# Elliotshui/ABRSimulator

Hardware: AMD Instinct MI355X
Metric: env_steps_per_sec (higher is better)
Workload: dtype f64

## Files before the change

abrsimulator_amd/csrc/abr_env.hip:

```cpp
#include <hip/hip_runtime.h>

#include <climits>
#include <cmath>
#include <cstdarg>
#include <cstdio>
#include <cstdlib>
#include <cstring>
#include <new>
#include <type_traits>
#include <vector>

#include "abr_env.h"

#ifdef ABR_SPLIT_STAMPS
#include "abr_diag_stamps.h"
#else
#define ABR_STAMP(n)
#define ABR_STAMP_INIT()
#define ABR_STAMP_FLUSH()
#define ABR_WG_TIME(slot)
#define ABR_WG_WHERE(role)
#define K3_STAMP_DECL
#define K3_STAMP(n)
#define K3_STAMP_FLUSH()
// ... 104 lines not shown
    int32_t pending_speed_rows;
    bool pending_rule_on;
    abrx::SpeedRuleBlock pending_rule;
    bool speeds_dirty;
    const double *pending_br_table;
    bool br_table_dirty;
    bool armed;
    bool sampler_on;
    abrx::EpisodeSampler sampler;
    abrx::EpisodeLedger ledger;
};

static void apply_pending(abr_env *env) {
    if (env->br_table_dirty) { env->p.br_table = env->pending_br_table; env->br_table_dirty = false; }
    if (env->speeds_dirty) {
        env->p.lane_speeds = env->pending_speeds; env->p.speed_rows = env->pending_speed_rows;
        env->p.speed_rule = env->pending_rule;
        if (env->pending_rule_on) { env->p.lane_speeds = env->p.sd_lane; env->p.speed_rows = abrx::kSpeedRowsRule; }
        env->speeds_dirty = false;
    }
}

__device__ inline double chunk_bitrate(const EnvParams &p, int32_t chunk, int32_t rate) {
    return p.br_table ? p.br_table[(int64_t)chunk * p.n_rates + rate] : p.ladder[rate];
}

__host__ __device__ inline uint32_t philox_action(uint64_t seed, uint64_t lane, uint32_t step,
                                                  uint32_t episode, uint32_t n_rates) {
    uint32_t c0 = (uint32_t)lane, c1 = (uint32_t)(lane >> 32), c2 = step, c3 = episode;
    uint32_t k0 = (uint32_t)seed, k1 = (uint32_t)(seed >> 32);
#pragma unroll
    for (int r = 0; r < 10; r++) {
        uint64_t p0 = (uint64_t)0xD2511F53u * c0, p1 = (uint64_t)0xCD9E8D57u * c2;
        uint32_t n0 = (uint32_t)(p1 >> 32) ^ c1 ^ k0, n1 = (uint32_t)p1;
        uint32_t n2 = (uint32_t)(p0 >> 32) ^ c3 ^ k1, n3 = (uint32_t)p0;
        c0 = n0; c1 = n1; c2 = n2; c3 = n3;
        k0 += 0x9E3779B9u; k1 += 0xBB67AE85u;
    }
    return (uint32_t)(((uint64_t)c0 * n_rates) >> 32);
}

struct Lane {
    double buf, dl, target, c, c_next;
    long long sumk;
    int32_t k, k_end, chunk_id, n_su, n_rb, n_play, n_dl, j, tpos, tlen;
    int32_t avail_k, avail_next, cur_action, last_action;
    bool su, be, bf;
    bool done_dl;
    bool running;
    const double *trace;
};

__device__ inline void lane_head(Lane &s) {
    s.n_su += s.su ? 1 : 0;
    s.n_rb += (!s.su && s.be) ? 1 : 0;
    const bool call = s.done_dl && (s.k >= s.avail_k) && !s.bf;
    s.running = !call;
}

__device__ inline void lane_init(Lane &s, const EnvParams &p, int32_t offset0) {
    s.buf = 0.0; s.dl = 0.0; s.target = 0.0; s.sumk = 0;
    s.k = 0; s.chunk_id = 0; s.n_su = 0; s.n_rb = 0; s.n_play = 0; s.n_dl = 0;
    s.cur_action = -1; s.last_action = -1;
    s.su = true; s.be = true; s.bf = false;
    s.done_dl = true;
    s.j = 0;
    s.tpos = offset0 % s.tlen;
    s.avail_k = p.avail_tick[0];
    s.avail_next = s.avail_k;
    lane_head(s);
}

__device__ inline void lane_refresh_interval(Lane &s, const EnvParams &p) {
    int32_t ke = p.interval_tick[s.j + 1];
    while (s.k >= ke) {
        s.j++;
        s.tpos = (s.tpos + 1 == s.tlen) ? 0 : s.tpos + 1;
        ke = p.interval_tick[s.j + 1];
    }
    s.k_end = ke;
    const int32_t tn = (s.tpos + 1 == s.tlen) ? 0 : s.tpos + 1;
    s.c = s.trace[s.tpos] * kDt;
    s.c_next = s.trace[tn] * kDt;
}

__device__ inline double avg_latency_from(double sd, double play_time, long long sumk, int32_t n_play) {
    if (n_play == 0) return 0.0;
    double tri = (double)(((long long)n_play * (n_play - 1)) / 2);
    return (kDt * (double)sumk - sd * tri) / play_time;
}
__device__ inline double lane_avg_latency(const EnvParams &p, long long sumk, int32_t n_play) {
    return avg_latency_from(p.sd, p.GP[n_play], sumk, n_play);
}
__device__ inline double avg_latency_sched(double play_time, long long sumk, double pt_sum, int32_t n_play) {
    if (n_play == 0) return 0.0;
    return (kDt * (double)sumk - pt_sum) / play_time;
}

__device__ inline void lane_load(Lane &s, const EnvParams &p, int64_t i) {
    s.buf = p.buf[i]; s.sumk = p.sumk[i];
    s.k = p.k[i]; s.chunk_id = p.chunk_id[i]; s.n_su = p.n_su[i]; s.n_rb = p.n_rb[i];
    s.n_play = p.n_play[i]; s.j = p.j[i]; s.tpos = p.tpos[i];
    s.last_action = p.last_action[i]; s.cur_action = -1;
    const uint8_t f = p.flags[i];
    s.su = f & kFlagStartUp; s.be = f & kFlagBufEmpty; s.bf = f & kFlagBufFull;
    s.dl = 0.0; s.n_dl = 0; s.target = 0.0; s.done_dl = true; s.running = false;
    const int32_t c = s.chunk_id < p.video_length ? s.chunk_id : p.video_length;
    s.avail_k = p.avail_tick[c];
    s.avail_next = s.avail_k;
}

__device__ inline void lane_store(const Lane &s, const EnvParams &p, int64_t i) {
    p.buf[i] = s.buf; p.sumk[i] = s.sumk;
    p.k[i] = s.k; p.chunk_id[i] = s.chunk_id; p.n_su[i] = s.n_su; p.n_rb[i] = s.n_rb;
    p.n_play[i] = s.n_play; p.j[i] = s.j; p.tpos[i] = s.tpos; p.last_action[i] = s.last_action;
    p.flags[i] = (uint8_t)((s.su ? kFlagStartUp : 0) | (s.be ? kFlagBufEmpty : 0) |
                           (s.bf ? kFlagBufFull : 0) | kFlagArmed);
}

__device__ inline void write_obs(const Lane &s, const EnvParams &p, int64_t i, float *obs,
                                 double last_bw) {
    if (!obs) return;
    const int64_t n = p.n_lanes;
    obs[ABR_OBS_CHUNK_ID * n + i] = (float)s.chunk_id;
    obs[ABR_OBS_LAST_BITRATE * n + i] = (float)s.last_action;
    obs[ABR_OBS_LAST_BANDWIDTH * n + i] = (float)last_bw;
    obs[ABR_OBS_BUFFER_LEVEL * n + i] = (float)s.buf;
    obs[ABR_OBS_GLOBAL_TIME * n + i] = (float)p.G[s.k];
    obs[ABR_OBS_PLAY_TIME * n + i] = (float)p.GP[s.n_play];
    obs[ABR_OBS_REBUFFER_TIME * n + i] = (float)p.G[s.n_rb];
    obs[ABR_OBS_STARTUP_TIME * n + i] = (float)p.G[s.n_su];
}


__device__ inline int32_t rule_action(const EnvParams &p, const abrx::RuleParams &rule, int64_t i, int32_t c, int32_t pv,
                                      double B) {
    const auto br = [&](int32_t m) { return chunk_bitrate(p, c, m); };
    const auto hist = [&](int32_t j) { return p.bw_hist[(int64_t)j * p.n_lanes + i]; };
    return abrx::rule_select_at(rule, br, hist, p.n_rates, p.video_length, c, pv, B);
}

__device__ inline void sampled_episode(const EnvParams &p, const abrx::EpisodeSampler &smp, int64_t i, int32_t e,
                                       int32_t &t, int32_t &off) {
    abrx::episode_assign(smp, (uint64_t)(p.lane_id_base + i), (uint32_t)e, p.n_traces, p.trace_len, t, off);
}

__device__ inline void ledger_record(const EnvParams &p, const abrx::EpisodeLedger &led, int64_t i, double g_rb, double g_su,
                                     double lat, double var_run, int32_t episode_no, int32_t trace_id, int32_t offset0,
                                     int32_t chunks, uint8_t done) {
    abrx::ledger_append(led, p.n_lanes, i, p.wr, p.wv, p.ws, p.wl, g_rb, g_su, lat, var_run, episode_no, trace_id, offset0,
                        chunks, (int32_t)done);
}

template <int MODE, bool SAMPLE = false, bool LEDGER = false>
__global__ __launch_bounds__(64) void env_advance_kernel(
    EnvParams p, const int32_t *__restrict__ actions, const int32_t *__restrict__ trace_id_in,
    const int32_t *__restrict__ offset_in, const uint8_t *__restrict__ lane_mask,
    float *__restrict__ obs_out, float *__restrict__ reward_out, uint8_t *__restrict__ done_out,
    int32_t *__restrict__ actions_out, int32_t n_steps, uint64_t seed, abrx::RuleParams rule,
    abrx::EpisodeSampler smp, abrx::EpisodeLedger led) {
    const int64_t i = (int64_t)blockIdx.x * 64 + threadIdx.x;
    const bool in_range = i < p.n_lanes;
    const int32_t n_total = (MODE >= 2) ? n_steps : 1;
    Lane s;
    bool active = in_range;
    bool touched = in_range;
    bool fresh = (MODE == 0);
    bool need_action = false;
    uint8_t done = 0;
    int32_t n_su_obs = 0, n_rb_obs = 0, episode_no = 0, offset0 = 0, prev_action = -1;
    double last_bw = 0.0, hist_n = 0.0, hist_s = 0.0, var_run = 0.0;
    int32_t step_idx = 0;
    s.running = false; s.done_dl = true;

    if (in_range) {
        if (MODE == 0) {
            if (lane_mask && !lane_mask[i]) { active = false; touched = false; }
            if (active) {
                int32_t t;
                if constexpr (SAMPLE) {
                    sampled_episode(p, smp, i, (p.flags[i] & kFlagArmed) ? p.episode_no[i] + 1 : 0, t, offset0);
                } else {
                    t = trace_id_in[i];
                    offset0 = offset_in ? offset_in[i] : 0;
                }
                if (t < 0 || t >= p.n_traces || offset0 < 0) { done |= ABR_DONE_BADARG; t = 0; offset0 = 0; }
                episode_no = (p.flags[i] & kFlagArmed) ? p.episode_no[i] + 1 : 0;
                p.trace_id[i] = t; p.offset0[i] = offset0;
                s.tlen = p.trace_len[t]; s.trace = p.traces + p.trace_off[t];
                lane_init(s, p, offset0);
                if (done) {
                    write_obs(s, p, i, obs_out, 0.0);
                    active = false; s.running = false;
                }
            }
        } else {
            done = p.done[i];
            const int32_t t = p.trace_id[i];
            offset0 = p.offset0[i];
            s.tlen = p.trace_len[t]; s.trace = p.traces + p.trace_off[t];
            lane_load(s, p, i);
            n_su_obs = p.n_su_obs[i]; n_rb_obs = p.n_rb_obs[i]; episode_no = p.episode_no[i];
            last_bw = p.last_bw[i]; hist_n = p.hist_n[i]; hist_s = p.hist_s[i]; var_run = p.var_run[i];
            if (done) active = false;
            need_action = active;
        }
    }

    const double L = p.chunk_length, sd = p.sd, max_buffer = p.max_buffer, sul = p.start_up_length;
    const int32_t V = p.video_length, max_ticks = p.max_ticks, T = p.t_block;

    while (__any(active)) {
        if (active && !s.running) {
            const bool ended = s.chunk_id >= V;
            const bool timeout = !ended && (s.k >= max_ticks);
            bool emit_obs = !need_action;
            if (!need_action && !fresh) {
                const int64_t o = (int64_t)step_idx * p.n_lanes + i;
                double var = 0.0;
                if (s.done_dl && s.cur_action >= 0) {
                    const double bw = s.dl / p.G[s.n_dl];
                    const int64_t h = (int64_t)(s.chunk_id - 1) * p.n_lanes + i;
                    p.bw_hist[h] = bw;
                    p.action_hist[h] = (uint8_t)s.cur_action;
                    last_bw = bw;
                    hist_s = hist_s + 1.0 / bw;
                    hist_n = hist_n + 1.0;
                    s.last_action = s.cur_action;
                    if (prev_action >= 0)
                        var = fabs(chunk_bitrate(p, s.chunk_id - 1, s.cur_action) -
                                   chunk_bitrate(p, s.chunk_id - 2, prev_action));
                    var_run = var_run + var;
                }
                const double r = p.wr * (p.G[s.n_rb] - p.G[n_rb_obs]) +
                                 p.ws * (p.G[s.n_su] - p.G[n_su_obs]) + p.wv * var;
                if (ended) done |= ABR_DONE_EPISODE;
                if (timeout) done |= ABR_DONE_TIMEOUT;
                if (reward_out) reward_out[o] = (float)r;
                if (done_out) done_out[o] = done;
                n_su_obs = s.n_su; n_rb_obs = s.n_rb;
                s.cur_action = -1;
                if (ended || timeout) {
                    p.ep_qoe_terms[0 * p.n_lanes + i] = p.G[s.n_rb];
                    p.ep_qoe_terms[1 * p.n_lanes + i] = p.G[s.n_su];
                    p.ep_qoe_terms[2 * p.n_lanes + i] = lane_avg_latency(p, s.sumk, s.n_play);
                    p.ep_qoe_terms[3 * p.n_lanes + i] = var_run;
                    if constexpr (LEDGER)
                        ledger_record(p, led, i, p.G[s.n_rb], p.G[s.n_su], lane_avg_latency(p, s.sumk, s.n_play), var_run,
                                      episode_no, p.trace_id[i], offset0, s.chunk_id, done);
                    if (p.auto_reset && ended) {
                        if constexpr (SAMPLE) {
                            int32_t t;
                            sampled_episode(p, smp, i, episode_no + 1, t, offset0);
                            p.trace_id[i] = t; p.offset0[i] = offset0;
                            s.tlen = p.trace_len[t]; s.trace = p.traces + p.trace_off[t];
                        }
                        lane_init(s, p, offset0);
                        episode_no++;
                        n_su_obs = 0; n_rb_obs = 0;
                        last_bw = 0.0; hist_n = 0.0; hist_s = 0.0; var_run = 0.0;
                        done = 0; fresh = true;
                        emit_obs = !s.running;
                    }
                }
            } else if (!need_action && fresh && timeout) {
                done |= ABR_DONE_TIMEOUT;
                if (MODE != 0 && done_out) done_out[(int64_t)step_idx * p.n_lanes + i] = done;
            }
            if (emit_obs) {
                fresh = false;
                float *obs = obs_out ? obs_out + (int64_t)step_idx * ABR_OBS_DIM * p.n_lanes : nullptr;
                write_obs(s, p, i, obs, last_bw);
                step_idx++;
                if (done || step_idx >= n_total) active = false;
                else need_action = true;
            }
            if (active && need_action) {
                int32_t a;
                if (MODE == 1) a = actions[i];
                else if (MODE == 3) a = actions[(int64_t)step_idx * p.n_lanes + i];
                else if (MODE == 4) a = rule_action(p, rule, i, s.chunk_id, s.last_action, s.buf);
                else a = (int32_t)philox_action(seed, (uint64_t)(p.lane_id_base + i),
                                                (uint32_t)s.chunk_id, (uint32_t)episode_no,
                                                (uint32_t)p.n_rates);
                if ((MODE == 2 || MODE == 4) && actions_out) actions_out[(int64_t)step_idx * p.n_lanes + i] = a;
                need_action = false;
                if (a < 0 || a >= p.n_rates) {
                    done |= ABR_DONE_BADACT;
                    if (done_out) done_out[(int64_t)step_idx * p.n_lanes + i] = done;
                    if (reward_out) reward_out[(int64_t)step_idx * p.n_lanes + i] = 0.0f;
                    float *obs = obs_out ? obs_out + (int64_t)step_idx * ABR_OBS_DIM * p.n_lanes : nullptr;
                    write_obs(s, p, i, obs, last_bw);
                    step_idx++;
                    active = false;
                } else {
                    prev_action = s.last_action;
                    s.cur_action = a;
                    s.target = chunk_bitrate(p, s.chunk_id, a) * L;
                    s.dl = 0.0; s.n_dl = 0; s.done_dl = false;
                    s.avail_next = p.avail_tick[s.chunk_id + 1];
                    s.running = true;
                }
            }
        }
        if (!__any(active)) break;
        if (active) lane_refresh_interval(s, p);

        double buf = s.buf, dl = s.dl, c = s.c;
        const double target = s.target, c_next = s.c_next;
        int32_t k = s.k, k_end = s.k_end, chunk_id = s.chunk_id, n_su = s.n_su, n_rb = s.n_rb;
        int32_t n_play = s.n_play, n_dl = s.n_dl, avail_k = s.avail_k;
        const int32_t avail_next = s.avail_next;
        uint32_t sk = 0;
        bool su = s.su, be = s.be, bf = s.bf, done_dl = s.done_dl;
        bool running = active && s.running;
        bool crossed = false;
        for (int32_t t = 0; t < T; t++) {
            if (!__any(running)) break;
            const bool dling = running && !done_dl;
            const double dl2 = dl + c;
            dl = dling ? dl2 : dl;
            n_dl += dling ? 1 : 0;
            const bool hit = dling && (dl2 >= target);
            done_dl = done_dl || hit;
            chunk_id += hit ? 1 : 0;
            avail_k = hit ? avail_next : avail_k;
            const double bufA = hit ? buf + L : buf;
            const bool playing = running && !(be || su);
            sk += playing ? (uint32_t)k : 0u;
            n_play += playing ? 1 : 0;
            const double bufB = playing ? bufA - sd : bufA;
            bf = bufB >= max_buffer;
            be = bufB <= 0.0;
            buf = be ? 0.0 : bufB;
            su = su && !(buf >= sul);
            k += running ? 1 : 0;
            const bool next = running && (chunk_id < V) && (k < max_ticks);
            n_su += (next && su) ? 1 : 0;
            n_rb += (next && !su && be) ? 1 : 0;
            const bool call = done_dl && (k >= avail_k) && !bf;
            running = next && !call;
            const bool cross = (k == k_end);
            c = cross ? c_next : c;
            crossed = crossed || cross;
        }
        if (active) {
            s.buf = buf; s.dl = dl; s.c = c; s.k = k; s.chunk_id = chunk_id; s.n_su = n_su;
            s.n_rb = n_rb; s.n_play = n_play; s.n_dl = n_dl; s.avail_k = avail_k;
            s.su = su; s.be = be; s.bf = bf; s.done_dl = done_dl; s.running = running;
            s.sumk += (long long)sk;
            (void)crossed;
        }
    }

    if (touched) {
        lane_store(s, p, i);
        p.n_su_obs[i] = n_su_obs; p.n_rb_obs[i] = n_rb_obs; p.episode_no[i] = episode_no;
        p.last_bw[i] = last_bw; p.hist_n[i] = hist_n; p.hist_s[i] = hist_s; p.var_run[i] = var_run;
        p.done[i] = done;
        if (MODE != 0) {
            for (int32_t t = step_idx; t < n_total; t++) {
                const int64_t o = (int64_t)t * p.n_lanes + i;
                if (reward_out) reward_out[o] = 0.0f;
                if (done_out) done_out[o] = done;
                if ((MODE == 2 || MODE == 4) && actions_out) actions_out[o] = -1;
                if (obs_out)
                    write_obs(s, p, i, obs_out + (int64_t)t * ABR_OBS_DIM * p.n_lanes, last_bw);
            }
        }
    }
}

using abrx::LaneJ;

__device__ inline abrx::Tables make_tables(const EnvParams &p, bool cascade = true) {
    abrx::Tables t;
    t.G = p.G; t.interval_tick = p.interval_tick; t.avail_tick = p.avail_tick;
    t.L = p.chunk_length; t.sd = p.sd; t.max_buffer = p.max_buffer;
    t.start_up_length = p.start_up_length; t.V = p.video_length; t.max_ticks = p.max_ticks;
    t.per_lane_speed = p.lane_speeds != nullptr;
    t.speed_rows = p.lane_speeds ? p.speed_rows : 0;
    t.speed_stride = p.n_lanes; t.speeds = p.lane_speeds;
    t.drain = p.drain;
    if (p.lane_speeds || !cascade) t.drain.n = 0;
#ifdef ABR_NO_DRAIN_CASCADE
    t.drain.n = 0;
#endif
    return t;
}

__device__ inline void lanej_load(LaneJ &s, const EnvParams &p, int64_t i) {
    s.buf = p.buf[i]; s.sumk = p.sumk[i];
    s.k = p.k[i]; s.chunk_id = p.chunk_id[i]; s.n_su = p.n_su[i]; s.n_rb = p.n_rb[i];
    s.n_play = p.n_play[i]; s.cur.j = p.j[i]; s.cur.tpos = p.tpos[i];
    s.last_action = p.last_action[i];
    const uint8_t f = p.flags[i];
    s.su = f & kFlagStartUp; s.be = f & kFlagBufEmpty; s.bf = f & kFlagBufFull;
    const int32_t c = s.chunk_id < p.video_length ? s.chunk_id : p.video_length;
    s.avail_k = p.avail_tick[c];
    if (p.lane_speeds) { s.sd = p.sd_lane[i]; s.pt = p.pt_lane[i]; } else { s.sd = p.sd; s.pt = 0.0; }
    s.lane = i; s.pl_left = 0; s.play_id = 0; s.pt_sum = 0.0;
    if (p.lane_speeds && p.speed_rows >= 2) { s.pl_left = p.pl_left[i]; s.play_id = p.play_id[i]; s.pt_sum = p.pt_sum[i]; }
}

__device__ inline void lanej_store(const LaneJ &s, const EnvParams &p, int64_t i) {
    p.buf[i] = s.buf; p.sumk[i] = s.sumk;
    p.k[i] = s.k; p.chunk_id[i] = s.chunk_id; p.n_su[i] = s.n_su; p.n_rb[i] = s.n_rb;
    p.n_play[i] = s.n_play; p.j[i] = s.cur.j; p.tpos[i] = s.cur.tpos; p.last_action[i] = s.last_action;
    p.flags[i] = (uint8_t)((s.su ? kFlagStartUp : 0) | (s.be ? kFlagBufEmpty : 0) |
                           (s.bf ? kFlagBufFull : 0) | kFlagArmed);
    if (p.lane_speeds) { p.sd_lane[i] = s.sd; p.pt_lane[i] = s.pt; }
    if (p.lane_speeds && p.speed_rows >= 2) { p.pl_left[i] = s.pl_left; p.play_id[i] = s.play_id; p.pt_sum[i] = s.pt_sum; }
}

#ifndef ABR_NO_NT_STORES
#define ABR_OUT(ref, val) __builtin_nontemporal_store((val), &(ref))
#else
#define ABR_OUT(ref, val) ((ref) = (val))
#endif

__device__ inline void write_obs_j(const LaneJ &s, const EnvParams &p, int64_t i, float *obs,
                                   double last_bw) {
    if (!obs) return;
    const int64_t n = p.n_lanes;
    ABR_OUT(obs[ABR_OBS_CHUNK_ID * n + i], (float)s.chunk_id);
    ABR_OUT(obs[ABR_OBS_LAST_BITRATE * n + i], (float)s.last_action);
    ABR_OUT(obs[ABR_OBS_LAST_BANDWIDTH * n + i], (float)last_bw);
    ABR_OUT(obs[ABR_OBS_BUFFER_LEVEL * n + i], (float)s.buf);
    ABR_OUT(obs[ABR_OBS_GLOBAL_TIME * n + i], (float)p.G[s.k]);
    ABR_OUT(obs[ABR_OBS_PLAY_TIME * n + i], (float)(p.lane_speeds ? s.pt : p.GP[s.n_play]));
    ABR_OUT(obs[ABR_OBS_REBUFFER_TIME * n + i], (float)p.G[s.n_rb]);
    ABR_OUT(obs[ABR_OBS_STARTUP_TIME * n + i], (float)p.G[s.n_su]);
}

__device__ inline void write_obs_vals(const LaneJ &s, const EnvParams &p, int64_t i, float *obs, double last_bw,
                                      double g_k, double g_play, double g_rb, double g_su) {
    if (!obs) return;
    const int64_t n = p.n_lanes;
    ABR_OUT(obs[ABR_OBS_CHUNK_ID * n + i], (float)s.chunk_id);
    ABR_OUT(obs[ABR_OBS_LAST_BITRATE * n + i], (float)s.last_action);
    ABR_OUT(obs[ABR_OBS_LAST_BANDWIDTH * n + i], (float)last_bw);
    ABR_OUT(obs[ABR_OBS_BUFFER_LEVEL * n + i], (float)s.buf);
    ABR_OUT(obs[ABR_OBS_GLOBAL_TIME * n + i], (float)g_k);
    ABR_OUT(obs[ABR_OBS_PLAY_TIME * n + i], (float)g_play);
    ABR_OUT(obs[ABR_OBS_REBUFFER_TIME * n + i], (float)g_rb);
    ABR_OUT(obs[ABR_OBS_STARTUP_TIME * n + i], (float)g_su);
}

#ifndef ABR_JUMP_WAVES
#define ABR_JUMP_WAVES 5
#endif
#define ABR_JUMP_BOUNDS(MODE, SAMPLE) __launch_bounds__(64, ((MODE) == 1 || (MODE) == 4 || (SAMPLE) ? 4 : ABR_JUMP_WAVES))
template <int MODE, bool SAMPLE = false, bool LEDGER = false>
__global__ ABR_JUMP_BOUNDS(MODE, SAMPLE || LEDGER) void env_jump_kernel(
    EnvParams p, const int32_t *__restrict__ actions, const int32_t *__restrict__ trace_id_in,
    const int32_t *__restrict__ offset_in, const uint8_t *__restrict__ lane_mask,
    float *__restrict__ obs_out, float *__restrict__ reward_out, uint8_t *__restrict__ done_out,
    int32_t *__restrict__ actions_out, int32_t n_steps, uint64_t seed, abrx::RuleParams rule,
    abrx::EpisodeSampler smp, abrx::EpisodeLedger led) {
    const int64_t i = (int64_t)blockIdx.x * 64 + threadIdx.x;
    const bool in_range = i < p.n_lanes;
    const int32_t n_total = (MODE >= 2) ? n_steps : 1;
    const abrx::Tables tb = make_tables(p);
    LaneJ s;
    bool active = in_range, touched = in_range;
    uint8_t done = 0;
    int32_t n_su_obs = 0, n_rb_obs = 0, episode_no = 0, offset0 = 0;
    double last_bw = 0.0, hist_n = 0.0, hist_s = 0.0, var_run = 0.0;
    double g_su_obs = 0.0, g_rb_obs = 0.0;

    if (in_range) {
        if (MODE == 0) {
            if (lane_mask && !lane_mask[i]) { active = false; touched = false; }
            if (active) {
                int32_t t;
                if constexpr (SAMPLE) {
                    sampled_episode(p, smp, i, (p.flags[i] & kFlagArmed) ? p.episode_no[i] + 1 : 0, t, offset0);
                } else {
                    t = trace_id_in[i];
                    offset0 = offset_in ? offset_in[i] : 0;
                }
                const bool bad = t < 0 || t >= p.n_traces || offset0 < 0;
                if (bad) { done |= ABR_DONE_BADARG; t = 0; offset0 = 0; }
                episode_no = (p.flags[i] & kFlagArmed) ? p.episode_no[i] + 1 : 0;
                p.trace_id[i] = t; p.offset0[i] = offset0;
                s.cur.tlen = p.trace_len[t]; s.cur.trace = p.traces + p.trace_off[t];
                s.sd = (p.lane_speeds && p.speed_rows != abrx::kSpeedRowsRule) ? p.lane_speeds[i] * kDt : p.sd;
                s.lane = i;
                abrx::lanej_init(s, tb, offset0);
                if (!bad && !abrx::lanej_wait_call(s, tb)) done |= ABR_DONE_TIMEOUT;
                write_obs_j(s, p, i, obs_out, 0.0);
            }
        } else {
            done = p.done[i];
            const int32_t t = p.trace_id[i];
            offset0 = p.offset0[i];
            s.cur.tlen = p.trace_len[t]; s.cur.trace = p.traces + p.trace_off[t];
            lanej_load(s, p, i);
            n_su_obs = p.n_su_obs[i]; n_rb_obs = p.n_rb_obs[i]; episode_no = p.episode_no[i];
            last_bw = p.last_bw[i]; hist_n = p.hist_n[i]; hist_s = p.hist_s[i]; var_run = p.var_run[i];
            g_su_obs = p.G[n_su_obs]; g_rb_obs = p.G[n_rb_obs];
            if (done) active = false;
        }
    }

    if (MODE != 0) {
        for (int32_t step = 0; step < n_total; step++) {
            const int64_t o = (int64_t)step * p.n_lanes + i;
            float *obs = obs_out ? obs_out + (int64_t)step * ABR_OBS_DIM * p.n_lanes : nullptr;
            if (active) {
                const int32_t a_rule = (MODE == 4) ? rule_action(p, rule, i, s.chunk_id, s.last_action, s.buf) : 0;
                const abrx::StepStart st = abrx::lanej_begin_step(s.cur, tb, s.k, s.chunk_id);
                int32_t a;
                if (MODE == 1) a = actions[i];
                else if (MODE == 3) a = actions[o];
                else if (MODE == 4) a = a_rule;
                else a = (int32_t)philox_action(seed, (uint64_t)(p.lane_id_base + i),
                                                (uint32_t)s.chunk_id, (uint32_t)episode_no,
                                                (uint32_t)p.n_rates);
                if ((MODE == 2 || MODE == 4) && actions_out) ABR_OUT(actions_out[o], a);
                if (a < 0 || a >= p.n_rates) {
                    done |= ABR_DONE_BADACT;
                    if (reward_out) ABR_OUT(reward_out[o], 0.0f);
                    if (done_out) ABR_OUT(done_out[o], (uint8_t)done);
                    write_obs_j(s, p, i, obs, last_bw);
                    active = false;
                } else {
                    const int32_t prev_action = s.last_action;
                    const int32_t chunk = s.chunk_id;
                    const abrx::StepResult r = abrx::lanej_download_and_wait(
                        s, tb, st, chunk_bitrate(p, chunk, a) * p.chunk_length , a);
                    const double g_rb = p.G[s.n_rb], g_su = p.G[s.n_su];
                    double o_k = p.G[s.k], o_pl = p.lane_speeds ? s.pt : p.GP[s.n_play], o_rb = g_rb, o_su = g_su;
                    double var = 0.0;
                    if (r.hit) {
                        const int64_t h = (int64_t)chunk * p.n_lanes + i;
                        ABR_OUT(p.bw_hist[h], r.bw);
                        ABR_OUT(p.action_hist[h], (uint8_t)a);
                        last_bw = r.bw;
                        hist_s = hist_s + 1.0 / r.bw;
                        hist_n = hist_n + 1.0;
                        if (prev_action >= 0)
                            var = fabs(chunk_bitrate(p, chunk, a) - chunk_bitrate(p, chunk - 1, prev_action));
                        var_run = var_run + var;
                    }
                    const double rew = p.wr * (g_rb - g_rb_obs) + p.ws * (g_su - g_su_obs) + p.wv * var;
                    if (r.ended) done |= ABR_DONE_EPISODE;
                    if (r.timeout) done |= ABR_DONE_TIMEOUT;
                    if (reward_out) ABR_OUT(reward_out[o], (float)rew);
                    if (done_out) ABR_OUT(done_out[o], (uint8_t)done);
                    n_su_obs = s.n_su; n_rb_obs = s.n_rb;
                    g_su_obs = g_su; g_rb_obs = g_rb;
                    if (r.ended || r.timeout) {
                        p.ep_qoe_terms[0 * p.n_lanes + i] = g_rb;
                        p.ep_qoe_terms[1 * p.n_lanes + i] = g_su;
                        p.ep_qoe_terms[2 * p.n_lanes + i] =
                            !p.lane_speeds ? lane_avg_latency(p, s.sumk, s.n_play)
                            : (p.speed_rows >= 2 ? avg_latency_sched(s.pt, s.sumk, s.pt_sum, s.n_play)
                                                 : avg_latency_from(s.sd, s.pt, s.sumk, s.n_play));
                        p.ep_qoe_terms[3 * p.n_lanes + i] = var_run;
                        if constexpr (LEDGER)
                            ledger_record(p, led, i, g_rb, g_su, p.ep_qoe_terms[2 * p.n_lanes + i], var_run, episode_no,
                                          p.trace_id[i], offset0, s.chunk_id, done);
                        if (p.auto_reset && r.ended) {
                            if constexpr (SAMPLE) {
                                int32_t t;
                                sampled_episode(p, smp, i, episode_no + 1, t, offset0);
                                p.trace_id[i] = t; p.offset0[i] = offset0;
                                s.cur.tlen = p.trace_len[t]; s.cur.trace = p.traces + p.trace_off[t];
                            }
                            abrx::lanej_init(s, tb, offset0);
                            episode_no++;
                            n_su_obs = 0; n_rb_obs = 0; g_su_obs = 0.0; g_rb_obs = 0.0;
                            last_bw = 0.0; hist_n = 0.0; hist_s = 0.0; var_run = 0.0;
                            done = 0;
                            if (!abrx::lanej_wait_call(s, tb)) done |= ABR_DONE_TIMEOUT;
                            o_k = p.G[s.k]; o_pl = p.lane_speeds ? s.pt : p.GP[s.n_play];
                            o_rb = p.G[s.n_rb]; o_su = p.G[s.n_su];
                        }
                    }
                    write_obs_vals(s, p, i, obs, last_bw, o_k, o_pl, o_rb, o_su);
                    if (done) active = false;
                }
            } else if (in_range) {
                if (reward_out) ABR_OUT(reward_out[o], 0.0f);
                if (done_out) ABR_OUT(done_out[o], (uint8_t)done);
                if ((MODE == 2 || MODE == 4) && actions_out) ABR_OUT(actions_out[o], (int32_t)-1);
                write_obs_j(s, p, i, obs, last_bw);
            }
        }
    }

    if (touched) {
        lanej_store(s, p, i);
        p.n_su_obs[i] = n_su_obs; p.n_rb_obs[i] = n_rb_obs; p.episode_no[i] = episode_no;
        p.last_bw[i] = last_bw; p.hist_n[i] = hist_n; p.hist_s[i] = hist_s; p.var_run[i] = var_run;
        p.done[i] = done;
    }
}

#include "abr_env_roles.h"
#ifdef ABR_WITH_RING
#include "abr_env_ring.h"
#include "abr_env_pair.h"
#endif
#ifdef ABR_WITH_ASYNC
#include "abr_env_async.h"
#endif

__global__ void episode_qoe_kernel(EnvParams p, double *__restrict__ qoe_out) {
    const int64_t i = (int64_t)blockIdx.x * blockDim.x + threadIdx.x;
    if (i >= p.n_lanes) return;
    double variance = 0.0;
    if (p.auto_reset) {
        variance = p.ep_qoe_terms[3 * p.n_lanes + i];
    } else {
        for (int c = 0; c < p.video_length - 1; c++) {
            int a0 = p.action_hist[(int64_t)c * p.n_lanes + i], a1 = p.action_hist[(int64_t)(c + 1) * p.n_lanes + i];
            variance += fabs(chunk_bitrate(p, c, a0) - chunk_bitrate(p, c + 1, a1));
        }
    }
    qoe_out[i] = p.wr * p.ep_qoe_terms[0 * p.n_lanes + i] + p.wv * variance +
                 p.ws * p.ep_qoe_terms[1 * p.n_lanes + i] +
                 p.wl * p.ep_qoe_terms[2 * p.n_lanes + i];
}

__global__ void observe_f64_kernel(EnvParams p, double *__restrict__ out) {
    const int64_t i = (int64_t)blockIdx.x * blockDim.x + threadIdx.x;
    if (i >= p.n_lanes) return;
    const int64_t n = p.n_lanes;
    out[ABR_F64_GLOBAL_TIME * n + i] = p.G[p.k[i]];
    out[ABR_F64_REBUFFER_TIME * n + i] = p.G[p.n_rb[i]];
    out[ABR_F64_STARTUP_TIME * n + i] = p.G[p.n_su[i]];
    int32_t P = p.play_ticks_per_chunk;
    const bool sched = p.lane_speeds && p.speed_rows >= 2;
    if (p.lane_speeds) {
        double x = 0.0; int32_t a = 0;
        abrx::chain<abrx::STOP_GE>(x, p.sd_lane[i], p.chunk_length, p.max_ticks + 1, a);
        P = a > 0 ? a : 1;
        out[ABR_F64_PLAY_TIME * n + i] = p.pt_lane[i];
        out[ABR_F64_AVERAGE_LATENCY * n + i] =
            sched ? avg_latency_sched(p.pt_lane[i], p.sumk[i], p.pt_sum[i], p.n_play[i])
                  : avg_latency_from(p.sd_lane[i], p.pt_lane[i], p.sumk[i], p.n_play[i]);
    } else {
        out[ABR_F64_PLAY_TIME * n + i] = p.GP[p.n_play[i]];
        out[ABR_F64_AVERAGE_LATENCY * n + i] = lane_avg_latency(p, p.sumk[i], p.n_play[i]);
    }
    out[ABR_F64_BUFFER_LEVEL * n + i] = p.buf[i];
    if (sched) {
        const int32_t pl = p.pl_left[i];
        double x = 0.0; int32_t a = 0;
        abrx::chain<abrx::STOP_GE>(x, p.sd_lane[i], 1.0e300, pl > 0 ? P - pl : 0, a);
        out[ABR_F64_PLAY_LENGTH * n + i] = x;
    } else if (p.lane_speeds) {
        double x = 0.0; int32_t a = 0;
        abrx::chain<abrx::STOP_GE>(x, p.sd_lane[i], 1.0e300, p.n_play[i] % P, a);
        out[ABR_F64_PLAY_LENGTH * n + i] = x;
    } else {
        out[ABR_F64_PLAY_LENGTH * n + i] = p.GP[p.n_play[i] % P];
    }
    out[ABR_F64_LAST_BANDWIDTH * n + i] = p.last_bw[i];
    out[ABR_F64_CHUNK_ID * n + i] = (double)p.chunk_id[i];
    out[ABR_F64_PLAY_ID * n + i] = sched ? (double)p.play_id[i] : (double)(p.n_play[i] / P);
    out[ABR_F64_LAST_BITRATE * n + i] = (double)p.last_action[i];
    out[ABR_F64_FLAGS * n + i] = (double)p.flags[i];
    out[ABR_F64_HIST_N * n + i] = p.hist_n[i];
    out[ABR_F64_HIST_SUM_INV * n + i] = p.hist_s[i];
    out[ABR_F64_TICK * n + i] = (double)p.k[i];
    out[ABR_F64_DOWNLOAD_TIME * n + i] = 0.0;
}

static size_t align_up(size_t x, size_t a) { return (x + a - 1) / a * a; }
static size_t mpc_scratch_bytes_max(size_t n_lanes) {
    return n_lanes * ((size_t)ABR_MAX_HORIZON * sizeof(double) + 2 * sizeof(int32_t));
}

struct Layout {
    size_t G, GP, interval_tick, avail_tick;
    size_t f64_state, i64_state, i32_state, u8_state, action_hist, bw_hist, ep_terms;
    size_t mpc_action, mpc_scratch;
    size_t tag;
    size_t total;
    int32_t max_ticks, n_intervals;
};

static double min_episode_ticks(const abr_env_config *c) {
    return ((double)c->video_length + 1.0) * ceil(c->chunk_length / kDt);
}
static double default_max_ticks(const abr_env_config *c) {
    double per_chunk = ceil(c->chunk_length / kDt);
    double mt = 32.0 * c->video_length * per_chunk;
    if (mt > 16.0e6) mt = 16.0e6;
    if (mt < 2.0 * min_episode_ticks(c)) mt = 2.0 * min_episode_ticks(c);
    if (mt < 1024) mt = 1024;
    return mt;
}

static int validate_cfg(const abr_env_config *c) {
    if (!c) return fail(ABR_E_INVALID, "config is NULL");
    if (c->n_rates < 1 || c->n_rates > ABR_MAX_RATES)
        return fail(ABR_E_INVALID, "n_rates %d outside 1..%d", c->n_rates, ABR_MAX_RATES);
    if (c->video_length < 1 || c->video_length > 65535)
        return fail(ABR_E_INVALID, "video_length %d outside 1..65535", c->video_length);
    if (!(c->chunk_length > 0) || !(c->interval > 0) || !(c->speed > 0))
        return fail(ABR_E_INVALID, "chunk_length, interval and speed must be > 0");
    if (!(c->max_buffer > 0)) return fail(ABR_E_INVALID, "max_buffer must be > 0");
    if (!(c->start_up_length >= 0)) return fail(ABR_E_INVALID, "start_up_length must be >= 0");
    if (c->chunk_length / kDt > 1.0e6)
        return fail(ABR_E_UNSUPPORTED, "chunk_length %g s is more than 1e6 ticks", c->chunk_length);
    for (int r = 0; r < c->n_rates; r++)
        if (!(c->ladder[r] > 0)) return fail(ABR_E_INVALID, "ladder[%d] must be > 0", r);
    return ABR_OK;
}

static int compute_layout(const abr_env_config *c, int64_t n_lanes, Layout *L) {
    int rc = validate_cfg(c);
    if (rc) return rc;
    if (n_lanes < 1) return fail(ABR_E_INVALID, "n_lanes must be >= 1");
    const double mtd = c->max_ticks > 0 ? (double)c->max_ticks : default_max_ticks(c);
    if (mtd > 256.0e6)
        return fail(ABR_E_UNSUPPORTED, "video_length %d x chunk_length %g s needs a %g-entry tick table",
                    c->video_length, c->chunk_length, mtd);
    if (mtd < min_episode_ticks(c))
        return fail(ABR_E_INVALID, "max_ticks %g is below (video_length + 1) * ceil(chunk_length / dt) = %g: "
                    "every lane would end in ABR_DONE_TIMEOUT", mtd, min_episode_ticks(c));
    const int32_t mt = (int32_t)mtd;
    double n_iv = (double)mt * kDt / c->interval + 4.0;
    if (n_iv > 32.0e6)
        return fail(ABR_E_UNSUPPORTED, "interval %g s needs a %g-entry tick table", c->interval, n_iv);
    L->max_ticks = mt;
    L->n_intervals = (int32_t)n_iv;
    size_t o = 0;
    const size_t A = 256;
    size_t N = (size_t)n_lanes, V = (size_t)c->video_length;
    L->G = o; o = align_up(o + sizeof(double) * ((size_t)mt + 2), A);
    L->GP = o; o = align_up(o + sizeof(double) * ((size_t)mt + 2), A);
    L->interval_tick = o; o = align_up(o + sizeof(int32_t) * ((size_t)L->n_intervals + 8), A);
    L->avail_tick = o; o = align_up(o + sizeof(int32_t) * (V + 2), A);
    L->f64_state = o; o = align_up(o + sizeof(double) * 8 * N, A);
    L->i64_state = o; o = align_up(o + sizeof(long long) * 1 * N, A);
    L->i32_state = o; o = align_up(o + sizeof(int32_t) * 15 * N, A);
    L->u8_state = o; o = align_up(o + 2 * N, A);
    L->action_hist = o; o = align_up(o + V * N, A);
    L->bw_hist = o; o = align_up(o + sizeof(double) * V * N, A);
    L->ep_terms = o; o = align_up(o + sizeof(double) * 4 * N, A);
    L->mpc_action = o; o = align_up(o + sizeof(int32_t) * N, A);
    L->mpc_scratch = o; o = align_up(o + mpc_scratch_bytes_max(N), A);
// ... 203 lines not shown
            return fail(ABR_E_INVALID, "speed rule: buf_thr must be strictly ascending (buf_thr[%d])", q);
    }
    for (int i = 0; i <= nl; i++)
        for (int j = 0; j <= nb; j++)
            if (!(std::isfinite(r->speed[i][j]) && r->speed[i][j] > 0.0))
                return fail(ABR_E_INVALID, "speed rule: speed[%d][%d] must be finite and > 0", i, j);
    return ABR_OK;
}

extern "C" int abr_env_set_speed_rule(abr_env *env, const abr_speed_rule *rule, double *speed_log_dev, int32_t log_rows) {
    if (rule) {
        const int rc = check_speed_rule(rule);
        if (rc != ABR_OK) return rc;
        if (log_rows < 0) return fail(ABR_E_INVALID, "log_rows must be >= 0, got %d", log_rows);
        if (log_rows > 0 && !speed_log_dev) return fail(ABR_E_INVALID, "log_rows > 0 needs speed_log_dev");
    }
    if (!env) return fail(ABR_E_INVALID, "env is NULL");
    int rc;
    if (rule && (rc = require(kSpeedRule, env->impl))) return rc;
    env->pending_speeds = nullptr;
    env->pending_speed_rows = 1;
    env->pending_rule_on = rule != nullptr;
    env->pending_rule = abrx::SpeedRuleBlock{};
    if (rule) {
        std::memcpy(&env->pending_rule.rule, rule, sizeof(abr_speed_rule));
        env->pending_rule.log = log_rows > 0 ? speed_log_dev : nullptr;
        env->pending_rule.log_rows = log_rows > 0 ? log_rows : 0;
    }
    env->speeds_dirty = true;
    if (!env->armed) apply_pending(env);
    return ABR_OK;
}

extern "C" int abr_env_set_bitrate_table(abr_env *env, const double *br_table_dev) {
    if (!env) return fail(ABR_E_INVALID, "env is NULL");
    env->pending_br_table = br_table_dev;
    env->br_table_dirty = true;
    if (!env->armed) apply_pending(env);
    return ABR_OK;
}

extern "C" int abr_env_notify_restore(abr_env *env) {
    if (!env) return fail(ABR_E_INVALID, "env is NULL");
    WorkspaceTag got;
    HIP_TRY(hipDeviceSynchronize());
    HIP_TRY(hipMemcpy(&got, env->tag_dev, sizeof(got), hipMemcpyDeviceToHost));
    const WorkspaceTag &w = env->tag;
    if (got.magic != kTagMagic)
        return fail(ABR_E_WORKSPACE, "the restored workspace carries no layout tag: it was not written by this library at ABI "
                    "version >= 4 (a version-2 / -3 checkpoint cannot be restored: the lane-state layout changed)");
    if (got.abi_version != w.abi_version || got.layout_rev != w.layout_rev)
        return fail(ABR_E_WORKSPACE, "the restored workspace was laid out by ABI version %u (layout %u), this library is %u (%u)",
                    got.abi_version, got.layout_rev, w.abi_version, w.layout_rev);
    if (got.n_lanes != w.n_lanes || got.video_length != w.video_length || got.n_rates != w.n_rates ||
        got.max_ticks != w.max_ticks || got.n_intervals != w.n_intervals || got.total_bytes != w.total_bytes ||
        got.chunk_length != w.chunk_length || got.interval != w.interval || got.speed != w.speed)
        return fail(ABR_E_WORKSPACE, "the restored workspace belongs to another configuration: %lld lanes, %d chunks, %u rates, "
                    "%d ticks, %llu bytes (this handle: %lld, %d, %u, %d, %llu)", (long long)got.n_lanes, got.video_length,
                    got.n_rates, got.max_ticks, (unsigned long long)got.total_bytes, (long long)w.n_lanes, w.video_length,
                    w.n_rates, w.max_ticks, (unsigned long long)w.total_bytes);
    apply_pending(env);
    env->armed = true;
    return ABR_OK;
}

extern "C" int abr_env_set_lane_id_base(abr_env *env, int64_t base) {
    if (!env) return fail(ABR_E_INVALID, "env is NULL");
    env->p.lane_id_base = base;
    return ABR_OK;
}

extern "C" int abr_env_set_episode_sampler(abr_env *env, const abr_episode_sampler *s) {
    if (s) {
        if (s->pool && s->n_pool < 1) return fail(ABR_E_INVALID, "episode sampler: a pool needs n_pool >= 1, got %d", s->n_pool);
        if (s->offset_span < 0) return fail(ABR_E_INVALID, "episode sampler: offset_span must be >= 0, got %d", s->offset_span);
    }
    if (!env) return fail(ABR_E_INVALID, "env is NULL");
    if (!s) { env->sampler_on = false; env->sampler = abrx::EpisodeSampler{}; return ABR_OK; }
    if (s->pool) {
        std::vector<int32_t> pool((size_t)s->n_pool);
        HIP_TRY(hipDeviceSynchronize());
        HIP_TRY(hipMemcpy(pool.data(), s->pool, pool.size() * sizeof(int32_t), hipMemcpyDefault));
        for (size_t q = 0; q < pool.size(); q++)
            if (pool[q] < 0 || pool[q] >= env->p.n_traces)
                return fail(ABR_E_INVALID, "episode sampler: pool[%zu] = %d outside [0, %d)", q, pool[q], env->p.n_traces);
    }
    abrx::EpisodeSampler v{};
    v.seed = s->seed; v.pool = s->pool; v.n_pool = s->pool ? s->n_pool : 0; v.offset_span = s->offset_span;
    env->sampler = v;
    env->sampler_on = true;
    return ABR_OK;
}

extern "C" int abr_env_ledger_bytes(int32_t n_lanes, int32_t rows, size_t *bytes_out) {
    if (!bytes_out) return fail(ABR_E_INVALID, "bytes_out is NULL");
    if (n_lanes < 1) return fail(ABR_E_INVALID, "episode ledger: n_lanes must be >= 1, got %d", n_lanes);
    if (rows < 1) return fail(ABR_E_INVALID, "episode ledger: rows must be >= 1, got %d", rows);
    *bytes_out = abrx::ledger_layout(n_lanes, rows).bytes;
    return ABR_OK;
}

extern "C" int abr_env_set_episode_ledger(abr_env *env, const abr_episode_ledger *l) {
    if (l) {
        if (l->rows < 1) return fail(ABR_E_INVALID, "episode ledger: rows must be >= 1, got %d", l->rows);
        if (!l->base_dev) return fail(ABR_E_INVALID, "episode ledger: base_dev is NULL");
        if ((uintptr_t)l->base_dev % 256) return fail(ABR_E_INVALID, "episode ledger: base_dev must be 256-byte aligned");
    }
    if (!env) return fail(ABR_E_INVALID, "env is NULL");
    abrx::EpisodeLedger v{};
    if (l) { v.base = l->base_dev; v.rows = l->rows; }
    env->ledger = v;
    return ABR_OK;
}

extern "C" int abr_env_get_episode(abr_env *env, int32_t *trace_id_out_dev, int32_t *offset_out_dev,
                                   int32_t *episode_out_dev, void *stream) {
    if (!env) return fail(ABR_E_INVALID, "env is NULL");
    const size_t bytes = (size_t)env->p.n_lanes * sizeof(int32_t);
    hipStream_t st = (hipStream_t)stream;
    if (trace_id_out_dev) HIP_TRY(hipMemcpyAsync(trace_id_out_dev, env->p.trace_id, bytes, hipMemcpyDeviceToDevice, st));
    if (offset_out_dev) HIP_TRY(hipMemcpyAsync(offset_out_dev, env->p.offset0, bytes, hipMemcpyDeviceToDevice, st));
    if (episode_out_dev) HIP_TRY(hipMemcpyAsync(episode_out_dev, env->p.episode_no, bytes, hipMemcpyDeviceToDevice, st));
    return ABR_OK;
}

static inline unsigned grid64(int64_t n) { return (unsigned)((n + 63) / 64); }

constexpr int64_t kSplit3MaxLanes = 65536;
constexpr int64_t kSplitMaxLanes = 131072;
#ifdef ABR_WITH_ASYNC
static inline bool async_eligible(const abr_env *env) {
    return !env->p.lane_speeds && env->p.video_length + 2 <= kAvailLds;
}
#endif
static inline int effective_impl(const abr_env *env, bool fused = false) {
    int impl = env->impl;
    if (impl == 3) {
        if (!fused) return 0;
        if (env->p.n_lanes <= kSplit3MaxLanes) return 5;
        return env->p.n_lanes <= kSplitMaxLanes ? 2 : 0;
    }
#ifdef ABR_WITH_ASYNC
    if (impl == 4) return (fused && async_eligible(env)) ? 4 : 2;
#endif
    (void)fused;
    return impl;
}
template <int MODE>
static inline int launch_impl(const abr_env *env, int32_t n_steps) {
    if (MODE == 0 || MODE == 4) return env->impl == 1 ? 1 : 0;
    return effective_impl(env, n_steps > 1);
}

template <int MODE, bool SAMPLE, bool LEDGER>
static void launch_env_kernels(const abr_env *env, int impl, hipStream_t st, const int32_t *actions, float *obs, float *rew,
                               uint8_t *dn, int32_t *acts, int32_t n_steps, uint64_t seed, const abrx::RuleParams &rule,
                               const int32_t *trace_id, const int32_t *start_offset, const uint8_t *lane_mask) {
    const EnvParams &p = env->p;
    const int64_t N = p.n_lanes;
    const abrx::EpisodeSampler smp = SAMPLE ? env->sampler : abrx::EpisodeSampler{};
    const abrx::EpisodeLedger led = LEDGER ? env->ledger : abrx::EpisodeLedger{};
    if (impl == 0 || impl == 1) {
        auto *k = impl == 1 ? env_advance_kernel<MODE, SAMPLE, LEDGER> : env_jump_kernel<MODE, SAMPLE, LEDGER>;
        hipLaunchKernelGGL(k, dim3(grid64(N)), dim3(64), 0, st, p, actions, trace_id, start_offset, lane_mask, obs, rew, dn,
                           acts, n_steps, seed, rule, smp, led);
    } else if constexpr (MODE >= 1 && MODE <= 3) {
        if (impl == 5) {
            auto *k = env_split3_kernel<MODE, SAMPLE, LEDGER>;
            hipLaunchKernelGGL(k, dim3(grid64(N)), dim3(192), 0, st, p, actions, obs, rew, dn, acts, n_steps, seed, smp, led);
        } else if (impl == 2) {
            auto *k = env_split_kernel<MODE, SAMPLE, LEDGER>;
            hipLaunchKernelGGL(k, dim3(grid64(N)), dim3(128), 0, st, p, actions, obs, rew, dn, acts, n_steps, seed, smp, led);
        }
#ifdef ABR_WITH_RING
        else if constexpr (!SAMPLE && !LEDGER) {
            if (impl == 6)
                hipLaunchKernelGGL(env_ring3_kernel<MODE>, dim3(grid64(N)), dim3(64 * ABR_RING_WAVES), 0, st, p, actions, obs,
                                   rew, dn, acts, n_steps, seed);
            else if (impl == 7)
                hipLaunchKernelGGL(env_pair3_kernel<MODE>, dim3(grid64(N)), dim3(192), 0, st, p, actions, obs, rew, dn, acts,
                                   n_steps, seed);
        }
#endif
    }
}

template <int MODE>
static int launch_env(const abr_env *env, int impl, hipStream_t st, const int32_t *actions, float *obs, float *rew,
                      uint8_t *dn, int32_t *acts, int32_t n_steps, uint64_t seed, const abrx::RuleParams &rule = {},
                      const int32_t *trace_id = nullptr, const int32_t *start_offset = nullptr,
                      const uint8_t *lane_mask = nullptr) {
    const EnvParams &p = env->p;
    const int64_t N = p.n_lanes;
    const bool sample = env->sampler_on && !(MODE == 0 && trace_id);
    if (sample && impl != 0 && impl != 1 && impl != 2 && impl != 5)
        return fail(ABR_E_UNSUPPORTED, "the episode sampler runs on impl 0, 1, 2, 3 and 5, not on the diagnostic impl %d", impl);
    if (env->ledger.base && impl != 0 && impl != 1 && impl != 2 && impl != 5)
        return fail(ABR_E_UNSUPPORTED, "the episode ledger runs on impl 0, 1, 2, 3 and 5, not on the diagnostic impl %d", impl);
    (void)N;
#ifdef ABR_WITH_ASYNC
    if constexpr (MODE == 2 || MODE == 3) {
        if (impl == 4) {
            for (int32_t s0 = 0; s0 < n_steps; s0 += kMaxFuse) {
                const int32_t n = n_steps - s0 < kMaxFuse ? n_steps - s0 : kMaxFuse;
                hipLaunchKernelGGL(env_async_kernel<MODE>, dim3((unsigned)((N + kAW - 1) / kAW)), dim3(3 * kAW), 0, st,
                                   p, actions ? actions + (int64_t)s0 * N : nullptr,
                                   obs ? obs + (int64_t)s0 * ABR_OBS_DIM * N : nullptr,
                                   rew ? rew + (int64_t)s0 * N : nullptr, dn ? dn + (int64_t)s0 * N : nullptr,
                                   acts ? acts + (int64_t)s0 * N : nullptr, n, seed);
            }
            HIP_TRY(hipGetLastError());
            return ABR_OK;
        }
    }
#endif
    const bool ledger = MODE != 0 && env->ledger.base;
    const auto go = [&](auto smp_on, auto led_on) {
        launch_env_kernels<MODE, decltype(smp_on)::value, decltype(led_on)::value>(
            env, impl, st, actions, obs, rew, dn, acts, n_steps, seed, rule, trace_id, start_offset, lane_mask);
    };
    if constexpr (MODE == 0) {
        if (sample) go(std::true_type{}, std::false_type{});
        else go(std::false_type{}, std::false_type{});
    } else {
        if (sample && ledger) go(std::true_type{}, std::true_type{});
        else if (sample) go(std::true_type{}, std::false_type{});
        else if (ledger) go(std::false_type{}, std::true_type{});
        else go(std::false_type{}, std::false_type{});
    }
    HIP_TRY(hipGetLastError());
    return ABR_OK;
}

extern "C" int abr_env_reset(abr_env *env, const int32_t *trace_id_dev,
                             const int32_t *start_offset_dev, const uint8_t *lane_mask_dev,
                             float *obs_out_dev, void *stream) {
    if (!env) return fail(ABR_E_INVALID, "env is NULL");
    if (!trace_id_dev && !env->sampler_on)
        return fail(ABR_E_INVALID, "trace_id_dev is NULL (allowed only while an episode sampler is installed)");
    if (!trace_id_dev && start_offset_dev)
        return fail(ABR_E_INVALID, "a sampled reset (trace_id_dev NULL) takes no start_offset_dev");
    if (env->br_table_dirty && lane_mask_dev)
        return fail(ABR_E_INVALID, "abr_env_set_bitrate_table takes effect at a reset of ALL lanes "
                    "(lane_mask_dev must be NULL for the first reset after it)");
    if (env->speeds_dirty && lane_mask_dev)
        return fail(ABR_E_INVALID, "abr_env_set_lane_speeds takes effect at a reset of ALL lanes "
                    "(lane_mask_dev must be NULL for the first reset after it)");
    apply_pending(env);
    env->armed = true;
    return launch_env<0>(env, launch_impl<0>(env, 0), (hipStream_t)stream, nullptr, obs_out_dev, nullptr, nullptr,
                         nullptr, 0, 0ull, {}, trace_id_dev, start_offset_dev, lane_mask_dev);
}

extern "C" int abr_env_step(abr_env *env, const int32_t *actions_dev, float *obs_out_dev,
                            float *reward_out_dev, uint8_t *done_out_dev, void *stream) {
    if (!env) return fail(ABR_E_INVALID, "env is NULL");
    if (!actions_dev) return fail(ABR_E_INVALID, "actions_dev is NULL");
    return launch_env<1>(env, launch_impl<1>(env, 1), (hipStream_t)stream, actions_dev, obs_out_dev, reward_out_dev,
                         done_out_dev, nullptr, 1, 0ull);
}

extern "C" int abr_env_step_random(abr_env *env, int32_t n_steps, uint64_t seed,
                                   float *obs_out_dev, float *reward_out_dev,
                                   uint8_t *done_out_dev, int32_t *actions_out_dev, void *stream) {
    if (!env) return fail(ABR_E_INVALID, "env is NULL");
    if (n_steps < 1) return fail(ABR_E_INVALID, "n_steps must be >= 1");
    return launch_env<2>(env, launch_impl<2>(env, n_steps), (hipStream_t)stream, nullptr, obs_out_dev, reward_out_dev,
                         done_out_dev, actions_out_dev, n_steps, seed);
}

extern "C" int abr_env_step_script(abr_env *env, int32_t n_steps, const int32_t *actions_dev,
                                   float *obs_out_dev, float *reward_out_dev, uint8_t *done_out_dev,
                                   void *stream) {
    if (!env) return fail(ABR_E_INVALID, "env is NULL");
    if (n_steps < 1) return fail(ABR_E_INVALID, "n_steps must be >= 1");
    if (!actions_dev) return fail(ABR_E_INVALID, "actions_dev is NULL");
    return launch_env<3>(env, launch_impl<3>(env, n_steps), (hipStream_t)stream, actions_dev, obs_out_dev, reward_out_dev,
                         done_out_dev, nullptr, n_steps, 0ull);
}

static int validate_rule(const abr_rule_config *r, abrx::RuleParams *out) {
    if (!r) return fail(ABR_E_INVALID, "rule is NULL");
    if (r->kind != ABR_RULE_BUFFER && r->kind != ABR_RULE_RATE && r->kind != ABR_RULE_BOLA)
        return fail(ABR_E_INVALID, "unknown rule kind %d", r->kind);
    const double v[5] = {r->reservoir, r->cushion, r->safety, r->bola_v, r->bola_gp};
    for (double x : v)
        if (!std::isfinite(x)) return fail(ABR_E_INVALID, "rule parameters must be finite");
    if (r->kind == ABR_RULE_BUFFER && !(r->reservoir >= 0.0 && r->cushion > 0.0))
        return fail(ABR_E_INVALID, "BUFFER needs reservoir >= 0 and cushion > 0 (got %g, %g)", r->reservoir, r->cushion);
    if (r->kind == ABR_RULE_RATE && r->window < 1) return fail(ABR_E_INVALID, "RATE needs window >= 1 (got %d)", r->window);
    if (r->kind == ABR_RULE_RATE && !(r->safety > 0.0)) return fail(ABR_E_INVALID, "RATE needs safety > 0 (got %g)", r->safety);
    if (r->kind == ABR_RULE_BOLA && !(r->bola_v > 0.0)) return fail(ABR_E_INVALID, "BOLA needs bola_v > 0 (got %g)", r->bola_v);
    if (r->kind == ABR_RULE_BOLA && !r->utility_dev) return fail(ABR_E_INVALID, "BOLA needs utility_dev");
    out->kind = r->kind; out->window = r->window;
    out->reservoir = r->reservoir; out->cushion = r->cushion; out->safety = r->safety;
    out->bola_v = r->bola_v; out->bola_gp = r->bola_gp; out->utility = r->utility_dev;
    return ABR_OK;
}

extern "C" int abr_env_step_rule(abr_env *env, const abr_rule_config *rule, int32_t n_steps, float *obs_out_dev,
                                 float *reward_out_dev, uint8_t *done_out_dev, int32_t *actions_out_dev, void *stream) {
    abrx::RuleParams rp;
    int rc = validate_rule(rule, &rp);
    if (rc) return rc;
    if (n_steps < 1) return fail(ABR_E_INVALID, "n_steps must be >= 1");
    if (!env) return fail(ABR_E_INVALID, "env is NULL");
    if ((rc = require(kRuleRollout, env->impl))) return rc;
    return launch_env<4>(env, launch_impl<4>(env, n_steps), (hipStream_t)stream, nullptr, obs_out_dev, reward_out_dev,
                         done_out_dev, actions_out_dev, n_steps, 0ull, rp);
}

__global__ __launch_bounds__(256) void rule_select_kernel(EnvParams p, abrx::RuleParams rule, int32_t *__restrict__ action_out) {
    const int64_t i = (int64_t)blockIdx.x * blockDim.x + threadIdx.x;
    if (i >= p.n_lanes) return;
    action_out[i] = p.done[i] ? -1 : rule_action(p, rule, i, p.chunk_id[i], p.last_action[i], p.buf[i]);
}

extern "C" int abr_env_rule_select(abr_env *env, const abr_rule_config *rule, int32_t *action_out_dev, void *stream) {
    abrx::RuleParams rp;
    int rc = validate_rule(rule, &rp);
    if (rc) return rc;
    if (!env || !action_out_dev) return fail(ABR_E_INVALID, "NULL argument");
    hipLaunchKernelGGL(rule_select_kernel, dim3((unsigned)((env->p.n_lanes + 255) / 256)), dim3(256), 0,
                       (hipStream_t)stream, env->p, rp, action_out_dev);
    HIP_TRY(hipGetLastError());
    return ABR_OK;
}

extern "C" int abr_env_get_effective_impl(abr_env *env, int32_t fused, int32_t *impl_out) {
    if (!env || !impl_out) return fail(ABR_E_INVALID, "NULL argument");
    *impl_out = effective_impl(env, fused != 0);
    return ABR_OK;
}

extern "C" int abr_env_episode_qoe(abr_env *env, double *qoe_out_dev, void *stream) {
    if (!env || !qoe_out_dev) return fail(ABR_E_INVALID, "NULL argument");
    hipLaunchKernelGGL(episode_qoe_kernel, dim3((unsigned)((env->p.n_lanes + 255) / 256)),
                       dim3(256), 0, (hipStream_t)stream, env->p, qoe_out_dev);
    HIP_TRY(hipGetLastError());
    return ABR_OK;
}

extern "C" int abr_env_observe_f64(abr_env *env, double *out_dev, void *stream) {
    if (!env || !out_dev) return fail(ABR_E_INVALID, "NULL argument");
    hipLaunchKernelGGL(observe_f64_kernel, dim3((unsigned)((env->p.n_lanes + 255) / 256)),
                       dim3(256), 0, (hipStream_t)stream, env->p, out_dev);
    HIP_TRY(hipGetLastError());
    return ABR_OK;
}

#ifdef ABR_SPLIT_STAMPS
extern "C" int abr_debug_read_stamps(unsigned long long *out32, int reset) {
    (void)hipDeviceSynchronize();
    (void)hipMemcpyFromSymbol(out32, HIP_SYMBOL(g_st_acc), 32 * sizeof(unsigned long long));
    if (reset) { unsigned long long z[32] = {0}; (void)hipMemcpyToSymbol(HIP_SYMBOL(g_st_acc), z, sizeof(z)); }
    return 0;
}
#endif

#ifdef ABR_SPLIT_STAMPS
extern "C" int abr_debug_read_stamps_xcd(unsigned long long *out8x32, int reset) {
    (void)hipDeviceSynchronize();
    (void)hipMemcpyFromSymbol(out8x32, HIP_SYMBOL(g_st_acc_xcd), 8 * 32 * sizeof(unsigned long long));
    if (reset) { static unsigned long long z[8 * 32]; (void)hipMemcpyToSymbol(HIP_SYMBOL(g_st_acc_xcd), z, sizeof(z)); }
    return 0;
}
extern "C" int abr_debug_read_wg_times(unsigned long long *out, int n_wg) {
    (void)hipDeviceSynchronize();
    (void)hipMemcpyFromSymbol(out, HIP_SYMBOL(g_wg_t), (size_t)n_wg * 10 * sizeof(unsigned long long));
    return 0;
}
#endif
// ... 2097 lines not shown
```

abrsimulator_amd/csrc/abr_env_roles.h:

```cpp
#ifndef ABR_ENV_ROLES_H
#define ABR_ENV_ROLES_H


#ifndef ABR_SPLIT3_CASCADE
#define ABR_SPLIT3_CASCADE 0
#endif
#ifndef ABR_PRIO_D
#define ABR_PRIO_D 2
#endif
#ifndef ABR_PRIO_P
#define ABR_PRIO_P 1
#endif
#ifndef ABR_PRIO_S
#define ABR_PRIO_S 0
#endif

struct SplitMail {
    double dl[2][64];
    int32_t n_dl[2][64], k_start[2][64], step[2][64], action[2][64], avail_next[2][64], flags[2][64];
    int32_t fb_step[2][64], fb_k[2][64], fb_chunk[2][64], fb_episode[2][64], fb_alive[2][64];
    double fb_buf[2][64];
    int32_t fb_pf[2][64];
    int32_t any_alive[2];
};
struct ActRing {
    uint8_t act[64][64];
    int32_t act_hi;
};
constexpr int kRecValid = 1, kRecHit = 2, kRecBadAct = 4;

struct SplitMail2 {
    double dl[2][64], buf[2][64], lat[2][64], pt[2][64];
    int32_t meta[2][64], step[2][64], n_dl[2][64], k[2][64], nplay_o[2][64], nrb_o[2][64], nsu_o[2][64],
        nrb_r[2][64], nsu_r[2][64];
};
constexpr int kS3Valid = 0x10000, kS3Hit = 0x100, kS3Bad = 0x200, kS3Ended = 0x400, kS3Timeout = 0x800,
              kS3Reset = 0x1000, kS3Timeout2 = 0x2000;

__device__ __forceinline__ int32_t lds_ld(const int32_t *w) {
    return __hip_atomic_load(w, __ATOMIC_RELAXED, __HIP_MEMORY_SCOPE_WORKGROUP);
}
__device__ __forceinline__ void lds_st(int32_t *w, int32_t v) {
    __hip_atomic_store(w, v, __ATOMIC_RELAXED, __HIP_MEMORY_SCOPE_WORKGROUP);
}
#define ABR_LDS_ORDER() asm volatile("" ::: "memory")
__device__ __forceinline__ void lds_writes_done() {
    ABR_LDS_ORDER();
    __builtin_amdgcn_s_waitcnt(0xc07f);
    ABR_LDS_ORDER();
}

__device__ __forceinline__ const EnvParams &fresh_params() {
    auto kp = __builtin_amdgcn_kernarg_segment_ptr();
    asm volatile("" : "+s"(kp));
    return *(const EnvParams *)kp;
}

__device__ __forceinline__ void selfcheck_answer(const EnvParams &p) {
    if (threadIdx.x == 0 && blockIdx.x == 0) {
        const EnvParams &f = fresh_params();
        *p.selfcheck_out = (f.sentinel == p.sentinel && f.selfcheck_out == p.selfcheck_out && f.n_lanes == p.n_lanes &&
                            f.traces == p.traces && f.G == p.G) ? 1u : 2u;
    }
}

struct RolePark3 { uint32_t p[24][64], s[32][64]; };
struct RolePark2 { uint32_t p[40][64]; };

struct ParkWords {
    uint32_t w[40];
    int n;
};
__device__ __forceinline__ void pw_i32(ParkWords &k, int32_t x) { k.w[k.n++] = (uint32_t)x; }
__device__ __forceinline__ void pw_i64(ParkWords &k, long long x) {
    k.w[k.n++] = (uint32_t)x; k.w[k.n++] = (uint32_t)((unsigned long long)x >> 32);
}
__device__ __forceinline__ void pw_f64(ParkWords &k, double x) { pw_i64(k, __double_as_longlong(x)); }
__device__ __forceinline__ int32_t pr_i32(const ParkWords &k, int &at) { return (int32_t)k.w[at++]; }
__device__ __forceinline__ long long pr_i64(const ParkWords &k, int &at) {
    const unsigned long long lo = k.w[at], hi = k.w[at + 1];
    at += 2;
    return (long long)(lo | (hi << 32));
}
__device__ __forceinline__ double pr_f64(const ParkWords &k, int &at) { return __longlong_as_double(pr_i64(k, at)); }
template <int Q>
__device__ __forceinline__ void park_store(uint32_t (*area)[64], const ParkWords &k) {
    const int l = threadIdx.x & 63;
#pragma unroll
    for (int q = 0; q < 4 * Q; q++) area[q][l] = k.w[q];
}
template <int Q>
__device__ __forceinline__ void park_load(uint32_t (*area)[64], ParkWords &k) {
    const int l = threadIdx.x & 63;
#pragma unroll
    for (int q = 0; q < 4 * Q; q++) k.w[q] = area[q][l];
    k.n = 0;
}

__device__ inline void lanej_store_player(const LaneJ &s, const EnvParams &p, int64_t i) {
    p.buf[i] = s.buf; p.sumk[i] = s.sumk;
    p.k[i] = s.k; p.chunk_id[i] = s.chunk_id; p.n_su[i] = s.n_su; p.n_rb[i] = s.n_rb;
    p.n_play[i] = s.n_play; p.last_action[i] = s.last_action;
    p.flags[i] = (uint8_t)((s.su ? kFlagStartUp : 0) | (s.be ? kFlagBufEmpty : 0) |
                           (s.bf ? kFlagBufFull : 0) | kFlagArmed);
    if (p.lane_speeds) { p.sd_lane[i] = s.sd; p.pt_lane[i] = s.pt; }
    if (p.lane_speeds && p.speed_rows >= 2) { p.pl_left[i] = s.pl_left; p.play_id[i] = s.play_id; p.pt_sum[i] = s.pt_sum; }
}

struct DVars {
    abrx::Cursor cur;
    int32_t snap_j, snap_tpos;
    int32_t d_step, d_k, d_chunk, d_ep, offset0, issued_step, issued_k;
    int32_t issued_ndl, issued_avail;
    bool d_alive, was_alive;
    const double *snap_trace;
    int32_t snap_tlen;
};
__device__ __forceinline__ void role_d_begin(DVars &v, const EnvParams &p) {
    const int l = threadIdx.x & 63;
    const int64_t i = (int64_t)blockIdx.x * 64 + l;
    v.cur.j = 0; v.cur.tpos = 0; v.cur.tlen = 1; v.cur.trace = p.traces;
    v.snap_j = 0; v.snap_tpos = 0; v.d_step = 0; v.d_k = 0; v.d_chunk = 0; v.d_ep = 0; v.offset0 = 0;
    v.issued_step = -1; v.issued_k = -1; v.issued_ndl = 0; v.issued_avail = 0; v.d_alive = false; v.was_alive = false;
    if (i < p.n_lanes) {
        const int32_t t = p.trace_id[i];
        v.offset0 = p.offset0[i];
        v.cur.tlen = p.trace_len[t]; v.cur.trace = p.traces + p.trace_off[t];
        v.cur.j = p.j[i]; v.cur.tpos = p.tpos[i];
        v.d_k = p.k[i]; v.d_chunk = p.chunk_id[i]; v.d_ep = p.episode_no[i];
        v.d_alive = v.was_alive = !p.done[i];
    }
    ABR_STAMP_INIT();
}

template <int MODE, bool ACT_RING, bool SAMPLE = false>
__device__ __forceinline__ void role_d_pre(DVars &v, const EnvParams &p, SplitMail &m, ActRing *ring,
                                           const int32_t *__restrict__ actions, int32_t *__restrict__ actions_out,
                                           int32_t n_total, uint64_t seed, int32_t t,
                                           const abrx::EpisodeSampler &smp = abrx::EpisodeSampler{}) {
    const int l = threadIdx.x & 63;
    const int64_t i = (int64_t)blockIdx.x * 64 + l;
    const int32_t V = p.video_length;
    const int cb = t & 1;
    const abrx::Tables tb = make_tables(p);
    int32_t flags = 0;
    ABR_STAMP(0);
    if (v.d_alive && v.d_step < n_total) {
        v.snap_j = v.cur.j; v.snap_tpos = v.cur.tpos;
        if constexpr (SAMPLE) { v.snap_trace = v.cur.trace; v.snap_tlen = v.cur.tlen; }
        const abrx::StepStart st = abrx::lanej_begin_step(v.cur, tb, v.d_k, v.d_chunk);
        ABR_STAMP(1);
        int32_t a = -1;
        bool drawn = false;
        if (MODE == 1) a = actions[i];
        else if (MODE == 3) a = actions[(int64_t)v.d_step * p.n_lanes + i];
        else if (ACT_RING && t > 0) {
            const int32_t hi = lds_ld(&ring->act_hi);
            ABR_LDS_ORDER();
            drawn = v.d_step < hi && v.d_step >= hi - 64;
            if (drawn) a = ring->act[v.d_step & 63][l];
        }
        if (MODE == 2 && !drawn)
            a = (int32_t)philox_action(seed, (uint64_t)(p.lane_id_base + i), (uint32_t)v.d_chunk,
                                       (uint32_t)v.d_ep, (uint32_t)p.n_rates);
        if (MODE == 2 && actions_out) actions_out[(int64_t)v.d_step * p.n_lanes + i] = a;
        flags = kRecValid;
        abrx::Download d; d.dl = 0.0; d.n_dl = 0; d.hit = false;
        ABR_STAMP(2);
        if (a < 0 || a >= p.n_rates) flags |= kRecBadAct;
        else d = abrx::lanej_download(v.cur, tb, st, v.d_k,
                                      chunk_bitrate(p, v.d_chunk, a) * p.chunk_length );
        ABR_STAMP(3);
        if (d.hit) flags |= kRecHit;
        m.dl[cb][l] = d.dl; m.n_dl[cb][l] = d.n_dl; m.k_start[cb][l] = v.d_k;
        m.step[cb][l] = v.d_step; m.action[cb][l] = a; m.avail_next[cb][l] = st.avail_next;
        v.issued_step = v.d_step; v.issued_k = v.d_k;
        v.issued_ndl = d.hit ? d.n_dl : 0; v.issued_avail = st.avail_next;
        if (!d.hit) v.d_alive = false;
        else {
            v.d_step++;
            v.d_chunk++;
            v.d_k = max(v.d_k + d.n_dl, st.avail_next);
            if (v.d_chunk >= V) {
                if (p.auto_reset) {
                    v.d_chunk = 0; v.d_ep++; v.d_k = tb.avail_tick[0];
                    if constexpr (SAMPLE) {
                        int32_t tr;
                        sampled_episode(p, smp, i, v.d_ep, tr, v.offset0);
                        v.cur.tlen = p.trace_len[tr]; v.cur.trace = p.traces + p.trace_off[tr];
                    }
                    abrx::cursor_init(v.cur, v.offset0);
                } else v.d_alive = false;
            }
            if (v.d_k >= tb.max_ticks) v.d_alive = false;
        }
    }
    m.flags[cb][l] = flags;
    ABR_STAMP(4);
}

template <bool SAMPLE = false>
__device__ __forceinline__ void role_d_validate(DVars &v, SplitMail &m, const abrx::Tables &tb, int32_t t) {
    const int l = threadIdx.x & 63;
    const int cb = t & 1;
    int32_t f_alive = m.fb_alive[cb][l], f_step = m.fb_step[cb][l], f_k = m.fb_k[cb][l], f_pf = m.fb_pf[cb][l];
    double f_buf = m.fb_buf[cb][l];
    asm volatile("" : "+v"(f_alive), "+v"(f_step), "+v"(f_k), "+v"(f_pf), "+v"(f_buf));
    if (!f_alive) v.d_alive = false;
    else if (v.issued_step != f_step || v.issued_k != f_k) {
        v.d_alive = true;
        v.d_step = f_step; v.d_k = f_k;
        v.d_chunk = m.fb_chunk[cb][l]; v.d_ep = m.fb_episode[cb][l];
        if (v.issued_step == v.d_step) {
            v.cur.j = v.snap_j; v.cur.tpos = v.snap_tpos;
            if constexpr (SAMPLE) { v.cur.trace = v.snap_trace; v.cur.tlen = v.snap_tlen; }
        }
        v.issued_step = -1;
    } else if (v.d_alive && v.issued_ndl > 0 && v.d_chunk > 0) {
        const int32_t pf = f_pf;
        const double buf = f_buf;
        if (abrx::lanej_gate_possible(buf, pf & 1, pf & 2, v.issued_ndl, tb)) {
            int32_t kn;
            if (abrx::lanej_predict_next_call(buf, v.issued_k, v.issued_ndl, v.issued_avail, tb, kn)) {
                v.d_k = kn;
                if (kn >= tb.max_ticks) v.d_alive = false;
            }
        }
    }
}

__device__ __forceinline__ void role_d_end(const DVars &v, const EnvParams &p) {
    const int64_t i = (int64_t)blockIdx.x * 64 + (threadIdx.x & 63);
    ABR_STAMP_FLUSH();
    if (i < p.n_lanes && v.was_alive) { p.j[i] = v.cur.j; p.tpos[i] = v.cur.tpos; }
}

struct PVars {
    LaneJ s;
    int32_t episode_no, b_step;
    bool b_alive, was_done;
};
__device__ __forceinline__ void p_words(ParkWords &k, const PVars &v) {
    const LaneJ &s = v.s;
    pw_f64(k, s.buf); pw_f64(k, s.sd); pw_f64(k, s.pt); pw_f64(k, s.pt_sum); pw_i64(k, s.sumk);
    pw_i32(k, s.k); pw_i32(k, s.chunk_id); pw_i32(k, s.n_su); pw_i32(k, s.n_rb); pw_i32(k, s.n_play);
    pw_i32(k, s.avail_k); pw_i32(k, s.last_action); pw_i32(k, s.pl_left); pw_i32(k, s.play_id);
    pw_i32(k, (s.su ? 1 : 0) | (s.be ? 2 : 0) | (s.bf ? 4 : 0) | (v.b_alive ? 8 : 0) | (v.was_done ? 16 : 0));
    pw_i32(k, v.episode_no); pw_i32(k, v.b_step);
    pw_i32(k, 0); pw_i32(k, 0);
}
__device__ __forceinline__ void p_unwords(const ParkWords &k, int &at, PVars &v, const EnvParams &p) {
    LaneJ &s = v.s;
    s.buf = pr_f64(k, at); s.sd = pr_f64(k, at); s.pt = pr_f64(k, at); s.pt_sum = pr_f64(k, at); s.sumk = pr_i64(k, at);
    s.k = pr_i32(k, at); s.chunk_id = pr_i32(k, at); s.n_su = pr_i32(k, at); s.n_rb = pr_i32(k, at);
    s.n_play = pr_i32(k, at); s.avail_k = pr_i32(k, at); s.last_action = pr_i32(k, at); s.pl_left = pr_i32(k, at);
    s.play_id = pr_i32(k, at);
    const int32_t fl = pr_i32(k, at);
    s.su = fl & 1; s.be = fl & 2; s.bf = fl & 4; v.b_alive = fl & 8; v.was_done = fl & 16;
    v.episode_no = pr_i32(k, at); v.b_step = pr_i32(k, at);
    at += 2;
    s.cur.j = 0; s.cur.tpos = 0; s.cur.tlen = 1; s.cur.trace = p.traces;
    s.lane = (int64_t)blockIdx.x * 64 + (threadIdx.x & 63);
}
__device__ __forceinline__ void p_park(uint32_t (*area)[64], const PVars &v) {
    ParkWords k; k.n = 0;
    p_words(k, v);
    park_store<6>(area, k);
}
__device__ __forceinline__ void p_unpark(uint32_t (*area)[64], PVars &v, const EnvParams &p) {
    ParkWords k; park_load<6>(area, k);
    int at = 0;
    p_unwords(k, at, v, p);
}

__device__ __forceinline__ double player_latency(const EnvParams &p, const LaneJ &s) {
    return !p.lane_speeds ? lane_avg_latency(p, s.sumk, s.n_play)
           : (p.speed_rows >= 2 ? avg_latency_sched(s.pt, s.sumk, s.pt_sum, s.n_play)
                                : avg_latency_from(s.sd, s.pt, s.sumk, s.n_play));
}

__device__ __forceinline__ void player_feedback(SplitMail &m, const PVars &v, int32_t n_total, int cb) {
    const int l = threadIdx.x & 63;
    const bool more = v.b_alive && v.b_step < n_total;
    m.fb_step[cb][l] = v.b_step; m.fb_k[cb][l] = v.s.k; m.fb_chunk[cb][l] = v.s.chunk_id;
    m.fb_episode[cb][l] = v.episode_no; m.fb_alive[cb][l] = more ? 1 : 0;
    m.fb_buf[cb][l] = v.s.buf; m.fb_pf[cb][l] = (v.s.su ? 1 : 0) | (v.s.be ? 2 : 0);
    const bool any = __any(more) != 0;
    if (l == 0) m.any_alive[cb] = any ? 1 : 0;
}

__device__ __forceinline__ void player_clear(PVars &v, const EnvParams &p) {
    LaneJ &s = v.s;
    s.buf = 0.0; s.sd = 0.0; s.pt = 0.0; s.pt_sum = 0.0; s.sumk = 0;
    s.k = 0; s.chunk_id = 0; s.n_su = 0; s.n_rb = 0; s.n_play = 0; s.avail_k = 0; s.last_action = -1;
    s.pl_left = 0; s.play_id = 0; s.su = false; s.be = false; s.bf = false;
    s.cur.j = 0; s.cur.tpos = 0; s.cur.tlen = 1; s.cur.trace = p.traces;
    s.lane = (int64_t)blockIdx.x * 64 + (threadIdx.x & 63);
    v.episode_no = 0; v.b_step = 0; v.b_alive = false; v.was_done = true;
}

__device__ __forceinline__ void role_p3_begin(PVars &v, const EnvParams &p) {
    const int64_t i = (int64_t)blockIdx.x * 64 + (threadIdx.x & 63);
    player_clear(v, p);
    if (i < p.n_lanes) {
        v.was_done = p.done[i] != 0;
        lanej_load(v.s, p, i);
        v.episode_no = p.episode_no[i];
        v.b_alive = !v.was_done;
    }
    ABR_STAMP_INIT();
}

template <int MODE, class M2>
__device__ __forceinline__ void role_p3_pre(PVars &v, const EnvParams &p, SplitMail &m, M2 &m2,
                                            int32_t n_total, int32_t t, int cb2) {
    const int l = threadIdx.x & 63;
    const int cb = t & 1, pb = (t + 1) & 1;
    const abrx::Tables tb = make_tables(p, ABR_SPLIT3_CASCADE != 0);
    const bool speeds = p.lane_speeds != nullptr;
    LaneJ &s = v.s;
    int32_t meta = 0;
    ABR_STAMP(8);
    if (v.b_alive && v.b_step < n_total && t >= 1) {
        int32_t fl = m.flags[pb][l];
        int32_t r_step = m.step[pb][l], r_k = m.k_start[pb][l], r_a = m.action[pb][l], r_ndl = m.n_dl[pb][l],
                r_avail = m.avail_next[pb][l];
        double r_dl = m.dl[pb][l];
        asm volatile("" : "+v"(fl), "+v"(r_step), "+v"(r_k), "+v"(r_a), "+v"(r_ndl), "+v"(r_avail), "+v"(r_dl));
        if ((fl & kRecValid) && r_step == v.b_step && r_k == s.k) {
            const int32_t a = r_a;
            meta = kS3Valid | (a & 0xff);
            m2.step[cb2][l] = v.b_step;
            if (fl & kRecBadAct) {
                meta |= kS3Bad;
                v.b_alive = false;
            } else {
                abrx::Download d;
                d.dl = r_dl; d.n_dl = r_ndl; d.hit = (fl & kRecHit) != 0;
                const abrx::StepResult sr = abrx::lanej_after_download(s, tb, d, r_avail, a);
                if (sr.hit) meta |= kS3Hit;
                if (sr.ended) meta |= kS3Ended;
                if (sr.timeout) meta |= kS3Timeout;
                m2.dl[cb2][l] = d.dl; m2.n_dl[cb2][l] = d.n_dl;
                m2.nrb_r[cb2][l] = s.n_rb; m2.nsu_r[cb2][l] = s.n_su;
                if (sr.ended || sr.timeout) {
                    m2.lat[cb2][l] = player_latency(p, s);
                    if (p.auto_reset && sr.ended) {
                        abrx::lanej_init_player(s, tb);
                        v.episode_no++;
                        meta |= kS3Reset;
                        if (!abrx::lanej_wait_call(s, tb)) { meta |= kS3Timeout2; v.b_alive = false; }
                    } else v.b_alive = false;
                }
                m2.buf[cb2][l] = s.buf; m2.k[cb2][l] = s.k; m2.nplay_o[cb2][l] = s.n_play;
                m2.nrb_o[cb2][l] = s.n_rb; m2.nsu_o[cb2][l] = s.n_su;
                if (speeds) m2.pt[cb2][l] = s.pt;
            }
            v.b_step++;
        }
    }
    ABR_STAMP(13);
    m2.meta[cb2][l] = meta;
    player_feedback(m, v, n_total, cb);
    ABR_STAMP(17);
}

__device__ __forceinline__ void role_p3_end(const PVars &v, const EnvParams &p) {
    const int64_t i = (int64_t)blockIdx.x * 64 + (threadIdx.x & 63);
    ABR_STAMP_FLUSH();
    if (i < p.n_lanes && !v.was_done) lanej_store_player(v.s, p, i);
}

struct SVars {
    double last_bw, hist_n, hist_s, g_su_obs, g_rb_obs;
    double var_run;
    double o_buf, o_pt;
    int32_t o_chunk, o_last, o_k, o_nplay, o_nrb, o_nsu;
    int32_t n_su_obs, n_rb_obs, episode_no, s_next;
    int32_t a_next, a_chunk, a_ep;
    int32_t last_cb;
    uint8_t done;
    bool was_done;
};
__device__ __forceinline__ void s_park(uint32_t (*area)[64], const SVars &v) {
    ParkWords k; k.n = 0;
    pw_f64(k, v.last_bw); pw_f64(k, v.hist_n); pw_f64(k, v.hist_s); pw_f64(k, v.g_su_obs); pw_f64(k, v.g_rb_obs);
    pw_f64(k, v.o_buf); pw_f64(k, v.o_pt);
    pw_i32(k, v.o_chunk); pw_i32(k, v.o_last); pw_i32(k, v.o_k); pw_i32(k, v.o_nplay); pw_i32(k, v.o_nrb);
    pw_i32(k, v.o_nsu); pw_i32(k, v.n_su_obs); pw_i32(k, v.n_rb_obs); pw_i32(k, v.episode_no); pw_i32(k, v.s_next);
    pw_i32(k, v.a_next); pw_i32(k, v.a_chunk); pw_i32(k, v.a_ep); pw_i32(k, v.last_cb);
    pw_i32(k, (int32_t)v.done | (v.was_done ? 0x100 : 0));
    pw_f64(k, v.var_run); pw_i32(k, 0);
    park_store<8>(area, k);
}
__device__ __forceinline__ void s_unpark(uint32_t (*area)[64], SVars &v) {
    ParkWords k; park_load<8>(area, k);
    int at = 0;
    v.last_bw = pr_f64(k, at); v.hist_n = pr_f64(k, at); v.hist_s = pr_f64(k, at); v.g_su_obs = pr_f64(k, at);
    v.g_rb_obs = pr_f64(k, at); v.o_buf = pr_f64(k, at); v.o_pt = pr_f64(k, at);
    v.o_chunk = pr_i32(k, at); v.o_last = pr_i32(k, at); v.o_k = pr_i32(k, at); v.o_nplay = pr_i32(k, at);
    v.o_nrb = pr_i32(k, at); v.o_nsu = pr_i32(k, at); v.n_su_obs = pr_i32(k, at); v.n_rb_obs = pr_i32(k, at);
    v.episode_no = pr_i32(k, at); v.s_next = pr_i32(k, at); v.a_next = pr_i32(k, at); v.a_chunk = pr_i32(k, at);
    v.a_ep = pr_i32(k, at); v.last_cb = pr_i32(k, at);
    const int32_t fl = pr_i32(k, at);
    v.done = (uint8_t)(fl & 0xff); v.was_done = (fl & 0x100) != 0;
    v.var_run = pr_f64(k, at);
}

__device__ __forceinline__ void service_write_obs(const SVars &v, const EnvParams &p, int64_t i, float *obs) {
    if (!obs) return;
    const int64_t n = p.n_lanes;
    ABR_OUT(obs[ABR_OBS_CHUNK_ID * n + i], (float)v.o_chunk);
    ABR_OUT(obs[ABR_OBS_LAST_BITRATE * n + i], (float)v.o_last);
    ABR_OUT(obs[ABR_OBS_LAST_BANDWIDTH * n + i], (float)v.last_bw);
    ABR_OUT(obs[ABR_OBS_BUFFER_LEVEL * n + i], (float)v.o_buf);
    ABR_OUT(obs[ABR_OBS_GLOBAL_TIME * n + i], (float)p.G[v.o_k]);
    ABR_OUT(obs[ABR_OBS_PLAY_TIME * n + i], (float)(p.lane_speeds ? v.o_pt : p.GP[v.o_nplay]));
    ABR_OUT(obs[ABR_OBS_REBUFFER_TIME * n + i], (float)p.G[v.o_nrb]);
    ABR_OUT(obs[ABR_OBS_STARTUP_TIME * n + i], (float)p.G[v.o_nsu]);
}

struct SplitKernargs {
    EnvParams p;
    const int32_t *actions;
    float *obs_out, *reward_out;
    uint8_t *done_out;
    int32_t *actions_out;
    int32_t n_steps;
    uint64_t seed;
    abrx::EpisodeSampler smp;
    abrx::EpisodeLedger led;
};
static_assert(offsetof(SplitKernargs, p) == 0 && offsetof(SplitKernargs, smp) == sizeof(EnvParams) + 56 &&
              offsetof(SplitKernargs, led) == sizeof(EnvParams) + 80 && sizeof(SplitKernargs) == sizeof(EnvParams) + 96,
              "the role-split kernels' kernarg segment (.offset of each argument in the code object's metadata)");
template <bool SAMPLE, bool VEC_PARAMS>
__device__ __forceinline__ void ledger_record_split(const EnvParams &p, int64_t i, double g_rb, double g_su, double lat,
                                                    double var_run, int32_t episode_no, int32_t chunks, uint8_t done) {
    auto kp = __builtin_amdgcn_kernarg_segment_ptr();
    asm volatile("" : "+v"(kp));
    const SplitKernargs &ka = *(const SplitKernargs *)kp;
    const EnvParams &pv = VEC_PARAMS ? ka.p : p;
    int32_t t = pv.trace_id[i], off = pv.offset0[i];
    if constexpr (SAMPLE) {
        if (episode_no != pv.episode_no[i]) sampled_episode(pv, ka.smp, i, episode_no, t, off);
    }
    ledger_record(pv, ka.led, i, g_rb, g_su, lat, var_run, episode_no, t, off, chunks, done);
}

template <bool SAMPLE = false, bool LEDGER = false, class M2>
__device__ __forceinline__ void service_record(SVars &v, const EnvParams &p, M2 &m2, int sl,
                                               float *__restrict__ obs_out, float *__restrict__ reward_out,
                                               uint8_t *__restrict__ done_out) {
    const int l = threadIdx.x & 63;
    const int64_t i = (int64_t)blockIdx.x * 64 + l;
    const int32_t m2m = m2.meta[sl][l];
    if (!(m2m & kS3Valid)) return;
    const int32_t step = m2.step[sl][l];
    const int64_t o = (int64_t)step * p.n_lanes + i;
    float *obs = obs_out ? obs_out + (int64_t)step * ABR_OBS_DIM * p.n_lanes : nullptr;
    const int32_t a = m2m & 0xff;
    v.s_next = step + 1;
    if (m2m & kS3Bad) {
        v.done |= ABR_DONE_BADACT;
        if (reward_out) ABR_OUT(reward_out[o], 0.0f);
        if (done_out) ABR_OUT(done_out[o], v.done);
        service_write_obs(v, p, i, obs);
        return;
    }
    const int32_t chunk = v.o_chunk, prev_action = v.o_last;
    const int32_t nrb_r = m2.nrb_r[sl][l], nsu_r = m2.nsu_r[sl][l];
    double var = 0.0;
    if (m2m & kS3Hit) {
        const double bw = m2.dl[sl][l] / p.G[m2.n_dl[sl][l]];
        const int64_t h = (int64_t)chunk * p.n_lanes + i;
        ABR_OUT(p.bw_hist[h], bw);
        ABR_OUT(p.action_hist[h], (uint8_t)a);
        v.last_bw = bw;
        v.hist_s = v.hist_s + 1.0 / bw;
        v.hist_n = v.hist_n + 1.0;
        if (prev_action >= 0)
            var = fabs(chunk_bitrate(p, chunk, a) - chunk_bitrate(p, chunk - 1, prev_action));
        v.var_run = v.var_run + var;
        v.o_last = a; v.o_chunk = chunk + 1;
    }
    const double g_rb = p.G[nrb_r], g_su = p.G[nsu_r];
    const double rew = p.wr * (g_rb - v.g_rb_obs) + p.ws * (g_su - v.g_su_obs) + p.wv * var;
    if (m2m & kS3Ended) v.done |= ABR_DONE_EPISODE;
    if (m2m & kS3Timeout) v.done |= ABR_DONE_TIMEOUT;
    if (reward_out) ABR_OUT(reward_out[o], (float)rew);
    if (done_out) ABR_OUT(done_out[o], v.done);
    v.n_su_obs = nsu_r; v.n_rb_obs = nrb_r; v.g_su_obs = g_su; v.g_rb_obs = g_rb;
    if (m2m & (kS3Ended | kS3Timeout)) {
        p.ep_qoe_terms[0 * p.n_lanes + i] = g_rb;
        p.ep_qoe_terms[1 * p.n_lanes + i] = g_su;
        p.ep_qoe_terms[2 * p.n_lanes + i] = m2.lat[sl][l];
        p.ep_qoe_terms[3 * p.n_lanes + i] = v.var_run;
        if constexpr (LEDGER)
            ledger_record_split<SAMPLE, true>(p, i, g_rb, g_su, m2.lat[sl][l], v.var_run, v.episode_no, v.o_chunk, v.done);
        if (m2m & kS3Reset) {
            v.episode_no++;
            v.n_su_obs = 0; v.n_rb_obs = 0; v.g_su_obs = 0.0; v.g_rb_obs = 0.0;
            v.last_bw = 0.0; v.hist_n = 0.0; v.hist_s = 0.0; v.var_run = 0.0;
            v.done = (m2m & kS3Timeout2) ? ABR_DONE_TIMEOUT : 0;
            v.o_chunk = 0; v.o_last = -1;
        }
    }
    v.o_buf = m2.buf[sl][l]; v.o_k = m2.k[sl][l]; v.o_nplay = m2.nplay_o[sl][l]; v.o_nrb = m2.nrb_o[sl][l];
    v.o_nsu = m2.nsu_o[sl][l];
    if (p.lane_speeds) v.o_pt = m2.pt[sl][l];
    service_write_obs(v, p, i, obs);
}

__device__ __forceinline__ void role_s_begin(SVars &v, const EnvParams &, ActRing &ring) {
    const EnvParams &p = fresh_params();
    const int l = threadIdx.x & 63;
    const int64_t i = (int64_t)blockIdx.x * 64 + l;
    v.last_bw = 0.0; v.hist_n = 0.0; v.hist_s = 0.0; v.g_su_obs = 0.0; v.g_rb_obs = 0.0; v.o_buf = 0.0; v.o_pt = 0.0; v.var_run = 0.0;
    v.o_chunk = 0; v.o_k = 0; v.o_nplay = 0; v.o_nrb = 0; v.o_nsu = 0; v.n_su_obs = 0; v.n_rb_obs = 0;
    v.episode_no = 0; v.s_next = 0; v.last_cb = 0; v.done = 0;
    v.o_last = -1; v.was_done = true;
    if (i < p.n_lanes) {
        v.done = p.done[i];
        v.was_done = v.done != 0;
        v.n_su_obs = p.n_su_obs[i]; v.n_rb_obs = p.n_rb_obs[i]; v.episode_no = p.episode_no[i];
        v.last_bw = p.last_bw[i]; v.hist_n = p.hist_n[i]; v.hist_s = p.hist_s[i]; v.var_run = p.var_run[i];
        v.g_su_obs = p.G[v.n_su_obs]; v.g_rb_obs = p.G[v.n_rb_obs];
        v.o_chunk = p.chunk_id[i]; v.o_last = p.last_action[i]; v.o_k = p.k[i]; v.o_nplay = p.n_play[i];
        v.o_nrb = p.n_rb[i]; v.o_nsu = p.n_su[i]; v.o_buf = p.buf[i];
        if (p.lane_speeds) v.o_pt = p.pt_lane[i];
    }
    v.a_next = 0; v.a_chunk = v.o_chunk; v.a_ep = v.episode_no;
    if (l == 0) lds_st(&ring.act_hi, 0);
    ABR_STAMP_INIT();
}

template <int MODE, bool SAMPLE = false, bool LEDGER = false>
__device__ __forceinline__ void role_s_pre(SVars &v, const EnvParams &, SplitMail &m, SplitMail2 &m2, ActRing &ring,
                                           float *__restrict__ obs_out, float *__restrict__ reward_out,
                                           uint8_t *__restrict__ done_out, int32_t n_total, uint64_t seed, int32_t t) {
    const EnvParams &p = fresh_params();
    const int l = threadIdx.x & 63;
    const int64_t i = (int64_t)blockIdx.x * 64 + l;
    const int cb = t & 1, pb = (t + 1) & 1;
    ABR_STAMP(20);
    if (MODE == 2) {
        int32_t lo = 0;
        if (t >= 1) {
            lo = m.fb_alive[pb][l] ? m.fb_step[pb][l] : 0x7fffffff;
#pragma unroll
            for (int sh = 32; sh >= 1; sh >>= 1) { const int32_t o2 = __shfl_xor(lo, sh, 64); lo = o2 < lo ? o2 : lo; }
            if (lo == 0x7fffffff) lo = n_total;
        }
        int32_t hi = lo + 60;
        if (hi > n_total) hi = n_total;
        const int32_t count = t == 0 ? 4 : 3;
        for (int32_t q = 0; q < count && v.a_next < hi; q++) {
            const uint32_t a = philox_action(seed, (uint64_t)(p.lane_id_base + i), (uint32_t)v.a_chunk, (uint32_t)v.a_ep,
                                             (uint32_t)p.n_rates);
            ring.act[v.a_next & 63][l] = (uint8_t)a;
            v.a_next++; v.a_chunk++;
            if (v.a_chunk >= p.video_length) { v.a_chunk = 0; v.a_ep++; }
        }
        lds_writes_done();
        if (l == 0) lds_st(&ring.act_hi, v.a_next);
    }
    if (t >= 1 && i < p.n_lanes) service_record<SAMPLE, LEDGER>(v, p, m2, pb, obs_out, reward_out, done_out);
    v.last_cb = cb;
    ABR_STAMP(21);
}

__device__ __forceinline__ void sampled_episode_store(const EnvParams &p, const abrx::EpisodeSampler &smp, int64_t i,
                                                      int32_t episode_no) {
    if (episode_no != p.episode_no[i]) {
        int32_t t, off;
        sampled_episode(p, smp, i, episode_no, t, off);
        p.trace_id[i] = t; p.offset0[i] = off;
    }
}

template <int MODE, bool SAMPLE = false, bool LEDGER = false>
__device__ __forceinline__ void role_s_end(SVars &v, const EnvParams &, SplitMail2 &m2, float *__restrict__ obs_out,
                                           float *__restrict__ reward_out, uint8_t *__restrict__ done_out,
                                           int32_t *__restrict__ actions_out, int32_t n_total,
                                           const abrx::EpisodeSampler &smp = abrx::EpisodeSampler{}) {
    const EnvParams &p = fresh_params();
    const int64_t i = (int64_t)blockIdx.x * 64 + (threadIdx.x & 63);
    ABR_STAMP_FLUSH();
    if (i >= p.n_lanes) return;
    service_record<SAMPLE, LEDGER>(v, p, m2, v.last_cb, obs_out, reward_out, done_out);
    if (!v.was_done) {
        if constexpr (SAMPLE) sampled_episode_store(p, smp, i, v.episode_no);
        p.n_su_obs[i] = v.n_su_obs; p.n_rb_obs[i] = v.n_rb_obs; p.episode_no[i] = v.episode_no;
        p.last_bw[i] = v.last_bw; p.hist_n[i] = v.hist_n; p.hist_s[i] = v.hist_s; p.var_run[i] = v.var_run;
        p.done[i] = v.done;
    }
    for (int32_t t2 = v.s_next; t2 < n_total; t2++) {
        const int64_t o = (int64_t)t2 * p.n_lanes + i;
        if (reward_out) reward_out[o] = 0.0f;
        if (done_out) done_out[o] = v.done;
        if (MODE == 2 && actions_out) actions_out[o] = -1;
        service_write_obs(v, p, i, obs_out ? obs_out + (int64_t)t2 * ABR_OBS_DIM * p.n_lanes : nullptr);
    }
}

template <int MODE, bool SAMPLE = false, bool LEDGER = false>
__global__ __launch_bounds__(192) __attribute__((amdgpu_waves_per_eu(1, 3))) void env_split3_kernel(
    EnvParams p, const int32_t *__restrict__ actions, float *__restrict__ obs_out,
    float *__restrict__ reward_out, uint8_t *__restrict__ done_out,
    int32_t *__restrict__ actions_out, int32_t n_steps, uint64_t seed, abrx::EpisodeSampler smp,
    abrx::EpisodeLedger led) {
    (void)led;
    __shared__ SplitMail m;
    __shared__ SplitMail2 m2;
    __shared__ ActRing ring;
    const int32_t n_total = (MODE >= 2) ? n_steps : 1;
    const int role = __builtin_amdgcn_readfirstlane((int)(threadIdx.x >> 6));
    if constexpr (MODE == 9) { selfcheck_answer(p); return; }
#ifdef ABR_SPLIT_STAMPS
    if (fresh_params().n_lanes != p.n_lanes || fresh_params().traces != p.traces) __builtin_trap();
#endif
    __shared__ RolePark3 park;
    DVars dv;
    role_d_begin(dv, p);
    if (role == 0) ABR_WG_TIME(0);
    ABR_WG_WHERE(role);
    if (role == 0) __builtin_amdgcn_s_setprio(ABR_PRIO_D);
    else if (role == 1) { __builtin_amdgcn_s_setprio(ABR_PRIO_P); PVars v; role_p3_begin(v, p); p_park(park.p, v); }
    else { __builtin_amdgcn_s_setprio(ABR_PRIO_S); SVars v; role_s_begin(v, p, ring); s_park(park.s, v); }
    for (int32_t t = 0;; t++) {
        if (role == 0) {
            if (t > 0) role_d_validate<SAMPLE>(dv, m, make_tables(p, ABR_SPLIT3_CASCADE != 0), t - 1);
            role_d_pre<MODE, true, SAMPLE>(dv, p, m, &ring, actions, actions_out, n_total, seed, t, smp);
        } else if (role == 1) {
            PVars v; p_unpark(park.p, v, p);
            role_p3_pre<MODE>(v, p, m, m2, n_total, t, t & 1);
            p_park(park.p, v);
        } else {
            SVars v; s_unpark(park.s, v);
            role_s_pre<MODE, SAMPLE, LEDGER>(v, p, m, m2, ring, obs_out, reward_out, done_out, n_total, seed, t);
            s_park(park.s, v);
        }
        __syncthreads();
        ABR_STAMP(role == 0 ? 5 : (role == 1 ? 18 : 22));
        if (!m.any_alive[t & 1]) break;
    }
    if (role == 0) { role_d_end(dv, p); ABR_WG_TIME(1); }
    else if (role == 1) { PVars v; p_unpark(park.p, v, p); role_p3_end(v, p); ABR_WG_TIME(2); }
    else { SVars v; s_unpark(park.s, v); role_s_end<MODE, SAMPLE, LEDGER>(v, p, m2, obs_out, reward_out, done_out, actions_out, n_total, smp); ABR_WG_TIME(3); }
}

struct P2Vars {
    PVars pv;
    double last_bw, hist_n, hist_s, g_su_obs, g_rb_obs, var_run;
    int32_t n_su_obs, n_rb_obs;
    uint8_t done;
};
__device__ __forceinline__ void p2_park(uint32_t (*area)[64], const P2Vars &v) {
    ParkWords k; k.n = 0;
    p_words(k, v.pv);
    pw_f64(k, v.last_bw); pw_f64(k, v.hist_n); pw_f64(k, v.hist_s); pw_f64(k, v.g_su_obs); pw_f64(k, v.g_rb_obs);
    pw_i32(k, v.n_su_obs); pw_i32(k, v.n_rb_obs); pw_i32(k, v.done);
    pw_f64(k, v.var_run); pw_i32(k, 0);
    park_store<10>(area, k);
}
__device__ __forceinline__ void p2_unpark(uint32_t (*area)[64], P2Vars &v, const EnvParams &p) {
    ParkWords k; park_load<10>(area, k);
    int at = 0;
    p_unwords(k, at, v.pv, p);
    v.last_bw = pr_f64(k, at); v.hist_n = pr_f64(k, at); v.hist_s = pr_f64(k, at); v.g_su_obs = pr_f64(k, at);
    v.g_rb_obs = pr_f64(k, at);
    v.n_su_obs = pr_i32(k, at); v.n_rb_obs = pr_i32(k, at); v.done = (uint8_t)pr_i32(k, at);
    v.var_run = pr_f64(k, at);
}

__device__ __forceinline__ void role_p2_begin(P2Vars &v, const EnvParams &) {
    const EnvParams &p = fresh_params();
    const int64_t i = (int64_t)blockIdx.x * 64 + (threadIdx.x & 63);
    player_clear(v.pv, p);
    v.last_bw = 0.0; v.hist_n = 0.0; v.hist_s = 0.0; v.g_su_obs = 0.0; v.g_rb_obs = 0.0; v.var_run = 0.0;
    v.n_su_obs = 0; v.n_rb_obs = 0; v.done = 0;
    if (i < p.n_lanes) {
        v.done = p.done[i];
        v.pv.was_done = v.done != 0;
        lanej_load(v.pv.s, p, i);
        v.n_su_obs = p.n_su_obs[i]; v.n_rb_obs = p.n_rb_obs[i]; v.pv.episode_no = p.episode_no[i];
        v.last_bw = p.last_bw[i]; v.hist_n = p.hist_n[i]; v.hist_s = p.hist_s[i]; v.var_run = p.var_run[i];
        v.g_su_obs = p.G[v.n_su_obs]; v.g_rb_obs = p.G[v.n_rb_obs];
        v.pv.b_alive = !v.done;
    }
    ABR_STAMP_INIT();
}

template <int MODE, bool SAMPLE = false, bool LEDGER = false>
__device__ __forceinline__ void role_p2_pre(P2Vars &v, const EnvParams &, SplitMail &m, float *__restrict__ obs_out,
                                            float *__restrict__ reward_out, uint8_t *__restrict__ done_out,
                                            int32_t n_total, int32_t t) {
    const EnvParams &p = fresh_params();
    const int l = threadIdx.x & 63;
    const int64_t i = (int64_t)blockIdx.x * 64 + l;
    const int cb = t & 1, pb = (t + 1) & 1;
    const abrx::Tables tb = make_tables(p);
    LaneJ &s = v.pv.s;
    ABR_STAMP(8);
    if (v.pv.b_alive && v.pv.b_step < n_total && t >= 1) {
        const int32_t fl = m.flags[pb][l];
        const int32_t r_step = m.step[pb][l], r_k = m.k_start[pb][l], r_a = m.action[pb][l], r_ndl = m.n_dl[pb][l],
                      r_avail = m.avail_next[pb][l];
        const double r_dl = m.dl[pb][l];
        if ((fl & kRecValid) && r_step == v.pv.b_step && r_k == s.k) {
            const int64_t o = (int64_t)v.pv.b_step * p.n_lanes + i;
            float *obs = obs_out ? obs_out + (int64_t)v.pv.b_step * ABR_OBS_DIM * p.n_lanes : nullptr;
            const int32_t a = r_a;
            if (fl & kRecBadAct) {
                v.done |= ABR_DONE_BADACT;
                if (reward_out) ABR_OUT(reward_out[o], 0.0f);
                if (done_out) ABR_OUT(done_out[o], (uint8_t)v.done);
                write_obs_j(s, p, i, obs, v.last_bw);
                v.pv.b_alive = false;
            } else {
                abrx::Download d;
                d.dl = r_dl; d.n_dl = r_ndl; d.hit = (fl & kRecHit) != 0;
                const int32_t prev_action = s.last_action;
                const int32_t chunk = s.chunk_id;
                ABR_STAMP(9);
                const abrx::StepResult sr = abrx::lanej_after_download(s, tb, d, r_avail, a);
                ABR_STAMP(13);
                const double g_rb = p.G[s.n_rb], g_su = p.G[s.n_su];
                double o_k = p.G[s.k], o_pl = p.lane_speeds ? s.pt : p.GP[s.n_play], o_rb = g_rb, o_su = g_su;
                double var = 0.0;
                if (sr.hit) {
                    const int64_t h = (int64_t)chunk * p.n_lanes + i;
                    ABR_OUT(p.bw_hist[h], sr.bw);
                    ABR_OUT(p.action_hist[h], (uint8_t)a);
                    v.last_bw = sr.bw;
                    v.hist_s = v.hist_s + 1.0 / sr.bw;
                    v.hist_n = v.hist_n + 1.0;
                    if (prev_action >= 0)
                        var = fabs(chunk_bitrate(p, chunk, a) - chunk_bitrate(p, chunk - 1, prev_action));
                    v.var_run = v.var_run + var;
                }
                const double rew = p.wr * (g_rb - v.g_rb_obs) + p.ws * (g_su - v.g_su_obs) + p.wv * var;
                if (sr.ended) v.done |= ABR_DONE_EPISODE;
                if (sr.timeout) v.done |= ABR_DONE_TIMEOUT;
                if (reward_out) ABR_OUT(reward_out[o], (float)rew);
                if (done_out) ABR_OUT(done_out[o], (uint8_t)v.done);
                v.n_su_obs = s.n_su; v.n_rb_obs = s.n_rb;
                v.g_su_obs = g_su; v.g_rb_obs = g_rb;
                ABR_STAMP(14);
                if (sr.ended || sr.timeout) {
                    p.ep_qoe_terms[0 * p.n_lanes + i] = g_rb;
                    p.ep_qoe_terms[1 * p.n_lanes + i] = g_su;
                    p.ep_qoe_terms[2 * p.n_lanes + i] = player_latency(p, s);
                    p.ep_qoe_terms[3 * p.n_lanes + i] = v.var_run;
                    if constexpr (LEDGER)
                        ledger_record_split<SAMPLE, false>(p, i, g_rb, g_su, player_latency(p, s), v.var_run, v.pv.episode_no, s.chunk_id, v.done);
                    if (p.auto_reset && sr.ended) {
                        abrx::lanej_init_player(s, tb);
                        v.pv.episode_no++;
                        v.n_su_obs = 0; v.n_rb_obs = 0; v.g_su_obs = 0.0; v.g_rb_obs = 0.0;
                        v.last_bw = 0.0; v.hist_n = 0.0; v.hist_s = 0.0; v.var_run = 0.0;
                        v.done = 0;
                        if (!abrx::lanej_wait_call(s, tb)) v.done |= ABR_DONE_TIMEOUT;
                        o_k = p.G[s.k]; o_pl = p.lane_speeds ? s.pt : p.GP[s.n_play];
                        o_rb = p.G[s.n_rb]; o_su = p.G[s.n_su];
                    }
                }
                ABR_STAMP(15);
                write_obs_vals(s, p, i, obs, v.last_bw, o_k, o_pl, o_rb, o_su);
                if (v.done) v.pv.b_alive = false;
                ABR_STAMP(16);
            }
            v.pv.b_step++;
        }
    }
    player_feedback(m, v.pv, n_total, cb);
    ABR_STAMP(17);
}

template <int MODE, bool SAMPLE = false>
__device__ __forceinline__ void role_p2_end(const P2Vars &v, const EnvParams &, float *__restrict__ obs_out,
                                            float *__restrict__ reward_out, uint8_t *__restrict__ done_out,
                                            int32_t *__restrict__ actions_out, int32_t n_total,
                                            const abrx::EpisodeSampler &smp = abrx::EpisodeSampler{}) {
    const EnvParams &p = fresh_params();
    const int64_t i = (int64_t)blockIdx.x * 64 + (threadIdx.x & 63);
    ABR_STAMP_FLUSH();
    if (i >= p.n_lanes) return;
    if (!v.pv.was_done) {
        if constexpr (SAMPLE) sampled_episode_store(p, smp, i, v.pv.episode_no);
        lanej_store_player(v.pv.s, p, i);
        p.n_su_obs[i] = v.n_su_obs; p.n_rb_obs[i] = v.n_rb_obs; p.episode_no[i] = v.pv.episode_no;
        p.last_bw[i] = v.last_bw; p.hist_n[i] = v.hist_n; p.hist_s[i] = v.hist_s; p.var_run[i] = v.var_run;
        p.done[i] = v.done;
    }
    for (int32_t t2 = v.pv.b_step; t2 < n_total; t2++) {
        const int64_t o = (int64_t)t2 * p.n_lanes + i;
        if (reward_out) ABR_OUT(reward_out[o], 0.0f);
        if (done_out) ABR_OUT(done_out[o], (uint8_t)v.done);
        if (MODE == 2 && actions_out) ABR_OUT(actions_out[o], (int32_t)-1);
        write_obs_j(v.pv.s, p, i, obs_out ? obs_out + (int64_t)t2 * ABR_OBS_DIM * p.n_lanes : nullptr, v.last_bw);
    }
}

template <int MODE, bool SAMPLE = false, bool LEDGER = false>
__global__ __launch_bounds__(128) void env_split_kernel(
    EnvParams p, const int32_t *__restrict__ actions, float *__restrict__ obs_out,
    float *__restrict__ reward_out, uint8_t *__restrict__ done_out,
    int32_t *__restrict__ actions_out, int32_t n_steps, uint64_t seed, abrx::EpisodeSampler smp,
    abrx::EpisodeLedger led) {
    (void)led;
    __shared__ SplitMail m;
    const int32_t n_total = (MODE >= 2) ? n_steps : 1;
    const int role = __builtin_amdgcn_readfirstlane((int)(threadIdx.x >> 6));
    if constexpr (MODE == 9) { selfcheck_answer(p); return; }
#ifdef ABR_SPLIT_STAMPS
    if (fresh_params().n_lanes != p.n_lanes || fresh_params().traces != p.traces) __builtin_trap();
#endif
    __shared__ RolePark2 park;
    DVars dv;
    role_d_begin(dv, p);
    if (role == 0) __builtin_amdgcn_s_setprio(2);
    else { P2Vars v; role_p2_begin(v, p); p2_park(park.p, v); }
    for (int32_t t = 0;; t++) {
        if (role == 0) {
            if (t > 0) role_d_validate<SAMPLE>(dv, m, make_tables(p), t - 1);
            role_d_pre<MODE, false, SAMPLE>(dv, p, m, nullptr, actions, actions_out, n_total, seed, t, smp);
        } else {
            P2Vars v; p2_unpark(park.p, v, fresh_params());
            role_p2_pre<MODE, SAMPLE, LEDGER>(v, p, m, obs_out, reward_out, done_out, n_total, t);
            p2_park(park.p, v);
        }
        __syncthreads();
        ABR_STAMP(role == 0 ? 5 : 18);
        if (!m.any_alive[t & 1]) break;
    }
    if (role == 0) role_d_end(dv, p);
    else { P2Vars v; p2_unpark(park.p, v, fresh_params()); role_p2_end<MODE, SAMPLE>(v, p, obs_out, reward_out, done_out, actions_out, n_total, smp); }
}

#endif
```

abrsimulator_amd/csrc/abr_lane_jump.h:

```cpp
#ifndef ABR_LANE_JUMP_H
#define ABR_LANE_JUMP_H

#include <math.h>

#include "abr_exact_jump.h"

#ifndef ABR_STAMP
#define ABR_STAMP(n)
#endif

namespace abrx {

constexpr double kTickDt = 0.01;
#ifndef ABR_K_DRAIN_TAIL
#define ABR_K_DRAIN_TAIL 16
#endif
constexpr int kPrologue = 16;
#ifndef ABR_PCHUNKS
#define ABR_PCHUNKS 12
#endif
#ifndef ABR_PCHECK
#define ABR_PCHECK 0x892
#endif
constexpr int kPChunks = ABR_PCHUNKS;
constexpr int kPCheck = ABR_PCHECK;

struct SpeedRule {
    int32_t n_lat, n_buf;
    double lat_thr[4], buf_thr[4];
    double speed[5][5];
};

ABR_HD double speed_rule_eval(const SpeedRule &r, double lat, double buf) {
    int32_t i = 0, j = 0;
    for (int32_t q = 0; q < r.n_lat; q++) i += lat >= r.lat_thr[q] ? 1 : 0;
    for (int32_t q = 0; q < r.n_buf; q++) j += buf >= r.buf_thr[q] ? 1 : 0;
    return r.speed[i][j];
}

constexpr int32_t kSpeedRowsRule = 0x7fffffff;

struct SpeedRuleBlock {
    SpeedRule rule;
    double *log;
    int32_t log_rows, reserved_;
};

struct Tables {
    const double *G;
    const int32_t *interval_tick;
    const int32_t *avail_tick;
    double L, sd, max_buffer, start_up_length;
    int32_t V, max_ticks;
    bool per_lane_speed;
    int32_t speed_rows;
    int64_t speed_stride;
    const double *speeds;
    const SpeedRuleBlock *rule = nullptr;
    DrainTab drain;
};

struct Cursor {
    int32_t j;
    int32_t tpos;
    int32_t tlen;
    const double *trace;
};

struct LaneJ {
    double buf;
    double sd;
    double pt;
    long long sumk;
    int32_t k, chunk_id, n_su, n_rb, n_play, avail_k, last_action;
    bool su, be, bf;
    Cursor cur;
    int32_t pl_left, play_id;
    double pt_sum;
    int64_t lane;
};

ABR_HD void cursor_init(Cursor &c, int32_t offset0) {
    c.j = 0;
    c.tpos = offset0 % c.tlen;
}

ABR_HD void lanej_init_player(LaneJ &s, const Tables &t) {
    s.buf = 0.0; s.sumk = 0;
    s.k = 0; s.chunk_id = 0; s.n_su = 1; s.n_rb = 0; s.n_play = 0;
    s.last_action = -1;
    s.su = true; s.be = true; s.bf = false;
    s.avail_k = t.avail_tick[0];
    s.pt = 0.0;
    s.pl_left = 0; s.play_id = 0; s.pt_sum = 0.0;
}

ABR_HD void lanej_init(LaneJ &s, const Tables &t, int32_t offset0) {
    lanej_init_player(s, t);
    cursor_init(s.cur, offset0);
}

ABR_HD void lanej_play(LaneJ &s, const Tables &t, int32_t a) {
    if (!t.per_lane_speed || a <= 0) return;
    int32_t done = 0;
    double x = s.pt;
    chain<STOP_GE>(x, s.sd, 1.0e300, a, done);
    s.pt = x;
}

constexpr int kDrainTail = ABR_K_DRAIN_TAIL;
ABR_HD bool drain_to_zero(double &b_io, double sd, int32_t m, int32_t &a_out) {
    ChainState cs;
    cs.x = b_io; cs.eb = -1;
    const double tail = (double)kDrainTail * sd;
    int32_t a = 0;
    bool below = false;
    while (a < m && !below) a += chain_segment<STOP_LE>(cs, -sd, tail, m - a, below);
    double b = cs.x;
    ABR_STAMP(24);
#ifdef ABR_DRAIN_HOOK
    const int32_t a_seg = a;
#endif
#if defined(__HIP_DEVICE_COMPILE__)
#pragma unroll 1
#endif
    while (a < m && b > 0.0) { b = b - sd; a++; }
    ABR_STAMP(25);
#ifdef ABR_DRAIN_HOOK
    ABR_DRAIN_HOOK(a > 0 && b <= 0.0, a - a_seg);
#endif
    b_io = b; a_out = a;
    return a > 0 && b <= 0.0;
}

ABR_HD bool lanej_drain(const Tables &t, double &b_io, double sd, int32_t m, int32_t &a_out) {
    if (t.drain.n > 0 && !wave_any(!(b_io < t.drain.top))) {
        const bool zero = drain_cascade(t.drain, sd, b_io, m, a_out);
        ABR_STAMP(24);
        return zero;
    }
    return drain_to_zero(b_io, sd, m, a_out);
}

ABR_HD void sched_begin_chunk(LaneJ &s, const Tables &t, int32_t k, double b) {
    double v;
    if (t.speed_rows == kSpeedRowsRule) {
#if defined(__HIP_DEVICE_COMPILE__) && defined(ABR_RULE_KERNARG_OFFSET)
        auto kp = __builtin_amdgcn_kernarg_segment_ptr();
        asm volatile("" : "+s"(kp));
        const SpeedRuleBlock &rb = *(const SpeedRuleBlock *)((const char *)kp + ABR_RULE_KERNARG_OFFSET);
#else
        const SpeedRuleBlock &rb = *t.rule;
#endif
        v = speed_rule_eval(rb.rule, t.G[k] - s.pt, b);
        if (s.play_id < rb.log_rows) rb.log[(int64_t)s.play_id * t.speed_stride + s.lane] = v;
    } else {
        const int32_t row = s.play_id < t.speed_rows ? s.play_id : t.speed_rows - 1;
        v = t.speeds[(int64_t)row * t.speed_stride + s.lane];
    }
    s.sd = v * kTickDt;
    double x = 0.0;
    int32_t a = 0;
    chain<STOP_GE>(x, s.sd, t.L, t.max_ticks + 1, a);
    s.pl_left = a > 0 ? a : 1;
}

ABR_HD void sched_played(LaneJ &s, const Tables &t, int32_t a) {
    if (a <= 0) return;
    s.pt_sum += (double)a * s.pt + s.sd * (double)(((long long)a * (a - 1)) / 2);
    int32_t done = 0;
    double x = s.pt;
    chain<STOP_GE>(x, s.sd, 1.0e300, a, done);
    s.pt = x;
    s.pl_left -= a;
    if (s.pl_left == 0) s.play_id++;
}

template <int STOP>
ABR_HD bool sched_drain(LaneJ &s, const Tables &t, double &b, double thr, int32_t m, int32_t &a_out) {
    int32_t a_tot = 0;
    bool hit = false;
    while (a_tot < m && !hit) {
        if (s.pl_left == 0) sched_begin_chunk(s, t, s.k + a_tot, b);
        const int32_t run = (m - a_tot < s.pl_left) ? m - a_tot : s.pl_left;
        int32_t a = 0;
        if (STOP == STOP_LE) hit = drain_to_zero(b, s.sd, run, a);
        else hit = chain<STOP_LT>(b, -s.sd, thr, run, a);
        sched_played(s, t, a);
        a_tot += a;
    }
    a_out = a_tot;
    return hit;
}

ABR_HD void lanej_idle(LaneJ &s, const Tables &t, int32_t m) {
    if (m <= 0) return;
    if (s.su && s.buf >= t.start_up_length) s.su = false;
    ABR_STAMP(23);
    if (s.su) {
        s.n_su += m;
    } else if (s.be) {
        s.n_rb += m;
    } else {
        int32_t a = 0;
        double b = s.buf;
        bool zero;
        if (t.speed_rows >= 2) zero = sched_drain<STOP_LE>(s, t, b, 0.0, m, a);
        else { zero = lanej_drain(t, b, s.sd, m, a); lanej_play(s, t, a); }
        s.n_play += a;
        s.sumk += (long long)a * s.k + ((long long)a * (a - 1)) / 2;
        if (zero) { b = 0.0; s.be = true; s.n_rb += (m - a + 1); }
        s.buf = b;
        s.bf = b >= t.max_buffer;
    }
    s.k += m;
}

ABR_HD bool lanej_wait_call(LaneJ &s, const Tables &t) {
    const int32_t mt = t.max_ticks;
    if (s.k >= s.avail_k && !s.bf) return true;
    int32_t w = s.avail_k - s.k;
    if (w < 0) w = 0;
    if (w > mt - s.k) w = mt - s.k;
    lanej_idle(s, t, w);
    if (s.k >= mt) return false;
    if (s.bf) {
        if (s.su || s.be) {
            if (s.su) s.n_su += mt - s.k; else s.n_rb += mt - s.k;
            s.k = mt;
            return false;
        }
        int32_t a = 0;
        double b = s.buf;
        bool cleared;
        if (t.speed_rows >= 2) cleared = sched_drain<STOP_LT>(s, t, b, t.max_buffer, mt - s.k, a);
        else { cleared = chain<STOP_LT>(b, -s.sd, t.max_buffer, mt - s.k, a); lanej_play(s, t, a); }
        s.n_play += a;
        s.sumk += (long long)a * s.k + ((long long)a * (a - 1)) / 2;
        s.k += a;
        s.be = b <= 0.0;
        if (s.be) { b = 0.0; s.n_rb += 1; }
        s.buf = b;
        s.bf = !cleared;
        if (!cleared) return false;
    }
    return true;
}

struct StepResult {
    double bw;
    bool hit;
    bool ended;
    bool timeout;
};

constexpr int kCatch = 4;
struct StepStart {
    double c;
    double bw_next;
    int32_t ke;
    int32_t ke_next;
    int32_t tn;
    int32_t avail_next;
};

ABR_HD int32_t trace_wrap(int32_t pos, int32_t tlen) {
    if (pos >= tlen) pos -= tlen;
    if (pos >= tlen) pos %= tlen;
    return pos;
}

struct StepLoads {
    int32_t ke[kCatch + 2];
    double bw[kCatch + 2];
    int32_t avail_next;
};

ABR_HD StepLoads lanej_begin_load(const Cursor &s, const Tables &t, int32_t chunk_id) {
    StepLoads ld;
#if defined(__HIP_DEVICE_COMPILE__)
#pragma unroll
#endif
    for (int i = 0; i < kCatch + 2; i++) {
        ld.ke[i] = t.interval_tick[s.j + 1 + i];
        ld.bw[i] = s.trace[trace_wrap(s.tpos + i, s.tlen)];
    }
    ld.avail_next = t.avail_tick[chunk_id + 1];
    return ld;
}

ABR_HD StepStart lanej_begin_select(Cursor &s, const Tables &t, const StepLoads &ld, int32_t k) {
    const int32_t *ke = ld.ke;
    const double *bw = ld.bw;
    StepStart st;
    st.avail_next = ld.avail_next;
    int32_t adv = 0;
#if defined(__HIP_DEVICE_COMPILE__)
#pragma unroll
#endif
    for (int i = 0; i < kCatch; i++) adv += (k >= ke[i]) ? 1 : 0;
    if (adv == kCatch && k >= ke[kCatch]) {
        s.j += kCatch; s.tpos = trace_wrap(s.tpos + kCatch, s.tlen);
        int32_t e = t.interval_tick[s.j + 1];
        while (k >= e && e != 0x7fffffff) {
            s.j++;
            s.tpos = (s.tpos + 1 == s.tlen) ? 0 : s.tpos + 1;
            e = t.interval_tick[s.j + 1];
        }
        st.ke = e; st.ke_next = t.interval_tick[s.j + 2];
        st.tn = (s.tpos + 1 == s.tlen) ? 0 : s.tpos + 1;
        st.c = s.trace[s.tpos] * kTickDt; st.bw_next = s.trace[st.tn];
        return st;
    }
    double c_bw = bw[0], n_bw = bw[1];
    int32_t c_ke = ke[0], n_ke = ke[1];
#if defined(__HIP_DEVICE_COMPILE__)
#pragma unroll
#endif
    for (int i = 1; i <= kCatch; i++) {
        const bool pick = adv == i;
        c_bw = pick ? bw[i] : c_bw; n_bw = pick ? bw[i + 1] : n_bw;
        c_ke = pick ? ke[i] : c_ke; n_ke = pick ? ke[i + 1] : n_ke;
    }
    s.j += adv;
    s.tpos = trace_wrap(s.tpos + adv, s.tlen);
    st.c = c_bw * kTickDt; st.bw_next = n_bw; st.ke = c_ke; st.ke_next = n_ke;
    st.tn = (s.tpos + 1 == s.tlen) ? 0 : s.tpos + 1;
    return st;
}

ABR_HD StepStart lanej_begin_step(Cursor &s, const Tables &t, int32_t k, int32_t chunk_id) {
    const StepLoads ld = lanej_begin_load(s, t, chunk_id);
    return lanej_begin_select(s, t, ld, k);
}

struct Download {
    double dl;
    int32_t n_dl;
    bool hit;
};

ABR_HD Download lanej_download(Cursor &s, const Tables &t, const StepStart &st, int32_t k,
                               double target) {
    const int32_t mt = t.max_ticks;
    int32_t ke = st.ke < mt ? st.ke : mt, ke_next = st.ke_next, tn = st.tn;
    double c = st.c, bw_next = st.bw_next;
    ChainState cs;
    cs.x = 0.0; cs.eb = -1;
    int32_t kk = k;
    bool hit = false;
    {
        const int32_t left = ke - kk;
        const int32_t n1 = left > 0 ? left : 0;
        const int32_t a = n1 & 7, q1 = n1 >> 3;
        const double c2 = bw_next * kTickDt;
        const int32_t room2 = (ke_next < mt ? ke_next : mt) - ke;
        double x = 0.0, xb = 0.0;
        int32_t T = 0;
#if defined(__HIP_DEVICE_COMPILE__)
#pragma unroll
#endif
        for (int i = 0; i < 7; i++) x = (i < a) ? x + c : x;
#if defined(__HIP_DEVICE_COMPILE__)
#pragma unroll
#endif
        for (int q = 0; q < kPChunks; q++) {
            const double cq = (q < q1) ? c : c2;
#if defined(__HIP_DEVICE_COMPILE__)
#pragma unroll
#endif
            for (int i = 0; i < 8; i++) x = x + cq;
            if ((kPCheck >> q) & 1) {
                const int32_t Tq = a + 8 * (q + 1);
                const bool ok = (x < target) & ((Tq <= n1) | (Tq - n1 < room2));
                xb = ok ? x : xb;
                T = ok ? Tq : T;
            }
        }
        cs.x = xb;
        const bool crossed = T > n1;
        kk += T;
        c = crossed ? c2 : c;
        ke = crossed ? (ke_next < mt ? ke_next : mt) : ke;
        s.j += crossed ? 1 : 0;
        s.tpos = crossed ? tn : s.tpos;
    }
    while (!hit && kk < mt) {
        const bool adv = kk >= ke;
        c = adv ? bw_next * kTickDt : c;
        ke = adv ? (ke_next < mt ? ke_next : mt) : ke;
        s.j += adv ? 1 : 0;
        s.tpos = adv ? tn : s.tpos;
        cs.eb = adv ? -1 : cs.eb;
        tn = (s.tpos + 1 == s.tlen) ? 0 : s.tpos + 1;
        bw_next = s.trace[(uint32_t)tn];
        ke_next = t.interval_tick[(uint32_t)(s.j + 2)];
        kk += chain_segment<STOP_GE>(cs, c, target, ke - kk, hit);
    }
    Download d;
    d.dl = cs.x; d.n_dl = kk - k; d.hit = hit;
    return d;
}

ABR_HD StepResult lanej_after_download(LaneJ &s, const Tables &t, const Download &d,
                                       int32_t avail_next, int32_t action) {
    StepResult r;
    r.bw = 0.0; r.hit = false; r.ended = false; r.timeout = false;
    const int32_t mt = t.max_ticks;
    const bool hit = d.hit;
    const int32_t n_dl = d.n_dl;
    const double g_ndl = t.G[n_dl];
    lanej_idle(s, t, hit ? n_dl - 1 : n_dl);
    ABR_STAMP(10);
    if (!hit) { r.timeout = true; return r; }
    const bool playing = !(s.be || s.su);
    double b = s.buf + t.L;
    if (playing) {
        s.sumk += s.k; s.n_play++;
        if (t.speed_rows >= 2) {
            if (s.pl_left == 0) sched_begin_chunk(s, t, s.k, b);
            b = b - s.sd;
            sched_played(s, t, 1);
        } else { b = b - s.sd; lanej_play(s, t, 1); }
    }
    s.bf = b >= t.max_buffer;
    s.be = b <= 0.0;
    if (s.be) b = 0.0;
    s.buf = b;
    s.su = s.su && !(b >= t.start_up_length);
    s.k++;
    r.hit = true;
    r.bw = d.dl / g_ndl;
    s.last_action = action;
    s.chunk_id++;
    s.avail_k = avail_next;
    r.ended = s.chunk_id >= t.V;
    r.timeout = !r.ended && s.k >= mt;
    ABR_STAMP(11);
    if (!r.ended && !r.timeout) {
        s.n_su += s.su ? 1 : 0;
        s.n_rb += (!s.su && s.be) ? 1 : 0;
        r.timeout = !lanej_wait_call(s, t);
    }
    ABR_STAMP(12);
    return r;
}

ABR_HD bool lanej_gate_possible(double buf, bool su, bool be, int32_t n_dl, const Tables &t) {
    return !su && !be && !t.per_lane_speed && (buf + t.L) - (double)n_dl * t.sd >= t.max_buffer - 1.0e-6;
}
ABR_HD bool lanej_predict_next_call(double buf, int32_t k, int32_t n_dl, int32_t avail_next, const Tables &t,
                                    int32_t &k_next, double *buf_next = nullptr) {
    const int32_t mt = t.max_ticks;
    double b = buf;
    int32_t a = 0;
    if (n_dl > 1 && lanej_drain(t, b, t.sd, n_dl - 1, a)) return false;
    b = b + t.L;
    b = b - t.sd;
    if (b <= 0.0) return false;
    bool bf = b >= t.max_buffer;
    k += n_dl;
    if (k >= mt) return false;
    if (!(k >= avail_next && !bf)) {
        int32_t w = avail_next - k;
        if (w < 0) w = 0;
        if (w > mt - k) w = mt - k;
        if (w > 0) {
            if (lanej_drain(t, b, t.sd, w, a)) return false;
            bf = b >= t.max_buffer;
            k += w;
        }
        if (k >= mt) return false;
        if (bf) {
            a = 0;
            if (!chain<STOP_LT>(b, -t.sd, t.max_buffer, mt - k, a)) return false;
            k += a;
            if (b <= 0.0) return false;
        }
    }
    k_next = k;
    if (buf_next) *buf_next = b;
    return true;
}

ABR_HD StepResult lanej_download_and_wait(LaneJ &s, const Tables &t, const StepStart &st,
                                          double target, int32_t action) {
    const Download d = lanej_download(s.cur, t, st, s.k, target);
    return lanej_after_download(s, t, d, st.avail_next, action);
}

ABR_HD StepResult lanej_step(LaneJ &s, const Tables &t, double target, int32_t action) {
    const StepStart st = lanej_begin_step(s.cur, t, s.k, s.chunk_id);
    return lanej_download_and_wait(s, t, st, target, action);
}

enum { kRuleBuffer = 1, kRuleRate = 2, kRuleBola = 3, kRuleFastMpc = 4 };

struct RuleParams {
    int32_t kind, window;
    double reservoir, cushion;
    double safety;
    double bola_v, bola_gp;
    const double *utility;
    const uint8_t *fm_table;
    int32_t fm_uniform;
    int32_t fm_horizon, fm_nb, fm_nq;
};

template <class BR>
ABR_HD int32_t rule_hi(const BR &br, int32_t M, double X) {
    int32_t a = 0;
    for (int32_t m = 1; m < M; m++) a = br(m) <= X ? m : a;
    return a;
}

template <class BR>
ABR_HD int32_t rule_buffer(const RuleParams &r, const BR &br, int32_t M, double B) {
    if (B <= r.reservoir) return 0;
    if (B >= r.reservoir + r.cushion) return M - 1;
    const double lo = br(0);
    return rule_hi(br, M, lo + ((B - r.reservoir) / r.cushion) * (br(M - 1) - lo));
}

template <class HIST>
ABR_HD double harmonic_tail(const HIST &hist, int32_t c, int32_t n) {
    double S = 0.0;
    for (int32_t j = c - n; j < c; j++) S = S + 1.0 / hist(j);
    return (double)n / S;
}

template <class BR, class HIST>
ABR_HD int32_t rule_rate(const RuleParams &r, const BR &br, const HIST &hist, int32_t M, int32_t c) {
    const int32_t n = r.window < c ? r.window : c;
    if (n <= 0) return 0;
    return rule_hi(br, M, r.safety * harmonic_tail(hist, c, n));
}

template <class BR>
ABR_HD int32_t rule_bola(const RuleParams &r, const BR &br, int32_t M, int32_t c, double B) {
    const double *u = r.utility + (int64_t)c * M;
    double best = (r.bola_v * (u[0] + r.bola_gp) - B) / br(0);
    int32_t a = 0;
    for (int32_t m = 1; m < M; m++) {
        const double sc = (r.bola_v * (u[m] + r.bola_gp) - B) / br(m);
        a = sc > best ? m : a;
        best = sc > best ? sc : best;
    }
    return a;
}

template <class BR, class HIST>
ABR_HD int32_t rule_select(const RuleParams &r, const BR &br, const HIST &hist, int32_t M, int32_t c, double B) {
    if (r.kind == kRuleBuffer) return rule_buffer(r, br, M, B);
    if (r.kind == kRuleRate) return rule_rate(r, br, hist, M, c);
    return rule_bola(r, br, M, c, B);
}

ABR_HD int32_t fastmpc_cell(const double *e, int32_t n, double x) {
    int32_t lo = 0, hi = n;
    while (lo < hi) {
        const int32_t mid = (lo + hi) >> 1;
        if (e[mid] <= x) lo = mid + 1;
        else hi = mid;
    }
    return lo;
}

ABR_HD int64_t fastmpc_entry_bytes(int32_t n_rows, int32_t M, int32_t nb, int32_t nq) {
    return (((int64_t)n_rows * M * nb * nq) + 7) & ~(int64_t)7;
}

template <class HIST>
ABR_HD int32_t fastmpc_lookup(const RuleParams &r, const HIST &hist, int32_t M, int32_t V, int32_t c, int32_t pv,
                              double B) {
    if (c < 0 || c >= V || pv < -M || pv >= M) return -1;
    const int32_t n = r.window < c ? r.window : c;
    if (n <= 0) return 0;
    const double P = harmonic_tail(hist, c, n);
    if (pv < 0) pv += M;
    const int32_t row = r.fm_uniform ? ((V - c < r.fm_horizon ? V - c : r.fm_horizon) - 1) : c;
    const int32_t rows = r.fm_uniform ? r.fm_horizon : V;
    const double *be = (const double *)(r.fm_table + fastmpc_entry_bytes(rows, M, r.fm_nb, r.fm_nq));
    const double *te = be + (r.fm_nb - 1);
    const int32_t bi = fastmpc_cell(be, r.fm_nb - 1, B);
    const int32_t qi = fastmpc_cell(te, r.fm_nq - 1, P);
    return r.fm_table[(((int64_t)row * M + pv) * r.fm_nb + bi) * r.fm_nq + qi];
}

template <class BR, class HIST>
ABR_HD int32_t rule_select_at(const RuleParams &r, const BR &br, const HIST &hist, int32_t M, int32_t V, int32_t c,
                              int32_t pv, double B) {
    if (r.kind == kRuleFastMpc) return fastmpc_lookup(r, hist, M, V, c, pv, B);
    return rule_select(r, br, hist, M, c, B);
}

template <class HIST, class ERR>
ABR_HD double robust_estimate(int32_t W, int32_t c, const HIST &hist, int32_t &cs1, int32_t &cnt, double &ps,
                              const ERR &err) {
    if (cnt < 0 || cnt > W) cnt = 0;
    if (cs1 > 0 && (int64_t)cs1 == (int64_t)c) {
        const double hc = hist(c - 1);
        const double e = fabs(ps - hc) / hc;
        if (cnt < W) {
            err(cnt) = e;
            cnt = cnt + 1;
        } else {
            for (int32_t k = 1; k < W; k++) err(k - 1) = err(k);
            err(W - 1) = e;
        }
    } else if (!(cs1 > 0 && (int64_t)cs1 == (int64_t)c + 1)) {
        cnt = 0;
    }
    const int32_t n = W < c ? W : c;
    if (n <= 0) {
        cs1 = 0; cnt = 0; ps = 0.0;
        return 0.0;
    }
    const double hm = harmonic_tail(hist, c, n);
    double E = 0.0;
    if (cnt > 0) {
        E = err(0);
        for (int32_t k = 1; k < cnt; k++) E = err(k) > E ? err(k) : E;
    }
    const double P = hm / (1.0 + E);
    if (!(hm > 0.0 && hm <= 1.79769313486231570815e+308)) {
        cs1 = 0; cnt = 0; ps = 0.0;
        return 0.0;
    }
    ps = hm;
    cs1 = c + 1;
    return P > 0.0 ? P : 0.0;
}


constexpr int kPolicyMaxWindow = 16, kPolicyMaxWidth = 64, kPolicyMaxRates = 16;
constexpr int kPolicyMaxF = 4 + kPolicyMaxWindow + kPolicyMaxRates;

struct PolicyNet {
    int32_t window, n_hidden, w0, w1, M, F;
    const double *norm;
    uint64_t seed, thr;
};

ABR_HD void philox4(uint64_t seed, uint64_t lane, uint32_t step, uint32_t episode, uint32_t out[4]) {
// ... 397 lines not shown
```

Before: 12.30 billion.

## Specialize env kernels at compile time for lanes without per-lane playback speeds

Adds a SPEEDS template parameter threaded through the tables, lane load/store, the step helpers and the split mailbox layouts. When no per-lane speeds are configured, the speed-schedule state (pt, pl_left, play_id, pt_sum) and its branches compile away, cutting register pressure, shared memory and global traffic. Host dispatch picks the specialization at run time. It also adds a separate launch-bounds knob for mode 1 and makes split kernels' fresh-parameter handling configurable, at the cost of more kernel instantiations.

After: 12.69 billion (median of 6 runs). 1.03x the previous value.

```diff
diff --git a/abrsimulator_amd/csrc/abr_env.hip b/abrsimulator_amd/csrc/abr_env.hip
--- a/abrsimulator_amd/csrc/abr_env.hip
+++ b/abrsimulator_amd/csrc/abr_env.hip
@@ -280,7 +280,7 @@
                         chunks, (int32_t)done);
 }
 
-template <int MODE, bool SAMPLE = false, bool LEDGER = false>
+template <int MODE, bool SAMPLE = false, bool LEDGER = false, bool SPEEDS = false>
 __global__ __launch_bounds__(64) void env_advance_kernel(
     EnvParams p, const int32_t *__restrict__ actions, const int32_t *__restrict__ trace_id_in,
     const int32_t *__restrict__ offset_in, const uint8_t *__restrict__ lane_mask,
@@ -289,6 +289,7 @@
     abrx::EpisodeSampler smp, abrx::EpisodeLedger led) {
     const int64_t i = (int64_t)blockIdx.x * 64 + threadIdx.x;
     const bool in_range = i < p.n_lanes;
+    static_assert(!SPEEDS, "the tick kernel takes no per-lane speeds");
     const int32_t n_total = (MODE >= 2) ? n_steps : 1;
     Lane s;
     bool active = in_range;
@@ -501,23 +502,47 @@
 
 using abrx::LaneJ;
 
-__device__ inline abrx::Tables make_tables(const EnvParams &p, bool cascade = true) {
-    abrx::Tables t;
+template <bool SPEEDS>
+struct SpeedParams;
+template <>
+struct SpeedParams<true> {
+    static __device__ __forceinline__ const double *lane_speeds(const EnvParams &p) { return p.lane_speeds; }
+    static __device__ __forceinline__ int32_t speed_rows(const EnvParams &p) { return p.speed_rows; }
+    static __device__ __forceinline__ double *sd_lane(const EnvParams &p) { return p.sd_lane; }
+    static __device__ __forceinline__ double *pt_lane(const EnvParams &p) { return p.pt_lane; }
+    static __device__ __forceinline__ double *pt_sum(const EnvParams &p) { return p.pt_sum; }
+    static __device__ __forceinline__ int32_t *pl_left(const EnvParams &p) { return p.pl_left; }
+    static __device__ __forceinline__ int32_t *play_id(const EnvParams &p) { return p.play_id; }
+};
+template <>
+struct SpeedParams<false> {
+    static __device__ __forceinline__ constexpr const double *lane_speeds(const EnvParams &) { return nullptr; }
+    static __device__ __forceinline__ constexpr int32_t speed_rows(const EnvParams &) { return 1; }
+};
+
+template <bool SPEEDS = true>
+__device__ inline abrx::TablesT<SPEEDS> make_tables(const EnvParams &p, bool cascade = true) {
+    abrx::TablesT<SPEEDS> t;
     t.G = p.G; t.interval_tick = p.interval_tick; t.avail_tick = p.avail_tick;
     t.L = p.chunk_length; t.sd = p.sd; t.max_buffer = p.max_buffer;
     t.start_up_length = p.start_up_length; t.V = p.video_length; t.max_ticks = p.max_ticks;
-    t.per_lane_speed = p.lane_speeds != nullptr;
-    t.speed_rows = p.lane_speeds ? p.speed_rows : 0;
-    t.speed_stride = p.n_lanes; t.speeds = p.lane_speeds;
+    using SP = SpeedParams<SPEEDS>;
+    if constexpr (SPEEDS) {
+        t.per_lane_speed = SP::lane_speeds(p) != nullptr;
+        t.speed_rows = SP::lane_speeds(p) ? SP::speed_rows(p) : 0;
+        t.speed_stride = p.n_lanes; t.speeds = SP::lane_speeds(p);
+    }
     t.drain = p.drain;
-    if (p.lane_speeds || !cascade) t.drain.n = 0;
+    if (SP::lane_speeds(p) || !cascade) t.drain.n = 0;
 #ifdef ABR_NO_DRAIN_CASCADE
     t.drain.n = 0;
 #endif
     return t;
 }
 
+template <bool SPEEDS = true>
 __device__ inline void lanej_load(LaneJ &s, const EnvParams &p, int64_t i) {
+    using SP = SpeedParams<SPEEDS>;
     s.buf = p.buf[i]; s.sumk = p.sumk[i];
     s.k = p.k[i]; s.chunk_id = p.chunk_id[i]; s.n_su = p.n_su[i]; s.n_rb = p.n_rb[i];
     s.n_play = p.n_play[i]; s.cur.j = p.j[i]; s.cur.tpos = p.tpos[i];
@@ -526,19 +551,27 @@
     s.su = f & kFlagStartUp; s.be = f & kFlagBufEmpty; s.bf = f & kFlagBufFull;
     const int32_t c = s.chunk_id < p.video_length ? s.chunk_id : p.video_length;
     s.avail_k = p.avail_tick[c];
-    if (p.lane_speeds) { s.sd = p.sd_lane[i]; s.pt = p.pt_lane[i]; } else { s.sd = p.sd; s.pt = 0.0; }
-    s.lane = i; s.pl_left = 0; s.play_id = 0; s.pt_sum = 0.0;
-    if (p.lane_speeds && p.speed_rows >= 2) { s.pl_left = p.pl_left[i]; s.play_id = p.play_id[i]; s.pt_sum = p.pt_sum[i]; }
-}
-
+    if constexpr (SPEEDS) {
+        if (SP::lane_speeds(p)) { s.sd = SP::sd_lane(p)[i]; s.pt = SP::pt_lane(p)[i]; } else { s.sd = p.sd; s.pt = 0.0; }
+        s.lane = i; s.pl_left = 0; s.play_id = 0; s.pt_sum = 0.0;
+        if (SP::lane_speeds(p) && SP::speed_rows(p) >= 2) { s.pl_left = SP::pl_left(p)[i]; s.play_id = SP::play_id(p)[i]; s.pt_sum = SP::pt_sum(p)[i]; }
+    } else {
+        s.sd = p.sd; s.lane = i;
+    }
+}
+
+template <bool SPEEDS = true>
 __device__ inline void lanej_store(const LaneJ &s, const EnvParams &p, int64_t i) {
     p.buf[i] = s.buf; p.sumk[i] = s.sumk;
     p.k[i] = s.k; p.chunk_id[i] = s.chunk_id; p.n_su[i] = s.n_su; p.n_rb[i] = s.n_rb;
     p.n_play[i] = s.n_play; p.j[i] = s.cur.j; p.tpos[i] = s.cur.tpos; p.last_action[i] = s.last_action;
     p.flags[i] = (uint8_t)((s.su ? kFlagStartUp : 0) | (s.be ? kFlagBufEmpty : 0) |
                            (s.bf ? kFlagBufFull : 0) | kFlagArmed);
-    if (p.lane_speeds) { p.sd_lane[i] = s.sd; p.pt_lane[i] = s.pt; }
-    if (p.lane_speeds && p.speed_rows >= 2) { p.pl_left[i] = s.pl_left; p.play_id[i] = s.play_id; p.pt_sum[i] = s.pt_sum; }
+    if constexpr (SPEEDS) {
+        using SP = SpeedParams<SPEEDS>;
+        if (SP::lane_speeds(p)) { SP::sd_lane(p)[i] = s.sd; SP::pt_lane(p)[i] = s.pt; }
+        if (SP::lane_speeds(p) && SP::speed_rows(p) >= 2) { SP::pl_left(p)[i] = s.pl_left; SP::play_id(p)[i] = s.play_id; SP::pt_sum(p)[i] = s.pt_sum; }
+    }
 }
 
 #ifndef ABR_NO_NT_STORES
@@ -547,6 +580,7 @@
 #define ABR_OUT(ref, val) ((ref) = (val))
 #endif
 
+template <bool SPEEDS = true>
 __device__ inline void write_obs_j(const LaneJ &s, const EnvParams &p, int64_t i, float *obs,
                                    double last_bw) {
     if (!obs) return;
@@ -556,7 +590,7 @@
     ABR_OUT(obs[ABR_OBS_LAST_BANDWIDTH * n + i], (float)last_bw);
     ABR_OUT(obs[ABR_OBS_BUFFER_LEVEL * n + i], (float)s.buf);
     ABR_OUT(obs[ABR_OBS_GLOBAL_TIME * n + i], (float)p.G[s.k]);
-    ABR_OUT(obs[ABR_OBS_PLAY_TIME * n + i], (float)(p.lane_speeds ? s.pt : p.GP[s.n_play]));
+    ABR_OUT(obs[ABR_OBS_PLAY_TIME * n + i], (float)(SpeedParams<SPEEDS>::lane_speeds(p) ? s.pt : p.GP[s.n_play]));
     ABR_OUT(obs[ABR_OBS_REBUFFER_TIME * n + i], (float)p.G[s.n_rb]);
     ABR_OUT(obs[ABR_OBS_STARTUP_TIME * n + i], (float)p.G[s.n_su]);
 }
@@ -578,8 +612,12 @@
 #ifndef ABR_JUMP_WAVES
 #define ABR_JUMP_WAVES 5
 #endif
-#define ABR_JUMP_BOUNDS(MODE, SAMPLE) __launch_bounds__(64, ((MODE) == 1 || (MODE) == 4 || (SAMPLE) ? 4 : ABR_JUMP_WAVES))
-template <int MODE, bool SAMPLE = false, bool LEDGER = false>
+#ifndef ABR_JUMP_WAVES_ONE
+#define ABR_JUMP_WAVES_ONE 4
+#endif
+#define ABR_JUMP_BOUNDS(MODE, SAMPLE) \
+    __launch_bounds__(64, ((MODE) == 1 ? ABR_JUMP_WAVES_ONE : ((MODE) == 4 || (SAMPLE)) ? 4 : ABR_JUMP_WAVES))
+template <int MODE, bool SAMPLE = false, bool LEDGER = false, bool SPEEDS = true>
 __global__ ABR_JUMP_BOUNDS(MODE, SAMPLE || LEDGER) void env_jump_kernel(
     EnvParams p, const int32_t *__restrict__ actions, const int32_t *__restrict__ trace_id_in,
     const int32_t *__restrict__ offset_in, const uint8_t *__restrict__ lane_mask,
@@ -589,7 +627,8 @@
     const int64_t i = (int64_t)blockIdx.x * 64 + threadIdx.x;
     const bool in_range = i < p.n_lanes;
     const int32_t n_total = (MODE >= 2) ? n_steps : 1;
-    const abrx::Tables tb = make_tables(p);
+    const abrx::TablesT<SPEEDS> tb = make_tables<SPEEDS>(p);
+    using SP = SpeedParams<SPEEDS>;
     LaneJ s;
     bool active = in_range, touched = in_range;
     uint8_t done = 0;
@@ -613,18 +652,18 @@
                 episode_no = (p.flags[i] & kFlagArmed) ? p.episode_no[i] + 1 : 0;
                 p.trace_id[i] = t; p.offset0[i] = offset0;
                 s.cur.tlen = p.trace_len[t]; s.cur.trace = p.traces + p.trace_off[t];
-                s.sd = (p.lane_speeds && p.speed_rows != abrx::kSpeedRowsRule) ? p.lane_speeds[i] * kDt : p.sd;
+                s.sd = (SP::lane_speeds(p) && SP::speed_rows(p) != abrx::kSpeedRowsRule) ? SP::lane_speeds(p)[i] * kDt : p.sd;
                 s.lane = i;
                 abrx::lanej_init(s, tb, offset0);
                 if (!bad && !abrx::lanej_wait_call(s, tb)) done |= ABR_DONE_TIMEOUT;
-                write_obs_j(s, p, i, obs_out, 0.0);
+                write_obs_j<SPEEDS>(s, p, i, obs_out, 0.0);
             }
         } else {
             done = p.done[i];
             const int32_t t = p.trace_id[i];
             offset0 = p.offset0[i];
             s.cur.tlen = p.trace_len[t]; s.cur.trace = p.traces + p.trace_off[t];
-            lanej_load(s, p, i);
+            lanej_load<SPEEDS>(s, p, i);
             n_su_obs = p.n_su_obs[i]; n_rb_obs = p.n_rb_obs[i]; episode_no = p.episode_no[i];
             last_bw = p.last_bw[i]; hist_n = p.hist_n[i]; hist_s = p.hist_s[i]; var_run = p.var_run[i];
             g_su_obs = p.G[n_su_obs]; g_rb_obs = p.G[n_rb_obs];
@@ -651,7 +690,7 @@
                     done |= ABR_DONE_BADACT;
                     if (reward_out) ABR_OUT(reward_out[o], 0.0f);
                     if (done_out) ABR_OUT(done_out[o], (uint8_t)done);
-                    write_obs_j(s, p, i, obs, last_bw);
+                    write_obs_j<SPEEDS>(s, p, i, obs, last_bw);
                     active = false;
                 } else {
                     const int32_t prev_action = s.last_action;
@@ -659,7 +698,7 @@
                     const abrx::StepResult r = abrx::lanej_download_and_wait(
                         s, tb, st, chunk_bitrate(p, chunk, a) * p.chunk_length , a);
                     const double g_rb = p.G[s.n_rb], g_su = p.G[s.n_su];
-                    double o_k = p.G[s.k], o_pl = p.lane_speeds ? s.pt : p.GP[s.n_play], o_rb = g_rb, o_su = g_su;
+                    double o_k = p.G[s.k], o_pl = SP::lane_speeds(p) ? s.pt : p.GP[s.n_play], o_rb = g_rb, o_su = g_su;
                     double var = 0.0;
                     if (r.hit) {
                         const int64_t h = (int64_t)chunk * p.n_lanes + i;
@@ -683,9 +722,9 @@
                         p.ep_qoe_terms[0 * p.n_lanes + i] = g_rb;
                         p.ep_qoe_terms[1 * p.n_lanes + i] = g_su;
                         p.ep_qoe_terms[2 * p.n_lanes + i] =
-                            !p.lane_speeds ? lane_avg_latency(p, s.sumk, s.n_play)
-                            : (p.speed_rows >= 2 ? avg_latency_sched(s.pt, s.sumk, s.pt_sum, s.n_play)
-                                                 : avg_latency_from(s.sd, s.pt, s.sumk, s.n_play));
+                            !SP::lane_speeds(p) ? lane_avg_latency(p, s.sumk, s.n_play)
+                            : (SP::speed_rows(p) >= 2 ? avg_latency_sched(s.pt, s.sumk, s.pt_sum, s.n_play)
+                                                    : avg_latency_from(s.sd, s.pt, s.sumk, s.n_play));
                         p.ep_qoe_terms[3 * p.n_lanes + i] = var_run;
                         if constexpr (LEDGER)
                             ledger_record(p, led, i, g_rb, g_su, p.ep_qoe_terms[2 * p.n_lanes + i], var_run, episode_no,
@@ -703,7 +742,7 @@
                             last_bw = 0.0; hist_n = 0.0; hist_s = 0.0; var_run = 0.0;
                             done = 0;
                             if (!abrx::lanej_wait_call(s, tb)) done |= ABR_DONE_TIMEOUT;
-                            o_k = p.G[s.k]; o_pl = p.lane_speeds ? s.pt : p.GP[s.n_play];
+                            o_k = p.G[s.k]; o_pl = SP::lane_speeds(p) ? s.pt : p.GP[s.n_play];
                             o_rb = p.G[s.n_rb]; o_su = p.G[s.n_su];
                         }
                     }
@@ -714,13 +753,13 @@
                 if (reward_out) ABR_OUT(reward_out[o], 0.0f);
                 if (done_out) ABR_OUT(done_out[o], (uint8_t)done);
                 if ((MODE == 2 || MODE == 4) && actions_out) ABR_OUT(actions_out[o], (int32_t)-1);
-                write_obs_j(s, p, i, obs, last_bw);
+                write_obs_j<SPEEDS>(s, p, i, obs, last_bw);
             }
         }
     }
 
     if (touched) {
-        lanej_store(s, p, i);
+        lanej_store<SPEEDS>(s, p, i);
         p.n_su_obs[i] = n_su_obs; p.n_rb_obs[i] = n_rb_obs; p.episode_no[i] = episode_no;
         p.last_bw[i] = last_bw; p.hist_n[i] = hist_n; p.hist_s[i] = hist_s; p.var_run[i] = var_run;
         p.done[i] = done;
@@ -1230,7 +1269,7 @@
     return effective_impl(env, n_steps > 1);
 }
 
-template <int MODE, bool SAMPLE, bool LEDGER>
+template <int MODE, bool SAMPLE, bool LEDGER, bool SPEEDS>
 static void launch_env_kernels(const abr_env *env, int impl, hipStream_t st, const int32_t *actions, float *obs, float *rew,
                                uint8_t *dn, int32_t *acts, int32_t n_steps, uint64_t seed, const abrx::RuleParams &rule,
                                const int32_t *trace_id, const int32_t *start_offset, const uint8_t *lane_mask) {
@@ -1238,20 +1277,24 @@
     const int64_t N = p.n_lanes;
     const abrx::EpisodeSampler smp = SAMPLE ? env->sampler : abrx::EpisodeSampler{};
     const abrx::EpisodeLedger led = LEDGER ? env->ledger : abrx::EpisodeLedger{};
-    if (impl == 0 || impl == 1) {
-        auto *k = impl == 1 ? env_advance_kernel<MODE, SAMPLE, LEDGER> : env_jump_kernel<MODE, SAMPLE, LEDGER>;
+    if (impl == 0) {
+        auto *k = env_jump_kernel<MODE, SAMPLE, LEDGER, SPEEDS>;
+        hipLaunchKernelGGL(k, dim3(grid64(N)), dim3(64), 0, st, p, actions, trace_id, start_offset, lane_mask, obs, rew, dn,
+                           acts, n_steps, seed, rule, smp, led);
+    } else if (impl == 1) {
+        auto *k = env_advance_kernel<MODE, SAMPLE, LEDGER, false>;
         hipLaunchKernelGGL(k, dim3(grid64(N)), dim3(64), 0, st, p, actions, trace_id, start_offset, lane_mask, obs, rew, dn,
                            acts, n_steps, seed, rule, smp, led);
     } else if constexpr (MODE >= 1 && MODE <= 3) {
         if (impl == 5) {
-            auto *k = env_split3_kernel<MODE, SAMPLE, LEDGER>;
+            auto *k = env_split3_kernel<MODE, SAMPLE, LEDGER, SPEEDS>;
             hipLaunchKernelGGL(k, dim3(grid64(N)), dim3(192), 0, st, p, actions, obs, rew, dn, acts, n_steps, seed, smp, led);
         } else if (impl == 2) {
-            auto *k = env_split_kernel<MODE, SAMPLE, LEDGER>;
+            auto *k = env_split_kernel<MODE, SAMPLE, LEDGER, SPEEDS>;
             hipLaunchKernelGGL(k, dim3(grid64(N)), dim3(128), 0, st, p, actions, obs, rew, dn, acts, n_steps, seed, smp, led);
         }
 #ifdef ABR_WITH_RING
-        else if constexpr (!SAMPLE && !LEDGER) {
+        else if constexpr (!SAMPLE && !LEDGER && SPEEDS) {
             if (impl == 6)
                 hipLaunchKernelGGL(env_ring3_kernel<MODE>, dim3(grid64(N)), dim3(64 * ABR_RING_WAVES), 0, st, p, actions, obs,
                                    rew, dn, acts, n_steps, seed);
@@ -1293,9 +1336,20 @@
     }
 #endif
     const bool ledger = MODE != 0 && env->ledger.base;
+    const bool speeds_on = env->p.lane_speeds != nullptr;
     const auto go = [&](auto smp_on, auto led_on) {
-        launch_env_kernels<MODE, decltype(smp_on)::value, decltype(led_on)::value>(
-            env, impl, st, actions, obs, rew, dn, acts, n_steps, seed, rule, trace_id, start_offset, lane_mask);
+        constexpr bool kSample = decltype(smp_on)::value;
+        constexpr bool kLedger = decltype(led_on)::value;
+        if constexpr (kSample) {
+            launch_env_kernels<MODE, true, kLedger, true>(
+                env, impl, st, actions, obs, rew, dn, acts, n_steps, seed, rule, trace_id, start_offset, lane_mask);
+        } else if (speeds_on || impl == 6 || impl == 7) {
+            launch_env_kernels<MODE, false, kLedger, true>(
+                env, impl, st, actions, obs, rew, dn, acts, n_steps, seed, rule, trace_id, start_offset, lane_mask);
+        } else {
+            launch_env_kernels<MODE, false, kLedger, false>(
+                env, impl, st, actions, obs, rew, dn, acts, n_steps, seed, rule, trace_id, start_offset, lane_mask);
+        }
     };
     if constexpr (MODE == 0) {
         if (sample) go(std::true_type{}, std::false_type{});
diff --git a/abrsimulator_amd/csrc/abr_env_roles.h b/abrsimulator_amd/csrc/abr_env_roles.h
--- a/abrsimulator_amd/csrc/abr_env_roles.h
+++ b/abrsimulator_amd/csrc/abr_env_roles.h
@@ -4,6 +4,9 @@
 
 #ifndef ABR_SPLIT3_CASCADE
 #define ABR_SPLIT3_CASCADE 0
+#endif
+#ifndef ABR_S_FRESH_PARAMS
+#define ABR_S_FRESH_PARAMS 1
 #endif
 #ifndef ABR_PRIO_D
 #define ABR_PRIO_D 2
@@ -29,11 +32,17 @@
 };
 constexpr int kRecValid = 1, kRecHit = 2, kRecBadAct = 4;
 
-struct SplitMail2 {
-    double dl[2][64], buf[2][64], lat[2][64], pt[2][64];
+struct SplitMail2Head { double dl[2][64], buf[2][64], lat[2][64]; };
+template <bool SPEEDS> struct SplitMail2Pt { double pt[2][64]; };
+template <> struct SplitMail2Pt<false> {};
+struct SplitMail2Tail {
     int32_t meta[2][64], step[2][64], n_dl[2][64], k[2][64], nplay_o[2][64], nrb_o[2][64], nsu_o[2][64],
         nrb_r[2][64], nsu_r[2][64];
 };
+template <bool SPEEDS> struct SplitMail2T : SplitMail2Head, SplitMail2Pt<SPEEDS>, SplitMail2Tail {};
+using SplitMail2 = SplitMail2T<true>;
+static_assert(sizeof(SplitMail2T<true>) == sizeof(SplitMail2T<false>) + sizeof(double) * 2 * 64, "the forms differ by `pt` alone");
+template <bool SPEEDS> struct SplitMail2Of { using type = SplitMail2T<SPEEDS>; };
 constexpr int kS3Valid = 0x10000, kS3Hit = 0x100, kS3Bad = 0x200, kS3Ended = 0x400, kS3Timeout = 0x800,
               kS3Reset = 0x1000, kS3Timeout2 = 0x2000;
 
@@ -64,8 +73,12 @@
     }
 }
 
-struct RolePark3 { uint32_t p[24][64], s[32][64]; };
-struct RolePark2 { uint32_t p[40][64]; };
+template <bool SPEEDS = true>
+struct RolePark3T { uint32_t p[SPEEDS ? 24 : 16][64], s[32][64]; };
+template <bool SPEEDS = true>
+struct RolePark2T { uint32_t p[SPEEDS ? 40 : 32][64]; };
+using RolePark3 = RolePark3T<true>;
+using RolePark2 = RolePark2T<true>;
 
 struct ParkWords {
     uint32_t w[40];
@@ -97,14 +110,18 @@
     k.n = 0;
 }
 
+template <bool SPEEDS = true>
 __device__ inline void lanej_store_player(const LaneJ &s, const EnvParams &p, int64_t i) {
     p.buf[i] = s.buf; p.sumk[i] = s.sumk;
     p.k[i] = s.k; p.chunk_id[i] = s.chunk_id; p.n_su[i] = s.n_su; p.n_rb[i] = s.n_rb;
     p.n_play[i] = s.n_play; p.last_action[i] = s.last_action;
     p.flags[i] = (uint8_t)((s.su ? kFlagStartUp : 0) | (s.be ? kFlagBufEmpty : 0) |
                            (s.bf ? kFlagBufFull : 0) | kFlagArmed);
-    if (p.lane_speeds) { p.sd_lane[i] = s.sd; p.pt_lane[i] = s.pt; }
-    if (p.lane_speeds && p.speed_rows >= 2) { p.pl_left[i] = s.pl_left; p.play_id[i] = s.play_id; p.pt_sum[i] = s.pt_sum; }
+    if constexpr (SPEEDS) {
+        using SP = SpeedParams<SPEEDS>;
+        if (SP::lane_speeds(p)) { SP::sd_lane(p)[i] = s.sd; SP::pt_lane(p)[i] = s.pt; }
+        if (SP::lane_speeds(p) && SP::speed_rows(p) >= 2) { SP::pl_left(p)[i] = s.pl_left; SP::play_id(p)[i] = s.play_id; SP::pt_sum(p)[i] = s.pt_sum; }
+    }
 }
 
 struct DVars {
@@ -133,7 +150,7 @@
     ABR_STAMP_INIT();
 }
 
-template <int MODE, bool ACT_RING, bool SAMPLE = false>
+template <int MODE, bool ACT_RING, bool SAMPLE = false, bool SPEEDS = true>
 __device__ __forceinline__ void role_d_pre(DVars &v, const EnvParams &p, SplitMail &m, ActRing *ring,
                                            const int32_t *__restrict__ actions, int32_t *__restrict__ actions_out,
                                            int32_t n_total, uint64_t seed, int32_t t,
@@ -142,7 +159,7 @@
     const int64_t i = (int64_t)blockIdx.x * 64 + l;
     const int32_t V = p.video_length;
     const int cb = t & 1;
-    const abrx::Tables tb = make_tables(p);
+    const abrx::TablesT<SPEEDS> tb = make_tables<SPEEDS>(p);
     int32_t flags = 0;
     ABR_STAMP(0);
     if (v.d_alive && v.d_step < n_total) {
@@ -199,8 +216,8 @@
     ABR_STAMP(4);
 }
 
-template <bool SAMPLE = false>
-__device__ __forceinline__ void role_d_validate(DVars &v, SplitMail &m, const abrx::Tables &tb, int32_t t) {
+template <bool SAMPLE = false, class TB>
+__device__ __forceinline__ void role_d_validate(DVars &v, SplitMail &m, const TB &tb, int32_t t) {
     const int l = threadIdx.x & 63;
     const int cb = t & 1;
     int32_t f_alive = m.fb_alive[cb][l], f_step = m.fb_step[cb][l], f_k = m.fb_k[cb][l], f_pf = m.fb_pf[cb][l];
@@ -240,21 +257,29 @@
     int32_t episode_no, b_step;
     bool b_alive, was_done;
 };
+template <bool SPEEDS = true>
 __device__ __forceinline__ void p_words(ParkWords &k, const PVars &v) {
     const LaneJ &s = v.s;
-    pw_f64(k, s.buf); pw_f64(k, s.sd); pw_f64(k, s.pt); pw_f64(k, s.pt_sum); pw_i64(k, s.sumk);
+    pw_f64(k, s.buf);
+    if constexpr (SPEEDS) { pw_f64(k, s.sd); pw_f64(k, s.pt); pw_f64(k, s.pt_sum); }
+    pw_i64(k, s.sumk);
     pw_i32(k, s.k); pw_i32(k, s.chunk_id); pw_i32(k, s.n_su); pw_i32(k, s.n_rb); pw_i32(k, s.n_play);
-    pw_i32(k, s.avail_k); pw_i32(k, s.last_action); pw_i32(k, s.pl_left); pw_i32(k, s.play_id);
+    pw_i32(k, s.avail_k); pw_i32(k, s.last_action);
+    if constexpr (SPEEDS) { pw_i32(k, s.pl_left); pw_i32(k, s.play_id); }
     pw_i32(k, (s.su ? 1 : 0) | (s.be ? 2 : 0) | (s.bf ? 4 : 0) | (v.b_alive ? 8 : 0) | (v.was_done ? 16 : 0));
     pw_i32(k, v.episode_no); pw_i32(k, v.b_step);
     pw_i32(k, 0); pw_i32(k, 0);
 }
+template <bool SPEEDS = true>
 __device__ __forceinline__ void p_unwords(const ParkWords &k, int &at, PVars &v, const EnvParams &p) {
     LaneJ &s = v.s;
-    s.buf = pr_f64(k, at); s.sd = pr_f64(k, at); s.pt = pr_f64(k, at); s.pt_sum = pr_f64(k, at); s.sumk = pr_i64(k, at);
+    s.buf = pr_f64(k, at);
+    if constexpr (SPEEDS) { s.sd = pr_f64(k, at); s.pt = pr_f64(k, at); s.pt_sum = pr_f64(k, at); }
+    else s.sd = p.sd;
+    s.sumk = pr_i64(k, at);
     s.k = pr_i32(k, at); s.chunk_id = pr_i32(k, at); s.n_su = pr_i32(k, at); s.n_rb = pr_i32(k, at);
-    s.n_play = pr_i32(k, at); s.avail_k = pr_i32(k, at); s.last_action = pr_i32(k, at); s.pl_left = pr_i32(k, at);
-    s.play_id = pr_i32(k, at);
+    s.n_play = pr_i32(k, at); s.avail_k = pr_i32(k, at); s.last_action = pr_i32(k, at);
+    if constexpr (SPEEDS) { s.pl_left = pr_i32(k, at); s.play_id = pr_i32(k, at); }
     const int32_t fl = pr_i32(k, at);
     s.su = fl & 1; s.be = fl & 2; s.bf = fl & 4; v.b_alive = fl & 8; v.was_done = fl & 16;
     v.episode_no = pr_i32(k, at); v.b_step = pr_i32(k, at);
@@ -262,21 +287,25 @@
     s.cur.j = 0; s.cur.tpos = 0; s.cur.tlen = 1; s.cur.trace = p.traces;
     s.lane = (int64_t)blockIdx.x * 64 + (threadIdx.x & 63);
 }
+template <bool SPEEDS = true>
 __device__ __forceinline__ void p_park(uint32_t (*area)[64], const PVars &v) {
     ParkWords k; k.n = 0;
-    p_words(k, v);
-    park_store<6>(area, k);
-}
+    p_words<SPEEDS>(k, v);
+    park_store<SPEEDS ? 6 : 4>(area, k);
+}
+template <bool SPEEDS = true>
 __device__ __forceinline__ void p_unpark(uint32_t (*area)[64], PVars &v, const EnvParams &p) {
-    ParkWords k; park_load<6>(area, k);
+    ParkWords k; park_load<SPEEDS ? 6 : 4>(area, k);
     int at = 0;
-    p_unwords(k, at, v, p);
-}
-
+    p_unwords<SPEEDS>(k, at, v, p);
+}
+
+template <bool SPEEDS = true>
 __device__ __forceinline__ double player_latency(const EnvParams &p, const LaneJ &s) {
-    return !p.lane_speeds ? lane_avg_latency(p, s.sumk, s.n_play)
-           : (p.speed_rows >= 2 ? avg_latency_sched(s.pt, s.sumk, s.pt_sum, s.n_play)
-                                : avg_latency_from(s.sd, s.pt, s.sumk, s.n_play));
+    using SP = SpeedParams<SPEEDS>;
+    return !SP::lane_speeds(p) ? lane_avg_latency(p, s.sumk, s.n_play)
+           : (SP::speed_rows(p) >= 2 ? avg_latency_sched(s.pt, s.sumk, s.pt_sum, s.n_play)
+                                   : avg_latency_from(s.sd, s.pt, s.sumk, s.n_play));
 }
 
 __device__ __forceinline__ void player_feedback(SplitMail &m, const PVars &v, int32_t n_total, int cb) {
@@ -299,25 +328,27 @@
     v.episode_no = 0; v.b_step = 0; v.b_alive = false; v.was_done = true;
 }
 
+template <bool SPEEDS = true>
 __device__ __forceinline__ void role_p3_begin(PVars &v, const EnvParams &p) {
     const int64_t i = (int64_t)blockIdx.x * 64 + (threadIdx.x & 63);
     player_clear(v, p);
     if (i < p.n_lanes) {
         v.was_done = p.done[i] != 0;
-        lanej_load(v.s, p, i);
+        lanej_load<SPEEDS>(v.s, p, i);
         v.episode_no = p.episode_no[i];
         v.b_alive = !v.was_done;
     }
     ABR_STAMP_INIT();
 }
 
-template <int MODE, class M2>
+template <int MODE, bool SPEEDS = true, class M2>
 __device__ __forceinline__ void role_p3_pre(PVars &v, const EnvParams &p, SplitMail &m, M2 &m2,
                                             int32_t n_total, int32_t t, int cb2) {
     const int l = threadIdx.x & 63;
     const int cb = t & 1, pb = (t + 1) & 1;
-    const abrx::Tables tb = make_tables(p, ABR_SPLIT3_CASCADE != 0);
-    const bool speeds = p.lane_speeds != nullptr;
+    const abrx::TablesT<SPEEDS> tb = make_tables<SPEEDS>(p, ABR_SPLIT3_CASCADE != 0);
+    const bool speeds = SpeedParams<SPEEDS>::lane_speeds(p) != nullptr;
+    (void)speeds;
     LaneJ &s = v.s;
     int32_t meta = 0;
     ABR_STAMP(8);
@@ -344,7 +375,7 @@
                 m2.dl[cb2][l] = d.dl; m2.n_dl[cb2][l] = d.n_dl;
                 m2.nrb_r[cb2][l] = s.n_rb; m2.nsu_r[cb2][l] = s.n_su;
                 if (sr.ended || sr.timeout) {
-                    m2.lat[cb2][l] = player_latency(p, s);
+                    m2.lat[cb2][l] = player_latency<SPEEDS>(p, s);
                     if (p.auto_reset && sr.ended) {
                         abrx::lanej_init_player(s, tb);
                         v.episode_no++;
@@ -354,7 +385,7 @@
                 }
                 m2.buf[cb2][l] = s.buf; m2.k[cb2][l] = s.k; m2.nplay_o[cb2][l] = s.n_play;
                 m2.nrb_o[cb2][l] = s.n_rb; m2.nsu_o[cb2][l] = s.n_su;
-                if (speeds) m2.pt[cb2][l] = s.pt;
+                if constexpr (SPEEDS) { if (speeds) m2.pt[cb2][l] = s.pt; }
             }
             v.b_step++;
         }
@@ -365,10 +396,11 @@
     ABR_STAMP(17);
 }
 
+template <bool SPEEDS = true>
 __device__ __forceinline__ void role_p3_end(const PVars &v, const EnvParams &p) {
     const int64_t i = (int64_t)blockIdx.x * 64 + (threadIdx.x & 63);
     ABR_STAMP_FLUSH();
-    if (i < p.n_lanes && !v.was_done) lanej_store_player(v.s, p, i);
+    if (i < p.n_lanes && !v.was_done) lanej_store_player<SPEEDS>(v.s, p, i);
 }
 
 struct SVars {
@@ -382,10 +414,11 @@
     uint8_t done;
     bool was_done;
 };
+template <bool SPEEDS = true>
 __device__ __forceinline__ void s_park(uint32_t (*area)[64], const SVars &v) {
     ParkWords k; k.n = 0;
     pw_f64(k, v.last_bw); pw_f64(k, v.hist_n); pw_f64(k, v.hist_s); pw_f64(k, v.g_su_obs); pw_f64(k, v.g_rb_obs);
-    pw_f64(k, v.o_buf); pw_f64(k, v.o_pt);
+    pw_f64(k, v.o_buf); pw_f64(k, SPEEDS ? v.o_pt : 0.0);
     pw_i32(k, v.o_chunk); pw_i32(k, v.o_last); pw_i32(k, v.o_k); pw_i32(k, v.o_nplay); pw_i32(k, v.o_nrb);
     pw_i32(k, v.o_nsu); pw_i32(k, v.n_su_obs); pw_i32(k, v.n_rb_obs); pw_i32(k, v.episode_no); pw_i32(k, v.s_next);
     pw_i32(k, v.a_next); pw_i32(k, v.a_chunk); pw_i32(k, v.a_ep); pw_i32(k, v.last_cb);
@@ -393,11 +426,13 @@
     pw_f64(k, v.var_run); pw_i32(k, 0);
     park_store<8>(area, k);
 }
+template <bool SPEEDS = true>
 __device__ __forceinline__ void s_unpark(uint32_t (*area)[64], SVars &v) {
     ParkWords k; park_load<8>(area, k);
     int at = 0;
     v.last_bw = pr_f64(k, at); v.hist_n = pr_f64(k, at); v.hist_s = pr_f64(k, at); v.g_su_obs = pr_f64(k, at);
-    v.g_rb_obs = pr_f64(k, at); v.o_buf = pr_f64(k, at); v.o_pt = pr_f64(k, at);
+    v.g_rb_obs = pr_f64(k, at); v.o_buf = pr_f64(k, at);
+    if constexpr (SPEEDS) v.o_pt = pr_f64(k, at); else { v.o_pt = 0.0; at += 2; }
     v.o_chunk = pr_i32(k, at); v.o_last = pr_i32(k, at); v.o_k = pr_i32(k, at); v.o_nplay = pr_i32(k, at);
     v.o_nrb = pr_i32(k, at); v.o_nsu = pr_i32(k, at); v.n_su_obs = pr_i32(k, at); v.n_rb_obs = pr_i32(k, at);
     v.episode_no = pr_i32(k, at); v.s_next = pr_i32(k, at); v.a_next = pr_i32(k, at); v.a_chunk = pr_i32(k, at);
@@ -407,6 +442,7 @@
     v.var_run = pr_f64(k, at);
 }
 
+template <bool SPEEDS = true>
 __device__ __forceinline__ void service_write_obs(const SVars &v, const EnvParams &p, int64_t i, float *obs) {
     if (!obs) return;
     const int64_t n = p.n_lanes;
@@ -415,7 +451,7 @@
     ABR_OUT(obs[ABR_OBS_LAST_BANDWIDTH * n + i], (float)v.last_bw);
     ABR_OUT(obs[ABR_OBS_BUFFER_LEVEL * n + i], (float)v.o_buf);
     ABR_OUT(obs[ABR_OBS_GLOBAL_TIME * n + i], (float)p.G[v.o_k]);
-    ABR_OUT(obs[ABR_OBS_PLAY_TIME * n + i], (float)(p.lane_speeds ? v.o_pt : p.GP[v.o_nplay]));
+    ABR_OUT(obs[ABR_OBS_PLAY_TIME * n + i], (float)(SpeedParams<SPEEDS>::lane_speeds(p) ? v.o_pt : p.GP[v.o_nplay]));
     ABR_OUT(obs[ABR_OBS_REBUFFER_TIME * n + i], (float)p.G[v.o_nrb]);
     ABR_OUT(obs[ABR_OBS_STARTUP_TIME * n + i], (float)p.G[v.o_nsu]);
 }
@@ -448,7 +484,7 @@
     ledger_record(pv, ka.led, i, g_rb, g_su, lat, var_run, episode_no, t, off, chunks, done);
 }
 
-template <bool SAMPLE = false, bool LEDGER = false, class M2>
+template <bool SAMPLE = false, bool LEDGER = false, bool SPEEDS = true, class M2>
 __device__ __forceinline__ void service_record(SVars &v, const EnvParams &p, M2 &m2, int sl,
                                                float *__restrict__ obs_out, float *__restrict__ reward_out,
                                                uint8_t *__restrict__ done_out) {
@@ -465,7 +501,7 @@
         v.done |= ABR_DONE_BADACT;
         if (reward_out) ABR_OUT(reward_out[o], 0.0f);
         if (done_out) ABR_OUT(done_out[o], v.done);
-        service_write_obs(v, p, i, obs);
+        service_write_obs<SPEEDS>(v, p, i, obs);
         return;
     }
     const int32_t chunk = v.o_chunk, prev_action = v.o_last;
@@ -508,12 +544,13 @@
     }
     v.o_buf = m2.buf[sl][l]; v.o_k = m2.k[sl][l]; v.o_nplay = m2.nplay_o[sl][l]; v.o_nrb = m2.nrb_o[sl][l];
     v.o_nsu = m2.nsu_o[sl][l];
-    if (p.lane_speeds) v.o_pt = m2.pt[sl][l];
-    service_write_obs(v, p, i, obs);
-}
-
-__device__ __forceinline__ void role_s_begin(SVars &v, const EnvParams &, ActRing &ring) {
-    const EnvParams &p = fresh_params();
+    if constexpr (SPEEDS) { if (SpeedParams<SPEEDS>::lane_speeds(p)) v.o_pt = m2.pt[sl][l]; }
+    service_write_obs<SPEEDS>(v, p, i, obs);
+}
+
+template <bool SPEEDS = true>
+__device__ __forceinline__ void role_s_begin(SVars &v, const EnvParams &pk, ActRing &ring) {
+    const EnvParams &p = ABR_S_FRESH_PARAMS ? fresh_params() : pk;
     const int l = threadIdx.x & 63;
     const int64_t i = (int64_t)blockIdx.x * 64 + l;
     v.last_bw = 0.0; v.hist_n = 0.0; v.hist_s = 0.0; v.g_su_obs = 0.0; v.g_rb_obs = 0.0; v.o_buf = 0.0; v.o_pt = 0.0; v.var_run = 0.0;
@@ -528,18 +565,18 @@
         v.g_su_obs = p.G[v.n_su_obs]; v.g_rb_obs = p.G[v.n_rb_obs];
         v.o_chunk = p.chunk_id[i]; v.o_last = p.last_action[i]; v.o_k = p.k[i]; v.o_nplay = p.n_play[i];
         v.o_nrb = p.n_rb[i]; v.o_nsu = p.n_su[i]; v.o_buf = p.buf[i];
-        if (p.lane_speeds) v.o_pt = p.pt_lane[i];
+        if constexpr (SPEEDS) { using SP = SpeedParams<SPEEDS>; if (SP::lane_speeds(p)) v.o_pt = SP::pt_lane(p)[i]; }
     }
     v.a_next = 0; v.a_chunk = v.o_chunk; v.a_ep = v.episode_no;
     if (l == 0) lds_st(&ring.act_hi, 0);
     ABR_STAMP_INIT();
 }
 
-template <int MODE, bool SAMPLE = false, bool LEDGER = false>
-__device__ __forceinline__ void role_s_pre(SVars &v, const EnvParams &, SplitMail &m, SplitMail2 &m2, ActRing &ring,
+template <int MODE, bool SAMPLE = false, bool LEDGER = false, bool SPEEDS = true>
+__device__ __forceinline__ void role_s_pre(SVars &v, const EnvParams &pk, SplitMail &m, typename SplitMail2Of<SPEEDS>::type &m2, ActRing &ring,
                                            float *__restrict__ obs_out, float *__restrict__ reward_out,
                                            uint8_t *__restrict__ done_out, int32_t n_total, uint64_t seed, int32_t t) {
-    const EnvParams &p = fresh_params();
+    const EnvParams &p = ABR_S_FRESH_PARAMS ? fresh_params() : pk;
     const int l = threadIdx.x & 63;
     const int64_t i = (int64_t)blockIdx.x * 64 + l;
     const int cb = t & 1, pb = (t + 1) & 1;
@@ -565,7 +602,7 @@
         lds_writes_done();
         if (l == 0) lds_st(&ring.act_hi, v.a_next);
     }
-    if (t >= 1 && i < p.n_lanes) service_record<SAMPLE, LEDGER>(v, p, m2, pb, obs_out, reward_out, done_out);
+    if (t >= 1 && i < p.n_lanes) service_record<SAMPLE, LEDGER, SPEEDS>(v, p, m2, pb, obs_out, reward_out, done_out);
     v.last_cb = cb;
     ABR_STAMP(21);
 }
@@ -579,16 +616,16 @@
     }
 }
 
-template <int MODE, bool SAMPLE = false, bool LEDGER = false>
-__device__ __forceinline__ void role_s_end(SVars &v, const EnvParams &, SplitMail2 &m2, float *__restrict__ obs_out,
+template <int MODE, bool SAMPLE = false, bool LEDGER = false, bool SPEEDS = true>
+__device__ __forceinline__ void role_s_end(SVars &v, const EnvParams &pk, typename SplitMail2Of<SPEEDS>::type &m2, float *__restrict__ obs_out,
                                            float *__restrict__ reward_out, uint8_t *__restrict__ done_out,
                                            int32_t *__restrict__ actions_out, int32_t n_total,
                                            const abrx::EpisodeSampler &smp = abrx::EpisodeSampler{}) {
-    const EnvParams &p = fresh_params();
+    const EnvParams &p = ABR_S_FRESH_PARAMS ? fresh_params() : pk;
     const int64_t i = (int64_t)blockIdx.x * 64 + (threadIdx.x & 63);
     ABR_STAMP_FLUSH();
     if (i >= p.n_lanes) return;
-    service_record<SAMPLE, LEDGER>(v, p, m2, v.last_cb, obs_out, reward_out, done_out);
+    service_record<SAMPLE, LEDGER, SPEEDS>(v, p, m2, v.last_cb, obs_out, reward_out, done_out);
     if (!v.was_done) {
         if constexpr (SAMPLE) sampled_episode_store(p, smp, i, v.episode_no);
         p.n_su_obs[i] = v.n_su_obs; p.n_rb_obs[i] = v.n_rb_obs; p.episode_no[i] = v.episode_no;
@@ -600,11 +637,11 @@
         if (reward_out) reward_out[o] = 0.0f;
         if (done_out) done_out[o] = v.done;
         if (MODE == 2 && actions_out) actions_out[o] = -1;
-        service_write_obs(v, p, i, obs_out ? obs_out + (int64_t)t2 * ABR_OBS_DIM * p.n_lanes : nullptr);
-    }
-}
-
-template <int MODE, bool SAMPLE = false, bool LEDGER = false>
+        service_write_obs<SPEEDS>(v, p, i, obs_out ? obs_out + (int64_t)t2 * ABR_OBS_DIM * p.n_lanes : nullptr);
+    }
+}
+
+template <int MODE, bool SAMPLE = false, bool LEDGER = false, bool SPEEDS = true>
 __global__ __launch_bounds__(192) __attribute__((amdgpu_waves_per_eu(1, 3))) void env_split3_kernel(
     EnvParams p, const int32_t *__restrict__ actions, float *__restrict__ obs_out,
     float *__restrict__ reward_out, uint8_t *__restrict__ done_out,
@@ -612,7 +649,7 @@
     abrx::EpisodeLedger led) {
     (void)led;
     __shared__ SplitMail m;
-    __shared__ SplitMail2 m2;
+    __shared__ typename SplitMail2Of<SPEEDS>::type m2;
     __shared__ ActRing ring;
     const int32_t n_total = (MODE >= 2) ? n_steps : 1;
     const int role = __builtin_amdgcn_readfirstlane((int)(threadIdx.x >> 6));
@@ -620,34 +657,34 @@
 #ifdef ABR_SPLIT_STAMPS
     if (fresh_params().n_lanes != p.n_lanes || fresh_params().traces != p.traces) __builtin_trap();
 #endif
-    __shared__ RolePark3 park;
+    __shared__ RolePark3T<SPEEDS> park;
     DVars dv;
     role_d_begin(dv, p);
     if (role == 0) ABR_WG_TIME(0);
     ABR_WG_WHERE(role);
     if (role == 0) __builtin_amdgcn_s_setprio(ABR_PRIO_D);
-    else if (role == 1) { __builtin_amdgcn_s_setprio(ABR_PRIO_P); PVars v; role_p3_begin(v, p); p_park(park.p, v); }
-    else { __builtin_amdgcn_s_setprio(ABR_PRIO_S); SVars v; role_s_begin(v, p, ring); s_park(park.s, v); }
+    else if (role == 1) { __builtin_amdgcn_s_setprio(ABR_PRIO_P); PVars v; role_p3_begin<SPEEDS>(v, p); p_park<SPEEDS>(park.p, v); }
+    else { __builtin_amdgcn_s_setprio(ABR_PRIO_S); SVars v; role_s_begin<SPEEDS>(v, p, ring); s_park<SPEEDS>(park.s, v); }
     for (int32_t t = 0;; t++) {
         if (role == 0) {
-            if (t > 0) role_d_validate<SAMPLE>(dv, m, make_tables(p, ABR_SPLIT3_CASCADE != 0), t - 1);
-            role_d_pre<MODE, true, SAMPLE>(dv, p, m, &ring, actions, actions_out, n_total, seed, t, smp);
+            if (t > 0) role_d_validate<SAMPLE>(dv, m, make_tables<SPEEDS>(p, ABR_SPLIT3_CASCADE != 0), t - 1);
+            role_d_pre<MODE, true, SAMPLE, SPEEDS>(dv, p, m, &ring, actions, actions_out, n_total, seed, t, smp);
         } else if (role == 1) {
-            PVars v; p_unpark(park.p, v, p);
-            role_p3_pre<MODE>(v, p, m, m2, n_total, t, t & 1);
-            p_park(park.p, v);
+            PVars v; p_unpark<SPEEDS>(park.p, v, p);
+            role_p3_pre<MODE, SPEEDS>(v, p, m, m2, n_total, t, t & 1);
+            p_park<SPEEDS>(park.p, v);
         } else {
-            SVars v; s_unpark(park.s, v);
-            role_s_pre<MODE, SAMPLE, LEDGER>(v, p, m, m2, ring, obs_out, reward_out, done_out, n_total, seed, t);
-            s_park(park.s, v);
+            SVars v; s_unpark<SPEEDS>(park.s, v);
+            role_s_pre<MODE, SAMPLE, LEDGER, SPEEDS>(v, p, m, m2, ring, obs_out, reward_out, done_out, n_total, seed, t);
+            s_park<SPEEDS>(park.s, v);
         }
         __syncthreads();
         ABR_STAMP(role == 0 ? 5 : (role == 1 ? 18 : 22));
         if (!m.any_alive[t & 1]) break;
     }
     if (role == 0) { role_d_end(dv, p); ABR_WG_TIME(1); }
-    else if (role == 1) { PVars v; p_unpark(park.p, v, p); role_p3_end(v, p); ABR_WG_TIME(2); }
-    else { SVars v; s_unpark(park.s, v); role_s_end<MODE, SAMPLE, LEDGER>(v, p, m2, obs_out, reward_out, done_out, actions_out, n_total, smp); ABR_WG_TIME(3); }
+    else if (role == 1) { PVars v; p_unpark<SPEEDS>(park.p, v, p); role_p3_end<SPEEDS>(v, p); ABR_WG_TIME(2); }
+    else { SVars v; s_unpark<SPEEDS>(park.s, v); role_s_end<MODE, SAMPLE, LEDGER, SPEEDS>(v, p, m2, obs_out, reward_out, done_out, actions_out, n_total, smp); ABR_WG_TIME(3); }
 }
 
 struct P2Vars {
@@ -656,24 +693,27 @@
     int32_t n_su_obs, n_rb_obs;
     uint8_t done;
 };
+template <bool SPEEDS = true>
 __device__ __forceinline__ void p2_park(uint32_t (*area)[64], const P2Vars &v) {
     ParkWords k; k.n = 0;
-    p_words(k, v.pv);
+    p_words<SPEEDS>(k, v.pv);
     pw_f64(k, v.last_bw); pw_f64(k, v.hist_n); pw_f64(k, v.hist_s); pw_f64(k, v.g_su_obs); pw_f64(k, v.g_rb_obs);
     pw_i32(k, v.n_su_obs); pw_i32(k, v.n_rb_obs); pw_i32(k, v.done);
     pw_f64(k, v.var_run); pw_i32(k, 0);
-    park_store<10>(area, k);
-}
+    park_store<SPEEDS ? 10 : 8>(area, k);
+}
+template <bool SPEEDS = true>
 __device__ __forceinline__ void p2_unpark(uint32_t (*area)[64], P2Vars &v, const EnvParams &p) {
-    ParkWords k; park_load<10>(area, k);
+    ParkWords k; park_load<SPEEDS ? 10 : 8>(area, k);
     int at = 0;
-    p_unwords(k, at, v.pv, p);
+    p_unwords<SPEEDS>(k, at, v.pv, p);
     v.last_bw = pr_f64(k, at); v.hist_n = pr_f64(k, at); v.hist_s = pr_f64(k, at); v.g_su_obs = pr_f64(k, at);
     v.g_rb_obs = pr_f64(k, at);
     v.n_su_obs = pr_i32(k, at); v.n_rb_obs = pr_i32(k, at); v.done = (uint8_t)pr_i32(k, at);
     v.var_run = pr_f64(k, at);
 }
 
+template <bool SPEEDS = true>
 __device__ __forceinline__ void role_p2_begin(P2Vars &v, const EnvParams &) {
     const EnvParams &p = fresh_params();
     const int64_t i = (int64_t)blockIdx.x * 64 + (threadIdx.x & 63);
@@ -683,7 +723,7 @@
     if (i < p.n_lanes) {
         v.done = p.done[i];
         v.pv.was_done = v.done != 0;
-        lanej_load(v.pv.s, p, i);
+        lanej_load<SPEEDS>(v.pv.s, p, i);
         v.n_su_obs = p.n_su_obs[i]; v.n_rb_obs = p.n_rb_obs[i]; v.pv.episode_no = p.episode_no[i];
         v.last_bw = p.last_bw[i]; v.hist_n = p.hist_n[i]; v.hist_s = p.hist_s[i]; v.var_run = p.var_run[i];
         v.g_su_obs = p.G[v.n_su_obs]; v.g_rb_obs = p.G[v.n_rb_obs];
@@ -692,7 +732,7 @@
     ABR_STAMP_INIT();
 }
 
-template <int MODE, bool SAMPLE = false, bool LEDGER = false>
+template <int MODE, bool SAMPLE = false, bool LEDGER = false, bool SPEEDS = true>
 __device__ __forceinline__ void role_p2_pre(P2Vars &v, const EnvParams &, SplitMail &m, float *__restrict__ obs_out,
                                             float *__restrict__ reward_out, uint8_t *__restrict__ done_out,
                                             int32_t n_total, int32_t t) {
@@ -700,7 +740,7 @@
     const int l = threadIdx.x & 63;
     const int64_t i = (int64_t)blockIdx.x * 64 + l;
     const int cb = t & 1, pb = (t + 1) & 1;
-    const abrx::Tables tb = make_tables(p);
+    const abrx::TablesT<SPEEDS> tb = make_tables<SPEEDS>(p);
     LaneJ &s = v.pv.s;
     ABR_STAMP(8);
     if (v.pv.b_alive && v.pv.b_step < n_total && t >= 1) {
@@ -716,7 +756,7 @@
                 v.done |= ABR_DONE_BADACT;
                 if (reward_out) ABR_OUT(reward_out[o], 0.0f);
                 if (done_out) ABR_OUT(done_out[o], (uint8_t)v.done);
-                write_obs_j(s, p, i, obs, v.last_bw);
+                write_obs_j<SPEEDS>(s, p, i, obs, v.last_bw);
                 v.pv.b_alive = false;
             } else {
                 abrx::Download d;
@@ -727,7 +767,7 @@
                 const abrx::StepResult sr = abrx::lanej_after_download(s, tb, d, r_avail, a);
                 ABR_STAMP(13);
                 const double g_rb = p.G[s.n_rb], g_su = p.G[s.n_su];
-                double o_k = p.G[s.k], o_pl = p.lane_speeds ? s.pt : p.GP[s.n_play], o_rb = g_rb, o_su = g_su;
+                double o_k = p.G[s.k], o_pl = SpeedParams<SPEEDS>::lane_speeds(p) ? s.pt : p.GP[s.n_play], o_rb = g_rb, o_su = g_su;
                 double var = 0.0;
                 if (sr.hit) {
                     const int64_t h = (int64_t)chunk * p.n_lanes + i;
@@ -751,10 +791,10 @@
                 if (sr.ended || sr.timeout) {
                     p.ep_qoe_terms[0 * p.n_lanes + i] = g_rb;
                     p.ep_qoe_terms[1 * p.n_lanes + i] = g_su;
-                    p.ep_qoe_terms[2 * p.n_lanes + i] = player_latency(p, s);
+                    p.ep_qoe_terms[2 * p.n_lanes + i] = player_latency<SPEEDS>(p, s);
                     p.ep_qoe_terms[3 * p.n_lanes + i] = v.var_run;
                     if constexpr (LEDGER)
-                        ledger_record_split<SAMPLE, false>(p, i, g_rb, g_su, player_latency(p, s), v.var_run, v.pv.episode_no, s.chunk_id, v.done);
+                        ledger_record_split<SAMPLE, false>(p, i, g_rb, g_su, player_latency<SPEEDS>(p, s), v.var_run, v.pv.episode_no, s.chunk_id, v.done);
                     if (p.auto_reset && sr.ended) {
                         abrx::lanej_init_player(s, tb);
                         v.pv.episode_no++;
@@ -762,7 +802,7 @@
                         v.last_bw = 0.0; v.hist_n = 0.0; v.hist_s = 0.0; v.var_run = 0.0;
                         v.done = 0;
                         if (!abrx::lanej_wait_call(s, tb)) v.done |= ABR_DONE_TIMEOUT;
-                        o_k = p.G[s.k]; o_pl = p.lane_speeds ? s.pt : p.GP[s.n_play];
+                        o_k = p.G[s.k]; o_pl = SpeedParams<SPEEDS>::lane_speeds(p) ? s.pt : p.GP[s.n_play];
                         o_rb = p.G[s.n_rb]; o_su = p.G[s.n_su];
                     }
                 }
@@ -778,7 +818,7 @@
     ABR_STAMP(17);
 }
 
-template <int MODE, bool SAMPLE = false>
+template <int MODE, bool SAMPLE = false, bool SPEEDS = true>
 __device__ __forceinline__ void role_p2_end(const P2Vars &v, const EnvParams &, float *__restrict__ obs_out,
                                             float *__restrict__ reward_out, uint8_t *__restrict__ done_out,
                                             int32_t *__restrict__ actions_out, int32_t n_total,
@@ -789,7 +829,7 @@
     if (i >= p.n_lanes) return;
     if (!v.pv.was_done) {
         if constexpr (SAMPLE) sampled_episode_store(p, smp, i, v.pv.episode_no);
-        lanej_store_player(v.pv.s, p, i);
+        lanej_store_player<SPEEDS>(v.pv.s, p, i);
         p.n_su_obs[i] = v.n_su_obs; p.n_rb_obs[i] = v.n_rb_obs; p.episode_no[i] = v.pv.episode_no;
         p.last_bw[i] = v.last_bw; p.hist_n[i] = v.hist_n; p.hist_s[i] = v.hist_s; p.var_run[i] = v.var_run;
         p.done[i] = v.done;
@@ -799,11 +839,11 @@
         if (reward_out) ABR_OUT(reward_out[o], 0.0f);
         if (done_out) ABR_OUT(done_out[o], (uint8_t)v.done);
         if (MODE == 2 && actions_out) ABR_OUT(actions_out[o], (int32_t)-1);
-        write_obs_j(v.pv.s, p, i, obs_out ? obs_out + (int64_t)t2 * ABR_OBS_DIM * p.n_lanes : nullptr, v.last_bw);
-    }
-}
-
-template <int MODE, bool SAMPLE = false, bool LEDGER = false>
+        write_obs_j<SPEEDS>(v.pv.s, p, i, obs_out ? obs_out + (int64_t)t2 * ABR_OBS_DIM * p.n_lanes : nullptr, v.last_bw);
+    }
+}
+
+template <int MODE, bool SAMPLE = false, bool LEDGER = false, bool SPEEDS = true>
 __global__ __launch_bounds__(128) void env_split_kernel(
     EnvParams p, const int32_t *__restrict__ actions, float *__restrict__ obs_out,
     float *__restrict__ reward_out, uint8_t *__restrict__ done_out,
@@ -817,26 +857,26 @@
 #ifdef ABR_SPLIT_STAMPS
     if (fresh_params().n_lanes != p.n_lanes || fresh_params().traces != p.traces) __builtin_trap();
 #endif
-    __shared__ RolePark2 park;
+    __shared__ RolePark2T<SPEEDS> park;
     DVars dv;
     role_d_begin(dv, p);
     if (role == 0) __builtin_amdgcn_s_setprio(2);
-    else { P2Vars v; role_p2_begin(v, p); p2_park(park.p, v); }
+    else { P2Vars v; role_p2_begin<SPEEDS>(v, p); p2_park<SPEEDS>(park.p, v); }
     for (int32_t t = 0;; t++) {
         if (role == 0) {
-            if (t > 0) role_d_validate<SAMPLE>(dv, m, make_tables(p), t - 1);
-            role_d_pre<MODE, false, SAMPLE>(dv, p, m, nullptr, actions, actions_out, n_total, seed, t, smp);
+            if (t > 0) role_d_validate<SAMPLE>(dv, m, make_tables<SPEEDS>(p), t - 1);
+            role_d_pre<MODE, false, SAMPLE, SPEEDS>(dv, p, m, nullptr, actions, actions_out, n_total, seed, t, smp);
         } else {
-            P2Vars v; p2_unpark(park.p, v, fresh_params());
-            role_p2_pre<MODE, SAMPLE, LEDGER>(v, p, m, obs_out, reward_out, done_out, n_total, t);
-            p2_park(park.p, v);
+            P2Vars v; p2_unpark<SPEEDS>(park.p, v, fresh_params());
+            role_p2_pre<MODE, SAMPLE, LEDGER, SPEEDS>(v, p, m, obs_out, reward_out, done_out, n_total, t);
+            p2_park<SPEEDS>(park.p, v);
         }
         __syncthreads();
         ABR_STAMP(role == 0 ? 5 : 18);
         if (!m.any_alive[t & 1]) break;
     }
     if (role == 0) role_d_end(dv, p);
-    else { P2Vars v; p2_unpark(park.p, v, fresh_params()); role_p2_end<MODE, SAMPLE>(v, p, obs_out, reward_out, done_out, actions_out, n_total, smp); }
+    else { P2Vars v; p2_unpark<SPEEDS>(park.p, v, fresh_params()); role_p2_end<MODE, SAMPLE, SPEEDS>(v, p, obs_out, reward_out, done_out, actions_out, n_total, smp); }
 }
 
 #endif
diff --git a/abrsimulator_amd/csrc/abr_lane_jump.h b/abrsimulator_amd/csrc/abr_lane_jump.h
--- a/abrsimulator_amd/csrc/abr_lane_jump.h
+++ b/abrsimulator_amd/csrc/abr_lane_jump.h
@@ -46,7 +46,12 @@
     int32_t log_rows, reserved_;
 };
 
-struct Tables {
+template <bool SPEEDS = true>
+struct TablesT;
+
+template <>
+struct TablesT<true> {
+    static constexpr bool kSpeeds = true;
     const double *G;
     const int32_t *interval_tick;
     const int32_t *avail_tick;
@@ -60,6 +65,24 @@
     DrainTab drain;
 };
 
+template <>
+struct TablesT<false> {
+    static constexpr bool kSpeeds = false;
+    const double *G;
+    const int32_t *interval_tick;
+    const int32_t *avail_tick;
+    double L, sd, max_buffer, start_up_length;
+    int32_t V, max_ticks;
+    static constexpr bool per_lane_speed = false;
+    static constexpr int32_t speed_rows = 0;
+    static constexpr int64_t speed_stride = 0;
+    static constexpr const double *speeds = nullptr;
+    static constexpr const SpeedRuleBlock *rule = nullptr;
+    DrainTab drain;
+};
+
+using Tables = TablesT<true>;
+
 struct Cursor {
     int32_t j;
     int32_t tpos;
@@ -85,22 +108,27 @@
     c.tpos = offset0 % c.tlen;
 }
 
-ABR_HD void lanej_init_player(LaneJ &s, const Tables &t) {
+template <class TB>
+ABR_HD void lanej_init_player(LaneJ &s, const TB &t) {
     s.buf = 0.0; s.sumk = 0;
     s.k = 0; s.chunk_id = 0; s.n_su = 1; s.n_rb = 0; s.n_play = 0;
     s.last_action = -1;
     s.su = true; s.be = true; s.bf = false;
     s.avail_k = t.avail_tick[0];
-    s.pt = 0.0;
-    s.pl_left = 0; s.play_id = 0; s.pt_sum = 0.0;
-}
-
-ABR_HD void lanej_init(LaneJ &s, const Tables &t, int32_t offset0) {
+    if constexpr (TB::kSpeeds) {
+        s.pt = 0.0;
+        s.pl_left = 0; s.play_id = 0; s.pt_sum = 0.0;
+    }
+}
+
+template <class TB>
+ABR_HD void lanej_init(LaneJ &s, const TB &t, int32_t offset0) {
     lanej_init_player(s, t);
     cursor_init(s.cur, offset0);
 }
 
-ABR_HD void lanej_play(LaneJ &s, const Tables &t, int32_t a) {
+template <class TB>
+ABR_HD void lanej_play(LaneJ &s, const TB &t, int32_t a) {
     if (!t.per_lane_speed || a <= 0) return;
     int32_t done = 0;
     double x = s.pt;
@@ -133,7 +161,8 @@
     return a > 0 && b <= 0.0;
 }
 
-ABR_HD bool lanej_drain(const Tables &t, double &b_io, double sd, int32_t m, int32_t &a_out) {
+template <class TB>
+ABR_HD bool lanej_drain(const TB &t, double &b_io, double sd, int32_t m, int32_t &a_out) {
     if (t.drain.n > 0 && !wave_any(!(b_io < t.drain.top))) {
         const bool zero = drain_cascade(t.drain, sd, b_io, m, a_out);
         ABR_STAMP(24);
@@ -142,7 +171,8 @@
     return drain_to_zero(b_io, sd, m, a_out);
 }
 
-ABR_HD void sched_begin_chunk(LaneJ &s, const Tables &t, int32_t k, double b) {
+template <class TB>
+ABR_HD void sched_begin_chunk(LaneJ &s, const TB &t, int32_t k, double b) {
     double v;
     if (t.speed_rows == kSpeedRowsRule) {
 #if defined(__HIP_DEVICE_COMPILE__) && defined(ABR_RULE_KERNARG_OFFSET)
@@ -165,7 +195,8 @@
     s.pl_left = a > 0 ? a : 1;
 }
 
-ABR_HD void sched_played(LaneJ &s, const Tables &t, int32_t a) {
+template <class TB>
+ABR_HD void sched_played(LaneJ &s, const TB &t, int32_t a) {
     if (a <= 0) return;
     s.pt_sum += (double)a * s.pt + s.sd * (double)(((long long)a * (a - 1)) / 2);
     int32_t done = 0;
@@ -176,8 +207,8 @@
     if (s.pl_left == 0) s.play_id++;
 }
 
-template <int STOP>
-ABR_HD bool sched_drain(LaneJ &s, const Tables &t, double &b, double thr, int32_t m, int32_t &a_out) {
+template <int STOP, class TB>
+ABR_HD bool sched_drain(LaneJ &s, const TB &t, double &b, double thr, int32_t m, int32_t &a_out) {
     int32_t a_tot = 0;
     bool hit = false;
     while (a_tot < m && !hit) {
@@ -193,7 +224,8 @@
     return hit;
 }
 
-ABR_HD void lanej_idle(LaneJ &s, const Tables &t, int32_t m) {
+template <class TB>
+ABR_HD void lanej_idle(LaneJ &s, const TB &t, int32_t m) {
     if (m <= 0) return;
     if (s.su && s.buf >= t.start_up_length) s.su = false;
     ABR_STAMP(23);
@@ -205,8 +237,12 @@
         int32_t a = 0;
         double b = s.buf;
         bool zero;
-        if (t.speed_rows >= 2) zero = sched_drain<STOP_LE>(s, t, b, 0.0, m, a);
-        else { zero = lanej_drain(t, b, s.sd, m, a); lanej_play(s, t, a); }
+        if constexpr (TB::kSpeeds) {
+            if (t.speed_rows >= 2) zero = sched_drain<STOP_LE>(s, t, b, 0.0, m, a);
+            else { zero = lanej_drain(t, b, s.sd, m, a); lanej_play(s, t, a); }
+        } else {
+            zero = lanej_drain(t, b, t.sd, m, a);
+        }
         s.n_play += a;
         s.sumk += (long long)a * s.k + ((long long)a * (a - 1)) / 2;
         if (zero) { b = 0.0; s.be = true; s.n_rb += (m - a + 1); }
@@ -216,7 +252,8 @@
     s.k += m;
 }
 
-ABR_HD bool lanej_wait_call(LaneJ &s, const Tables &t) {
+template <class TB>
+ABR_HD bool lanej_wait_call(LaneJ &s, const TB &t) {
     const int32_t mt = t.max_ticks;
     if (s.k >= s.avail_k && !s.bf) return true;
     int32_t w = s.avail_k - s.k;
@@ -233,8 +270,12 @@
         int32_t a = 0;
         double b = s.buf;
         bool cleared;
-        if (t.speed_rows >= 2) cleared = sched_drain<STOP_LT>(s, t, b, t.max_buffer, mt - s.k, a);
-        else { cleared = chain<STOP_LT>(b, -s.sd, t.max_buffer, mt - s.k, a); lanej_play(s, t, a); }
+        if constexpr (TB::kSpeeds) {
+            if (t.speed_rows >= 2) cleared = sched_drain<STOP_LT>(s, t, b, t.max_buffer, mt - s.k, a);
+            else { cleared = chain<STOP_LT>(b, -s.sd, t.max_buffer, mt - s.k, a); lanej_play(s, t, a); }
+        } else {
+            cleared = chain<STOP_LT>(b, -t.sd, t.max_buffer, mt - s.k, a);
+        }
         s.n_play += a;
         s.sumk += (long long)a * s.k + ((long long)a * (a - 1)) / 2;
         s.k += a;
@@ -276,7 +317,8 @@
     int32_t avail_next;
 };
 
-ABR_HD StepLoads lanej_begin_load(const Cursor &s, const Tables &t, int32_t chunk_id) {
+template <class TB>
+ABR_HD StepLoads lanej_begin_load(const Cursor &s, const TB &t, int32_t chunk_id) {
     StepLoads ld;
 #if defined(__HIP_DEVICE_COMPILE__)
 #pragma unroll
@@ -289,7 +331,8 @@
     return ld;
 }
 
-ABR_HD StepStart lanej_begin_select(Cursor &s, const Tables &t, const StepLoads &ld, int32_t k) {
+template <class TB>
+ABR_HD StepStart lanej_begin_select(Cursor &s, const TB &t, const StepLoads &ld, int32_t k) {
     const int32_t *ke = ld.ke;
     const double *bw = ld.bw;
     StepStart st;
@@ -329,7 +372,8 @@
     return st;
 }
 
-ABR_HD StepStart lanej_begin_step(Cursor &s, const Tables &t, int32_t k, int32_t chunk_id) {
+template <class TB>
+ABR_HD StepStart lanej_begin_step(Cursor &s, const TB &t, int32_t k, int32_t chunk_id) {
     const StepLoads ld = lanej_begin_load(s, t, chunk_id);
     return lanej_begin_select(s, t, ld, k);
 }
@@ -340,7 +384,8 @@
     bool hit;
 };
 
-ABR_HD Download lanej_download(Cursor &s, const Tables &t, const StepStart &st, int32_t k,
+template <class TB>
+ABR_HD Download lanej_download(Cursor &s, const TB &t, const StepStart &st, int32_t k,
                                double target) {
     const int32_t mt = t.max_ticks;
     int32_t ke = st.ke < mt ? st.ke : mt, ke_next = st.ke_next, tn = st.tn;
@@ -402,7 +447,8 @@
     return d;
 }
 
-ABR_HD StepResult lanej_after_download(LaneJ &s, const Tables &t, const Download &d,
+template <class TB>
+ABR_HD StepResult lanej_after_download(LaneJ &s, const TB &t, const Download &d,
                                        int32_t avail_next, int32_t action) {
     StepResult r;
     r.bw = 0.0; r.hit = false; r.ended = false; r.timeout = false;
@@ -417,11 +463,15 @@
     double b = s.buf + t.L;
     if (playing) {
         s.sumk += s.k; s.n_play++;
-        if (t.speed_rows >= 2) {
-            if (s.pl_left == 0) sched_begin_chunk(s, t, s.k, b);
-            b = b - s.sd;
-            sched_played(s, t, 1);
-        } else { b = b - s.sd; lanej_play(s, t, 1); }
+        if constexpr (TB::kSpeeds) {
+            if (t.speed_rows >= 2) {
+                if (s.pl_left == 0) sched_begin_chunk(s, t, s.k, b);
+                b = b - s.sd;
+                sched_played(s, t, 1);
+            } else { b = b - s.sd; lanej_play(s, t, 1); }
+        } else {
+            b = b - t.sd;
+        }
     }
     s.bf = b >= t.max_buffer;
     s.be = b <= 0.0;
@@ -446,10 +496,12 @@
     return r;
 }
 
-ABR_HD bool lanej_gate_possible(double buf, bool su, bool be, int32_t n_dl, const Tables &t) {
+template <class TB>
+ABR_HD bool lanej_gate_possible(double buf, bool su, bool be, int32_t n_dl, const TB &t) {
     return !su && !be && !t.per_lane_speed && (buf + t.L) - (double)n_dl * t.sd >= t.max_buffer - 1.0e-6;
 }
-ABR_HD bool lanej_predict_next_call(double buf, int32_t k, int32_t n_dl, int32_t avail_next, const Tables &t,
+template <class TB>
+ABR_HD bool lanej_predict_next_call(double buf, int32_t k, int32_t n_dl, int32_t avail_next, const TB &t,
                                     int32_t &k_next, double *buf_next = nullptr) {
     const int32_t mt = t.max_ticks;
     double b = buf;
@@ -483,13 +535,15 @@
     return true;
 }
 
-ABR_HD StepResult lanej_download_and_wait(LaneJ &s, const Tables &t, const StepStart &st,
+template <class TB>
+ABR_HD StepResult lanej_download_and_wait(LaneJ &s, const TB &t, const StepStart &st,
                                           double target, int32_t action) {
     const Download d = lanej_download(s.cur, t, st, s.k, target);
     return lanej_after_download(s, t, d, st.avail_next, action);
 }
 
-ABR_HD StepResult lanej_step(LaneJ &s, const Tables &t, double target, int32_t action) {
+template <class TB>
+ABR_HD StepResult lanej_step(LaneJ &s, const TB &t, double target, int32_t action) {
     const StepStart st = lanej_begin_step(s.cur, t, s.k, s.chunk_id);
     return lanej_download_and_wait(s, t, st, target, action);
 }
```
